# Maboroshi0327/MHAda-Style-Transfer

Hardware: AMD Instinct MI355X
Metric: stylized frames/sec (whole job) at 512x512 batch 8 fp32 [configs[1]] (higher is better)
Workload: dtype f32; 1 GPU; stylize 512x512 content+style, batch 8; resolution=512, batch_per_gpu=8, global_batch=8, compute_dtype=f32, parallelism=replicas x1

## Files before the change

### include/mhada_hip.h

```cpp
#ifndef MHADA_HIP_H
#define MHADA_HIP_H

#ifdef __cplusplus
extern "C" {
#endif

typedef void* mhada_stream_t;

enum { MHADA_OK = 0, MHADA_ERR_ARG = 1, MHADA_ERR_LAUNCH = 2 };
enum { MHADA_F32 = 0, MHADA_BF16 = 1 };
enum { MHADA_ACT_SOFTMAX = 0, MHADA_ACT_COSINE = 1 };
enum { MHADA_PAD_REFLECT = 0, MHADA_PAD_ZERO = 1 };
enum {
  MHADA_A_ROWS = 0,
  MHADA_A_PATCH8 = 1,
  MHADA_A_CONV3X3 = 2,
  MHADA_A_CONV3X3_UP2 = 3,
  MHADA_A_CONV3X3_ZERO = 4,
  MHADA_A_SPLIT3 = 5
};
enum { MHADA_BF16X3 = 2 };

int mhada_abi_version(void);
const char* mhada_last_error(void);

int mhada_set_tuning(const char* name, int value);
int mhada_get_tuning(const char* name, int* value);

int mhada_clock_probe(unsigned long long* stamps, int nblk, int iters, mhada_stream_t stream);

typedef struct mhada_gemm_args {
  int M, N, K;
  int nb1, nb2;
  int compute;
  int a_mode;
  const void* a; int a_dtype; long long lda, sa1, sa2;
  const float* a_mu; long long smu1, smu2;
  int img_c, img_h, img_w;
  const void* w; long long ldw, sw1, sw2;
  const float* bias; long long sb1, sb2;
  const void* r; int r_dtype; long long ldr, sr1, sr2;
  void* c; int c_dtype; long long ldc, sc1, sc2;
  int relu;
  int pad;
  void* c2; long long ldc2, sc21, sc22;
  void* vt; long long ldt, svt1, svt2;
  int c2_planes;
} mhada_gemm_args;

int mhada_gemm(const mhada_gemm_args* args, mhada_stream_t stream);

int mhada_layernorm(const float* x, void* y, int y_dtype, const float* gamma, const float* beta,
                    int rows, int cols, float eps, mhada_stream_t stream);

int mhada_vit_batch_attn(const void* qkv, void* out, int dtype, int L, int ntok, int heads,
                         int head_dim, mhada_stream_t stream);
int mhada_vit_batch_attn_split3(const float* qkv, void* planes, long long pstride, int L, int ntok, int heads,
                                int head_dim, mhada_stream_t stream);

int mhada_pos_embed(const float* pos, float* out, int C, int bh, int bw, int oh, int ow,
                    mhada_stream_t stream);

int mhada_instnorm_stats(const float* x, float* mu, float* rstd, double* work, int B, int N,
                         int C, int splits, float eps, mhada_stream_t stream);

int mhada_fold_block(const float* wf, const float* wg, const float* wh, const float* bg,
                     const float* bh, const float* rstd_c, const float* mu_s,
                     const float* rstd_s, void* wq, void* wkv, float* bkv, float* v_mu,
                     float kscale, int dtype, int B, int H, mhada_stream_t stream);

int mhada_transpose_v(const void* kv, void* vt, int dtype, int B, int H, int Ns, mhada_stream_t stream);

int mhada_cosine_prep(void* q, void* kv, int dtype, int B, int H, int Nc, int Ns,
                      mhada_stream_t stream);

int mhada_attn(const void* q, const void* kv, const void* vt, const float* fcs,
               const float* fcs_mu, const float* fcs_rstd, const float* v_mu, void* out,
               int dtype, int B, int H, int Nc, int Ns, int activation, mhada_stream_t stream);

int mhada_fold_block_hd(const float* wf, const float* wg, const float* wh, const float* bg,
                        const float* bh, const float* rstd_c, const float* mu_s,
                        const float* rstd_s, void* wq, void* wkv, float* bkv, float* v_mu,
                        float kscale, int dtype, int B, int H, int D, mhada_stream_t stream);

int mhada_cosine_prep_hd(void* q, void* kv, int dtype, int B, int H, int D, int Nc, int Ns,
                         mhada_stream_t stream);

int mhada_attn_hd(const void* q, const void* kv, const float* fcs, const float* fcs_mu,
                  const float* fcs_rstd, const float* v_mu, void* out, int dtype, int B, int H,
                  int D, int Nc, int Ns, int activation, mhada_stream_t stream);

int mhada_attn_wide(const void* q, const void* k, const void* v, const float* fcs, const float* fcs_mu,
                    const float* fcs_rstd, const float* v_mu, float* out, void* out16, int dtype, int B,
                    int Nc, int Ns, int D, mhada_stream_t stream);

int mhada_split3_kv(const float* kv, const float* vt, void* img, int B, int H, int Ns, mhada_stream_t stream);
int mhada_split3_rows(const float* x, void* planes, long long n, mhada_stream_t stream);
int mhada_split3_weight(const float* w, void* out, int N, int K0, int transposed, mhada_stream_t stream);

int mhada_layernorm_half2(const float* x, void* y, const float* gamma, const float* beta, int rows, int cols,
                          float eps, float scale, mhada_stream_t stream);
int mhada_half2_weight(const float* w, void* out, float* t, int N, int K0, mhada_stream_t stream);
int mhada_gemm_half2(const mhada_gemm_args* args, const float* col_scale, mhada_stream_t stream);
int mhada_gemm_half2_planes(const mhada_gemm_args* args, const float* col_scale, const float* out_scale,
                            mhada_stream_t stream);
int mhada_vit_batch_attn_half2(const float* qkv, void* planes, long long pstride, const float* out_scale, int L,
                               int ntok, int heads, int head_dim, mhada_stream_t stream);
int mhada_kv_proj_split3(const float* fs, const float* mu_s, const float* wkv, const float* bkv, void* img,
                         int B, int H, int Ns, mhada_stream_t stream);
int mhada_attn_split3(const float* q, const void* img, const float* fcs, const float* fcs_mu,
                      const float* fcs_rstd, const float* v_mu, float* out, int B, int H, int Nc, int Ns,
                      mhada_stream_t stream);
int mhada_attn_split3_planes(const float* q, const void* img, const float* fcs, const float* fcs_mu,
                             const float* fcs_rstd, const float* v_mu, void* planes, int B, int H, int Nc, int Ns,
                             mhada_stream_t stream);

int mhada_cosine_moments(const void* kv, const void* vt, int dtype, int B, int H, int Ns, float* mom,
                         float* work, int splits, mhada_stream_t stream);
int mhada_cosine_attn(const void* q, const float* mom, const float* fcs, const float* fcs_mu,
                      const float* fcs_rstd, const float* v_mu, void* out, int dtype, int B, int H,
                      int Nc, mhada_stream_t stream);

int mhada_attn_train_fwd(const float* q, const float* k, const float* v, const float* x, float* out,
                         float* mo, float* lse, int BH, int Nc, int Ns, mhada_stream_t stream);
int mhada_attn_train_fwd_vt(const float* q, const float* k, const float* v, float* vt, const float* x,
                            float* out, float* mo, float* lse, int BH, int Nc, int Ns, mhada_stream_t stream);
int mhada_attn_train_fwd_split3(const float* q, const float* k, const float* v, void* img, const float* x,
                                float* out, float* mo, float* lse, int BH, int Nc, int Ns, mhada_stream_t stream);
int mhada_transpose64(const float* src, float* dst, int BH, int N, int ldt, mhada_stream_t stream);
int mhada_gemm_n64_split3(const float* a, const void* w_planes, float* c, int nz, int M, int K, int lda,
                          long long sa, int ldw, long long sw, long long wps, int ldc, long long sc,
                          mhada_stream_t stream);
int mhada_transpose64_split3(const float* k, void* planes, int BH, int N, int ldt, mhada_stream_t stream);
int mhada_attn_train_bwd(const float* q, const float* k, const float* v, const float* lse,
                         const float* dmo, const float* dd, float* dq, float* dk, float* dv,
                         int BH, int Nc, int Ns, mhada_stream_t stream);
int mhada_attn_train_dkv(const float* q, const float* k, const float* v, const float* lse, const float* dmo,
                         const float* dd, float* dk, float* dv, float* ds, int BH, int Nc, int Ns,
                         mhada_stream_t stream);

int mhada_attn_train_fwd_hd(const float* q, const float* k, const float* v, const float* x, float* out,
                            float* mo, float* lse, int BH, int D, int Nc, int Ns, mhada_stream_t stream);
int mhada_attn_train_bwd_hd(const float* q, const float* k, const float* v, const float* lse,
                            const float* dmo, const float* dd, float* dq, float* dk, float* dv,
                            int BH, int D, int Nc, int Ns, mhada_stream_t stream);

int mhada_attn_train_dq(const float* q, const float* k, const float* v, const float* lse, const float* dmo,
                        const float* dd, float* dq, int BH, int Nc, int Ns, mhada_stream_t stream);
int mhada_attn_train_dq_hd(const float* q, const float* k, const float* v, const float* lse, const float* dmo,
                           const float* dd, float* dq, int BH, int D, int Nc, int Ns, mhada_stream_t stream);

long long mhada_attn_train_bf16_workspace(int BH, int Nc, int Ns, int backward);
int mhada_attn_train_fwd_bf16(const float* q, const float* k, const float* v, const float* x, float* out,
                              float* mo, float* lse, void* ws, long long ws_size, int BH, int Nc, int Ns,
                              mhada_stream_t stream);
int mhada_attn_train_bwd_bf16(const float* q, const float* k, const float* v, const float* lse,
                              const float* dmo, const float* mo, float* dq, float* dk, float* dv,
                              void* ws, long long ws_size, int BH, int Nc, int Ns, int phases,
                              mhada_stream_t stream);

int mhada_conv3x3_out3(const void* x, int dtype, const float* w, const float* b, float* y,
                       int B, int H, int W, int Cin, int clamp255, mhada_stream_t stream);

int mhada_upsample2x(const void* x, void* y, int dtype, int B, int H, int W, int C,
                     mhada_stream_t stream);


int mhada_warp(const float* x, const float* flow, float* y, int B, int C, int H, int W,
               int padding, mhada_stream_t stream);

int mhada_warp_bwd(const float* gy, const float* flow, float* gx, int B, int C, int H, int W,
                   int padding, mhada_stream_t stream);

int mhada_flow_warp_mask(const float* flo01, const float* flo10, float* mask, int H, int W,
                         float threshold, int padding, mhada_stream_t stream);

int mhada_warp_l1(const float* cs1, const float* cs2, const float* flow, const float* mask,
                  double* work, float* out, int B, int C, int H, int W, mhada_stream_t stream);


typedef struct mhada_gemm_tn_args {
  int M, N, K;
  const float* a; long long lda;
  const float* b; long long ldb;
  int b_mode;
  int img_c, img_h, img_w, pad;
  float* c; long long ldc;
  float* colsum;
  int nb;
  long long sza, szb;
} mhada_gemm_tn_args;
int mhada_gemm_tn_splits(int M, int N, int K);
int mhada_gemm_tn(const mhada_gemm_tn_args* args, float* work, long long work_floats, mhada_stream_t stream);

int mhada_vit_batch_attn_bwd(const float* qkv, const float* dout, float* dqkv, int L, int ntok, int heads,
                             int head_dim, mhada_stream_t stream);
int mhada_vit_batch_attn_bwd_split3(const float* qkv, const float* dout, float* dqkv, void* planes,
                                    long long pstride, int L, int ntok, int heads, int head_dim,
                                    mhada_stream_t stream);

int mhada_colsum(const float* x, float* out, long long rows, int C, float* work, long long work_floats,
                 mhada_stream_t stream);

int mhada_layernorm_fwd(const float* x, float* y, float* stats, const float* gamma, const float* beta,
                        int rows, int cols, float eps, mhada_stream_t stream);
int mhada_layernorm_fwd_split3(const float* x, float* y, void* planes, float* stats, const float* gamma,
                               const float* beta, int rows, int cols, float eps, mhada_stream_t stream);

int mhada_layernorm_bwd(const float* x, const float* dy, const float* stats, const float* gamma, float* dx,
                        float* dgamma, float* dbeta, float* work, long long work_floats, int rows, int cols,
                        mhada_stream_t stream);

int mhada_instnorm_bwd(const float* dy, const float* y, const float* rstd, float* dx, double* work,
                       int B, int N, int C, int splits, mhada_stream_t stream);

int mhada_attn_train_bwd_prep(const float* dout, const float* x, const float* mo, float* dx, float* dmo,
                              float* dd, long long rows, mhada_stream_t stream);
int mhada_attn_train_bwd_prep_hd(const float* dout, const float* x, const float* mo, float* dx, float* dmo,
                                 float* dd, long long rows, int D, mhada_stream_t stream);

int mhada_pos_embed_bwd(const float* g, float* gpos, int C, int bh, int bw, int oh, int ow,
                        mhada_stream_t stream);
long long mhada_feat_stats_work(int B, long long P, int C);
int mhada_feat_stats(const float* x, const float* t, float* mu, float* sd, float* mse, double* work,
                     long long work_doubles, int B, long long P, int C, mhada_stream_t stream);
int mhada_feat_loss_bwd(const float* x, const float* t, const float* mu, const float* alpha, const float* beta,
                        const float* kp, float ks, float* g, int B, long long P, int C, int relu, mhada_stream_t stream);
int mhada_relu_bwd(const float* dy, const float* y, float* dx, long long n, mhada_stream_t stream);
int mhada_reflect_fold(const float* dxp, float* dx, int B, int H, int W, int C, const float* relu_mask,
                       mhada_stream_t stream);
int mhada_maxpool2(const float* x, float* y, int B, int H, int W, int C, mhada_stream_t stream);
int mhada_maxpool2_bwd(const float* x, const float* dy, float* dx, int B, int H, int W, int C, int relu_mask,
                       mhada_stream_t stream);
int mhada_upsample2x_bwd(const float* dy, const float* relu_x, float* dx, int B, int H, int W, int C,
                         mhada_stream_t stream);
int mhada_vgg_input(const float* img, float* out, int B, int H, int W, int Cp, mhada_stream_t stream);
int mhada_vgg_input_bwd(const float* dout, float* dimg, int B, int H, int W, int Cp, mhada_stream_t stream);

int mhada_loss_attn(const float* q, const float* k, const float* v, const float* x, const float* x_mu,
                    const float* x_rs, float* out, int B, int Nq, int Ns, int Dqk, int Dv, int activation,
                    mhada_stream_t stream);
int mhada_rows_normalize(const float* x, const float* mu, const float* rs, float* out, int unit,
                         int B, int N, int C, mhada_stream_t stream);

int mhada_frame_ingest(const void* frames, int B, int H, int W, long long row_bytes, int bgr, float* out,
                       int Ho, int Wo, mhada_stream_t stream);

int mhada_wino_weights(const float* w, float* u, int Cout, int Cin, mhada_stream_t stream);
int mhada_conv3x3_wgrad_wino_splits(int B, int H, int W, int Cin, int Cout);
int mhada_conv3x3_wgrad_wino(const float* x, const float* g, float* dw, float* db, float* work, long long work_floats,
                             int B, int H, int W, int Cin, int Cout, long long ldg, int pad_mode,
                             mhada_stream_t stream);
int mhada_conv3x3_wino(const float* x, const float* u, const float* bias, float* y, int B, int H, int W,
                       int Cin, int Cout, long long ldc, int pad_mode, int pad, int relu,
                       const float* relu_mask, mhada_stream_t stream);
int mhada_wino_weights_split3(const float* w, void* up, int Cout, int Cin, mhada_stream_t stream);
int mhada_conv3x3_wino_split3(const float* x, const float* u, const void* up, const float* bias, float* y, int B,
                              int H, int W, int Cin, int Cout, long long ldc, int pad_mode, int pad, int relu,
                              const float* relu_mask, mhada_stream_t stream);

int mhada_vgg_stem_dgrad(const float* dy, const float* y, const float* wd, float* dimg, int B, int H, int W,
                         mhada_stream_t stream);
int mhada_out3_dgrad(const float* dy, const float* y, const float* wd, const float* relu_x, float* dx, int B, int H,
                     int W, mhada_stream_t stream);
long long mhada_out3_wgrad_work(int B, int H, int W);
int mhada_out3_wgrad(const float* x, const float* dy, const float* y, float* dw, float* db, float* work,
                     long long work_floats, int B, int H, int W, mhada_stream_t stream);

int mhada_patch_embed_dgrad(const float* dy, const float* w, float* dimg, int B, int C, int Ci, int H, int W,
                            mhada_stream_t stream);

#ifdef __cplusplus
}
#endif
#endif
```

### mhada-style-transfer_amd/csrc/attn_split3.hip

```cpp
#include "attn_common.h"

namespace mhada {

constexpr int kS3Tk = 64;

__host__ __device__ constexpr long long s3_image(int ldt) { return 576LL * ldt; }

struct Bf3 { bf16 a, b, c; };
MHADA_DEV Bf3 split3(float x) {
  const bf16 a = (bf16)x;
  const float r = x - (float)a;
  const bf16 b = (bf16)r;
  return Bf3{a, b, (bf16)(r - (float)b)};
}
template <typename V>
MHADA_DEV void split3_into(float x, V& a, V& b, V& c, int e) {
  const Bf3 s = split3(x);
  a[e] = s.a;
  b[e] = s.b;
  c[e] = s.c;
}

__global__ void __launch_bounds__(256) split3_kv_kernel(const float* __restrict__ kv, const float* __restrict__ vt,
                                                        bf16* __restrict__ img, int Ns, int ldt) {
  const int bh = blockIdx.y, n0 = blockIdx.x * 64, tid = threadIdx.x;
  bf16* kp = img + (long long)bh * s3_image(ldt);
  bf16* vp = kp + 192LL * ldt;
  const float* kvb = kv + (long long)bh * Ns * 128;
  const float* vtb = vt + (long long)bh * 128 * ldt;
  const long long kps = 64LL * ldt, vps = 128LL * ldt;
#pragma unroll
  for (int i = 0; i < 4; ++i) {
    const int idx = tid + 256 * i, key = n0 + (idx >> 4), d = (idx & 15) * 4;
    const f32x4 x = key < Ns ? *reinterpret_cast<const f32x4*>(kvb + (long long)key * 128 + d) : f32x4{0.f, 0.f, 0.f, 0.f};
    bf16x4 a, b, c;
#pragma unroll
    for (int e = 0; e < 4; ++e) split3_into(x[e], a, b, c, e);
    bf16* dst = kp + (long long)key * 64 + d;
    *reinterpret_cast<bf16x4*>(dst) = a;
    *reinterpret_cast<bf16x4*>(dst + kps) = b;
    *reinterpret_cast<bf16x4*>(dst + 2 * kps) = c;
  }
#pragma unroll
  for (int i = 0; i < 4; ++i) {
    const int idx = tid + 256 * i, row = idx >> 3, a8 = idx & 7;
    const float* src = vtb + (long long)row * ldt + n0 + 16 * (a8 >> 1) + 4 * (a8 & 1);
    const f32x4 lo = *reinterpret_cast<const f32x4*>(src), hi = *reinterpret_cast<const f32x4*>(src + 8);
    bf16x8 a, b, c;
#pragma unroll
    for (int j = 0; j < 8; ++j) split3_into(j < 4 ? lo[j] : hi[j - 4], a, b, c, j);
    bf16* dst = vp + (long long)row * ldt + n0 + 8 * a8;
    *reinterpret_cast<bf16x8*>(dst) = a;
    *reinterpret_cast<bf16x8*>(dst + vps) = b;
    *reinterpret_cast<bf16x8*>(dst + 2 * vps) = c;
  }
}

__global__ void __launch_bounds__(256) kv_proj_s3_kernel(const float* __restrict__ fs, const float* __restrict__ mu,
                                                         const float* __restrict__ wkv, const float* __restrict__ bkv,
                                                         bf16* __restrict__ img, int H, int Ns, int ldt) {
  constexpr int LX = 65, LY = 65;
  __shared__ float sm[192 * LX];
  float* sX = sm;
  float* sW = sm + 64 * LX;
  float* sY = sm;
  const int bh = blockIdx.y, b = bh / H, h = bh - b * H, n0 = blockIdx.x * 64, tid = threadIdx.x;
  const int C = 64 * H;
  const float* xb = fs + (long long)b * Ns * C + 64 * h;
  const float* mb = mu + (long long)b * C + 64 * h;
  const float* wb = wkv + (long long)bh * 128 * 64;
#pragma unroll
  for (int i = 0; i < 4; ++i) {
    const int idx = tid + 256 * i, n = idx >> 4, c = (idx & 15) * 4;
    f32x4 x = {0.f, 0.f, 0.f, 0.f};
    if (n0 + n < Ns) {
      x = *reinterpret_cast<const f32x4*>(xb + (long long)(n0 + n) * C + c);
      const f32x4 m = *reinterpret_cast<const f32x4*>(mb + c);
      x = x - m;
    }
#pragma unroll
    for (int e = 0; e < 4; ++e) sX[n * LX + c + e] = x[e];
  }
#pragma unroll
  for (int i = 0; i < 8; ++i) {
    const int idx = tid + 256 * i, o = idx >> 4, c = (idx & 15) * 4;
    const f32x4 w = *reinterpret_cast<const f32x4*>(wb + o * 64 + c);
#pragma unroll
    for (int e = 0; e < 4; ++e) sW[o * LX + c + e] = w[e];
  }
  __syncthreads();
  const int lane = tid & 63, wave = tid >> 6, r32 = lane & 31, hh = lane >> 5;
  const int nb = wave & 1, ob = wave >> 1;
  f32x16 acc[2] = {};
#pragma unroll 8
  for (int k = 0; k < 64; k += 2) {
    const float bv = sX[(32 * nb + r32) * LX + k + hh];
#pragma unroll
    for (int ni = 0; ni < 2; ++ni)
      acc[ni] = __builtin_amdgcn_mfma_f32_32x32x2f32(sW[(64 * ob + 32 * ni + r32) * LX + k + hh], bv, acc[ni], 0, 0, 0);
  }
  const float* bb = bkv + h * 128;
  __syncthreads();
#pragma unroll
  for (int ni = 0; ni < 2; ++ni)
#pragma unroll
    for (int r = 0; r < 16; ++r) {
      const int o = 64 * ob + 32 * ni + (r & 3) + 8 * (r >> 2) + 4 * hh;
      sY[o * LY + 32 * nb + r32] = acc[ni][r] + bb[o];
    }
  __syncthreads();
  bf16* kp = img + (long long)bh * s3_image(ldt);
  bf16* vp = kp + 192LL * ldt;
  const long long kps = 64LL * ldt, vps = 128LL * ldt;
#pragma unroll
  for (int i = 0; i < 2; ++i) {
    const int idx = tid + 256 * i, n = idx >> 3, o0 = (idx & 7) * 8;
    const bool valid = n0 + n < Ns;
    bf16x8 a, c1, c2;
#pragma unroll
    for (int j = 0; j < 8; ++j) split3_into(valid ? sY[(o0 + j) * LY + n] : 0.f, a, c1, c2, j);
    bf16* dst = kp + (long long)(n0 + n) * 64 + o0;
    *reinterpret_cast<bf16x8*>(dst) = a;
    *reinterpret_cast<bf16x8*>(dst + kps) = c1;
    *reinterpret_cast<bf16x8*>(dst + 2 * kps) = c2;
  }
#pragma unroll
  for (int i = 0; i < 2; ++i) {
    const int idx = tid + 256 * i, vo = idx >> 3, a8 = idx & 7;
    bf16x8 a, c1, c2, s0, s1, s2;
#pragma unroll
    for (int j = 0; j < 8; ++j) {
      const int n = 16 * (a8 >> 1) + 8 * (j >> 2) + 4 * (a8 & 1) + (j & 3);
      const float v = n0 + n < Ns ? sY[(64 + vo) * LY + n] : 0.f;
      split3_into(v, a, c1, c2, j);
      split3_into(v * v, s0, s1, s2, j);
    }
    bf16* dst = vp + (long long)vo * ldt + n0 + 8 * a8;
    *reinterpret_cast<bf16x8*>(dst) = a;
    *reinterpret_cast<bf16x8*>(dst + vps) = c1;
    *reinterpret_cast<bf16x8*>(dst + 2 * vps) = c2;
    *reinterpret_cast<bf16x8*>(dst + 64LL * ldt) = s0;
    *reinterpret_cast<bf16x8*>(dst + 64LL * ldt + vps) = s1;
    *reinterpret_cast<bf16x8*>(dst + 64LL * ldt + 2 * vps) = s2;
  }
}

MHADA_DEV f32x4 mfma6(const bf16x8& a0, const bf16x8& a1, const bf16x8& a2, const bf16x8& b0, const bf16x8& b1,
                      const bf16x8& b2, f32x4 acc) {
  acc = __builtin_amdgcn_mfma_f32_16x16x32_bf16(a2, b0, acc, 0, 0, 0);
  acc = __builtin_amdgcn_mfma_f32_16x16x32_bf16(a1, b1, acc, 0, 0, 0);
  acc = __builtin_amdgcn_mfma_f32_16x16x32_bf16(a0, b2, acc, 0, 0, 0);
  acc = __builtin_amdgcn_mfma_f32_16x16x32_bf16(a1, b0, acc, 0, 0, 0);
  acc = __builtin_amdgcn_mfma_f32_16x16x32_bf16(a0, b1, acc, 0, 0, 0);
  return __builtin_amdgcn_mfma_f32_16x16x32_bf16(a0, b0, acc, 0, 0, 0);
}

template <bool QK32>
MHADA_DEV void attn_exact_q3(const AttnP& p, const bf16* kp, const bf16* vp, const bf16x8 (&qf)[3][2][2],
                             const float (&qreg)[2][16], f32x4 (&O)[2][8], float (&lt)[2], float (&mx)[2], int g,
                             int r16) {
  const int Ns = p.Ns;
  const long long kps = 64LL * p.ldt, vps = 128LL * p.ldt;
  const f32x4 z4 = {0.f, 0.f, 0.f, 0.f};
  auto scores = [&](int k0, f32x4 (&S)[2][2]) {
#pragma unroll
    for (int t = 0; t < 2; ++t) {
      const bf16* kr = kp + (long long)(k0 + fsq_key(r16, t)) * 64 + 8 * g;
#pragma unroll
      for (int qg = 0; qg < 2; ++qg) S[qg][t] = z4;
      if constexpr (QK32) {
        const float* kf = reinterpret_cast<const float*>(kp) + (long long)(k0 + fsq_key(r16, t)) * 64 + 16 * g;
#pragma unroll
        for (int st = 0; st < 16; ++st)
#pragma unroll
          for (int qg = 0; qg < 2; ++qg) S[qg][t] = __builtin_amdgcn_mfma_f32_16x16x4f32(kf[st], qreg[qg][st], S[qg][t], 0, 0, 0);
      }
#pragma unroll
      for (int dh = 0; dh < (QK32 ? 0 : 2); ++dh) {
        const bf16x8 k0f = *reinterpret_cast<const bf16x8*>(kr + 32 * dh);
        const bf16x8 k1f = *reinterpret_cast<const bf16x8*>(kr + kps + 32 * dh);
        const bf16x8 k2f = *reinterpret_cast<const bf16x8*>(kr + 2 * kps + 32 * dh);
#pragma unroll
        for (int qg = 0; qg < 2; ++qg)
          S[qg][t] = mfma6(k0f, k1f, k2f, qf[0][qg][dh], qf[1][qg][dh], qf[2][qg][dh], S[qg][t]);
      }
#pragma unroll
      for (int j = 0; j < 4; ++j)
        if (k0 + fsq_key(4 * g + j, t) >= Ns) S[0][t][j] = S[1][t][j] = -INFINITY;
    }
  };
  float m2[2] = {-INFINITY, -INFINITY};
  for (int k0 = 0; k0 < Ns; k0 += 32) {
    f32x4 S[2][2];
    scores(k0, S);
#pragma unroll
    for (int qg = 0; qg < 2; ++qg)
#pragma unroll
      for (int t = 0; t < 2; ++t)
#pragma unroll
        for (int j = 0; j < 4; ++j) m2[qg] = fmaxf(m2[qg], S[qg][t][j]);
  }
#pragma unroll
  for (int qg = 0; qg < 2; ++qg) {
    m2[qg] = fmaxf(m2[qg], __shfl_xor(m2[qg], 16, 64));
    m2[qg] = fmaxf(m2[qg], __shfl_xor(m2[qg], 32, 64));
    lt[qg] = 0.f;
#pragma unroll
    for (int i = 0; i < 8; ++i) O[qg][i] = z4;
  }
  for (int k0 = 0; k0 < Ns; k0 += 32) {
    f32x4 S[2][2];
    scores(k0, S);
    bf16x8 pf[3][2];
#pragma unroll
    for (int qg = 0; qg < 2; ++qg)
#pragma unroll
      for (int j = 0; j < 8; ++j) {
        const float e = fast_exp2(S[qg][j >> 2][j & 3] - m2[qg]);
        lt[qg] += e;
        split3_into(e, pf[0][qg], pf[1][qg], pf[2][qg], j);
      }
#pragma unroll
    for (int dvb = 0; dvb < 8; ++dvb) {
      const bf16* vr = vp + (long long)(16 * dvb + r16) * p.ldt + k0 + 8 * g;
      const bf16x8 v0 = *reinterpret_cast<const bf16x8*>(vr);
      const bf16x8 v1 = *reinterpret_cast<const bf16x8*>(vr + vps);
      const bf16x8 v2 = *reinterpret_cast<const bf16x8*>(vr + 2 * vps);
#pragma unroll
      for (int qg = 0; qg < 2; ++qg) O[qg][dvb] += mfma6(v0, v1, v2, pf[0][qg], pf[1][qg], pf[2][qg], z4);
    }
  }
#pragma unroll
  for (int qg = 0; qg < 2; ++qg) {
    lt[qg] += __shfl_xor(lt[qg], 16, 64);
    lt[qg] += __shfl_xor(lt[qg], 32, 64);
    mx[qg] = m2[qg];
  }
}

MHADA_DEV void s3_mask(f32x4 (&S)[2][2][2], int key0, int Ns, int g) {
#pragma unroll
  for (int kg = 0; kg < 2; ++kg)
#pragma unroll
    for (int t = 0; t < 2; ++t)
#pragma unroll
      for (int j = 0; j < 4; ++j)
        if (key0 + 32 * kg + fsq_key(4 * g + j, t) >= Ns) S[0][kg][t][j] = S[1][kg][t][j] = -INFINITY;
}

__global__ void __launch_bounds__(256) train_s3_prep_kernel(const float* __restrict__ k, const float* __restrict__ v,
                                                            bf16* __restrict__ img, int Ns, int ldt) {
  __shared__ float sv[64 * 65];
  const int bh = blockIdx.y, n0 = blockIdx.x * 64, tid = threadIdx.x;
  bf16* kp = img + (long long)bh * s3_image(ldt);
  bf16* vp = kp + 192LL * ldt;
  const float* kb = k + (long long)bh * Ns * 64;
  const float* vb = v + (long long)bh * Ns * 64;
  const long long vps = 128LL * ldt;
#pragma unroll
  for (int i = 0; i < 4; ++i) {
    const int idx = tid + 256 * i, n = idx >> 4, d = (idx & 15) * 4;
    const bool ok = n0 + n < Ns;
    const f32x4 x = ok ? *reinterpret_cast<const f32x4*>(kb + (long long)(n0 + n) * 64 + d) : f32x4{0.f, 0.f, 0.f, 0.f};
    const f32x4 y = ok ? *reinterpret_cast<const f32x4*>(vb + (long long)(n0 + n) * 64 + d) : f32x4{0.f, 0.f, 0.f, 0.f};
    float* kf = reinterpret_cast<float*>(kp) + (long long)(n0 + n) * 64 + d / 4;
#pragma unroll
    for (int e = 0; e < 4; ++e) kf[16 * e] = x[e];
#pragma unroll
    for (int e = 0; e < 4; ++e) sv[n * 65 + d + e] = y[e];
  }
  __syncthreads();
#pragma unroll
  for (int i = 0; i < 2; ++i) {
    const int idx = tid + 256 * i, o = idx >> 3, a8 = idx & 7;
    bf16x8 a, c1, c2, s0, s1, s2;
#pragma unroll
    for (int j = 0; j < 8; ++j) {
      const int n = 16 * (a8 >> 1) + 8 * (j >> 2) + 4 * (a8 & 1) + (j & 3);
      const float x = sv[n * 65 + o];
      split3_into(x, a, c1, c2, j);
      split3_into(x * x, s0, s1, s2, j);
    }
    bf16* dst = vp + (long long)o * ldt + n0 + 8 * a8;
    *reinterpret_cast<bf16x8*>(dst) = a;
    *reinterpret_cast<bf16x8*>(dst + vps) = c1;
    *reinterpret_cast<bf16x8*>(dst + 2 * vps) = c2;
    *reinterpret_cast<bf16x8*>(dst + 64LL * ldt) = s0;
    *reinterpret_cast<bf16x8*>(dst + 64LL * ldt + vps) = s1;
    *reinterpret_cast<bf16x8*>(dst + 64LL * ldt + 2 * vps) = s2;
  }
}

MHADA_DEV void attn_train_epilogue_q(const AttnP& p, const f32x4 (&O)[2][8], const float (&lt)[2],
                                     const float (&m2)[2], long long bh, int q0, int g, int r16) {
#pragma unroll
  for (int qg = 0; qg < 2; ++qg) {
    const int q = q0 + 16 * qg + r16;
    if (q >= p.Nc) continue;
    const float inv = 1.0f / lt[qg];
    const long long row = bh * p.Nc + q;
    const float* xr = p.fcs + row * 64;
    float* orow = reinterpret_cast<float*>(p.out) + row * 64;
    float* mrow = p.mo + row * 128;
#pragma unroll
    for (int dvb = 0; dvb < 4; ++dvb) {
      const int dv0 = 16 * dvb + 4 * g;
      const f32x4 xx = *reinterpret_cast<const f32x4*>(xr + dv0);
      f32x4 o, mm, ee;
#pragma unroll
      for (int e = 0; e < 4; ++e) {
        const float m1 = O[qg][dvb][e] * inv;
        const float e2 = O[qg][dvb + 4][e] * inv;
        o[e] = sqrtf(fmaxf(e2 - m1 * m1, 1e-6f)) * xx[e] + m1;
        mm[e] = m1;
        ee[e] = e2;
      }
      *reinterpret_cast<f32x4*>(orow + dv0) = o;
      *reinterpret_cast<f32x4*>(mrow + dv0) = mm;
      *reinterpret_cast<f32x4*>(mrow + 64 + dv0) = ee;
    }
    if (g == 0) p.lse[row] = m2[qg] + __log2f(lt[qg]);
  }
}

template <int NW, bool TRAIN = false, bool QK32 = false, int ACC = 0, int IL = 0, bool PLANES = false>
__global__ void __launch_bounds__(64 * NW, 1) attn_s3_kernel(const AttnP p) {
  constexpr int TK = kS3Tk;
  constexpr int KPL = TK * 64, VPL = 128 * TK;
  constexpr int KREG = QK32 ? 2 * TK * 64 : 3 * KPL;
  constexpr int SLOT = KREG + 3 * VPL;
  constexpr int KPC = KREG / 512, VPC = 3 * VPL / 512;
  static_assert(KPC % NW == 0 && VPC % NW == 0, "tile config");
  constexpr int KPW = KPC / NW, VPW = VPC / NW;
  __shared__ __attribute__((aligned(16))) bf16 smem[2 * SLOT];
  int b, hh, qb;
  decode_block(p, b, hh, qb);
  const int tid = threadIdx.x, lane = tid & 63, wave = __builtin_amdgcn_readfirstlane(tid >> 6);
  const int g = lane >> 4, r16 = lane & 15;
  const int q0 = qb * (32 * NW) + wave * 32;
  const long long bh = (long long)b * p.H + hh;
  const int Ns = p.Ns, ldt = p.ldt;
  const f32x4 z4 = {0.f, 0.f, 0.f, 0.f};

  bf16x8 qf[3][2][2];
  float qreg[2][16];
#pragma unroll
  for (int qg = 0; qg < 2; ++qg) {
    const int q = q0 + 16 * qg + r16;
    if constexpr (QK32) {
      const float* qr = reinterpret_cast<const float*>(p.q) + (bh * p.Nc + (q < p.Nc ? q : 0)) * 64 + g;
#pragma unroll
      for (int st = 0; st < 16; ++st) qreg[qg][st] = q < p.Nc ? qr[4 * st] * 1.4426950408889634f : 0.f;
      continue;
    }
    const float* qp = reinterpret_cast<const float*>(p.q) + (bh * p.Nc + (q < p.Nc ? q : 0)) * 64 + 8 * g;
#pragma unroll
    for (int dh = 0; dh < 2; ++dh) {
      const f32x4 lo = *reinterpret_cast<const f32x4*>(qp + 32 * dh);
      const f32x4 hi = *reinterpret_cast<const f32x4*>(qp + 32 * dh + 4);
#pragma unroll
      for (int e = 0; e < 8; ++e) {
        const float x = q < p.Nc ? (e < 4 ? lo[e] : hi[e - 4]) * (TRAIN ? 1.4426950408889634f : 1.0f) : 0.f;
        split3_into(x, qf[0][qg][dh], qf[1][qg][dh], qf[2][qg][dh], e);
      }
    }
  }
  const bf16* kp = reinterpret_cast<const bf16*>(p.kv) + bh * s3_image(ldt);
  const bf16* vp = kp + 192LL * ldt;
  int ksrc[KPW], vsrc[VPW];
#pragma unroll
  for (int i = 0; i < KPW; ++i) {
    if constexpr (QK32) {
      const int pc = NW * i + wave, row = 4 * pc + (lane >> 4), slot = lane & 15;
      const int f = (row & 3) | (((row >> 2) & 1) << 3);
      ksrc[i] = 2 * (row * 64 + 4 * (slot ^ f));
    } else {
      const int pc = NW * i + wave, pl = pc >> 3, row = 8 * (pc & 7) + (lane >> 3), slot = lane & 7;
      ksrc[i] = pl * 64 * ldt + row * 64 + 8 * (slot ^ (row & 7));
    }
  }
#pragma unroll
  for (int i = 0; i < VPW; ++i) {
    const int pc = NW * i + wave, pl = pc >> 4, row = 8 * (pc & 15) + (lane >> 3), slot = lane & 7;
    vsrc[i] = pl * 128 * ldt + row * ldt + 8 * (slot ^ ((row >> 1) & 7));
  }
  auto stage = [&](int key0, int sl) {
    bf16* kd = smem + sl * SLOT;
    bf16* vd = kd + KREG;
    const bf16* ks = kp + (long long)key0 * (QK32 ? 128 : 64);
    const bf16* vs = vp + key0;
#pragma unroll
    for (int i = 0; i < KPW; ++i) attn_glds16(ks + ksrc[i], kd + 512 * (NW * i + wave));
#pragma unroll
    for (int i = 0; i < VPW; ++i) attn_glds16(vs + vsrc[i], vd + 512 * (NW * i + wave));
  };
  int krow[2];
#pragma unroll
  for (int t = 0; t < 2; ++t) krow[t] = fsq_key(r16, t) * 64;
  auto qk = [&](int sl, f32x4 (&S)[2][2][2], const f32x4 (&init)[2]) {
    if constexpr (QK32) {
      const float* ck = reinterpret_cast<const float*>(smem + sl * SLOT);
      const int f = (r16 & 3) | (((r16 >> 2) & 1) << 3);
#pragma unroll
      for (int kg = 0; kg < 2; ++kg)
#pragma unroll
        for (int t = 0; t < 2; ++t) {
          const float* kr = ck + (kg * 32 + fsq_key(r16, t)) * 64;
          f32x4 kf[4];
#pragma unroll
          for (int j = 0; j < 4; ++j) kf[j] = *reinterpret_cast<const f32x4*>(kr + 4 * ((4 * g + j) ^ f));
#pragma unroll
          for (int st = 0; st < 16; ++st)
#pragma unroll
            for (int qg = 0; qg < 2; ++qg)
              S[qg][kg][t] = __builtin_amdgcn_mfma_f32_16x16x4f32(kf[st >> 2][st & 3], qreg[qg][st],
                                                                  st == 0 ? init[qg] : S[qg][kg][t], 0, 0, 0);
        }
      return;
    }
    const bf16* ck = smem + sl * SLOT;
#pragma unroll
    for (int kg = 0; kg < 2; ++kg)
#pragma unroll
      for (int t = 0; t < 2; ++t) {
        const bf16* kr = ck + kg * 32 * 64 + krow[t];
#pragma unroll
        for (int dh = 0; dh < 2; ++dh) {
          const int off = 8 * ((4 * dh + g) ^ (r16 & 7));
          const bf16x8 k0f = *reinterpret_cast<const bf16x8*>(kr + off);
          const bf16x8 k1f = *reinterpret_cast<const bf16x8*>(kr + KPL + off);
          const bf16x8 k2f = *reinterpret_cast<const bf16x8*>(kr + 2 * KPL + off);
#pragma unroll
          for (int qg = 0; qg < 2; ++qg)
            S[qg][kg][t] = mfma6(k0f, k1f, k2f, qf[0][qg][dh], qf[1][qg][dh], qf[2][qg][dh],
                                 dh == 0 ? init[qg] : S[qg][kg][t]);
        }
      }
  };
  f32x4 O[2][8], L[2];
  float lsum[2] = {0.f, 0.f};
#pragma unroll
  for (int qg = 0; qg < 2; ++qg) {
    L[qg] = z4;
#pragma unroll
    for (int i = 0; i < 8; ++i) O[qg][i] = z4;
  }
  bf16x8 ones;
#pragma unroll
  for (int j = 0; j < 8; ++j) ones[j] = (bf16)1.0f;
  auto pv = [&](int sl, int kg, int dvb, const bf16x8 (&pf)[3][2]) {
    const int off = 8 * ((4 * kg + g) ^ ((r16 >> 1) & 7));
    const bf16* vr = smem + sl * SLOT + KREG + (16 * dvb + r16) * TK + off;
    const bf16x8 v0 = *reinterpret_cast<const bf16x8*>(vr);
    const bf16x8 v1 = *reinterpret_cast<const bf16x8*>(vr + VPL);
    const bf16x8 v2 = *reinterpret_cast<const bf16x8*>(vr + 2 * VPL);
#pragma unroll
    for (int qg = 0; qg < 2; ++qg) O[qg][dvb] = mfma6(v0, v1, v2, pf[0][qg], pf[1][qg], pf[2][qg], O[qg][dvb]);
  };
  auto rowsum = [&](const bf16x8 (&pf)[3][2]) {
#pragma unroll
    for (int qg = 0; qg < 2; ++qg) {
      L[qg] = __builtin_amdgcn_mfma_f32_16x16x32_bf16(ones, pf[2][qg], L[qg], 0, 0, 0);
      L[qg] = __builtin_amdgcn_mfma_f32_16x16x32_bf16(ones, pf[1][qg], L[qg], 0, 0, 0);
      L[qg] = __builtin_amdgcn_mfma_f32_16x16x32_bf16(ones, pf[0][qg], L[qg], 0, 0, 0);
    }
  };
  auto finish = [&](int sl, const f32x4 (&S)[2][2][2]) {
    const bf16* cv = smem + sl * SLOT + KREG;
    if constexpr (IL != 0 && ACC == 0) {
      bf16x8 pa[3][2], pb[3][2];
#pragma unroll
      for (int qg = 0; qg < 2; ++qg)
#pragma unroll
        for (int j = 0; j < 8; ++j) split3_into(fast_exp2(S[qg][0][j >> 2][j & 3]), pa[0][qg], pa[1][qg], pa[2][qg], j);
      rowsum(pa);
#pragma unroll
      for (int dvb = 0; dvb < 8; ++dvb) {
        pv(sl, 0, dvb, pa);
        const int qg = dvb >> 2, j = 2 * (dvb & 3);
        split3_into(fast_exp2(S[qg][1][j >> 2][j & 3]), pb[0][qg], pb[1][qg], pb[2][qg], j);
        split3_into(fast_exp2(S[qg][1][(j + 1) >> 2][(j + 1) & 3]), pb[0][qg], pb[1][qg], pb[2][qg], j + 1);
      }
      rowsum(pb);
#pragma unroll
      for (int dvb = 0; dvb < 8; ++dvb) pv(sl, 1, dvb, pb);
      return;
    }
#pragma unroll
    for (int kg = 0; kg < 2; ++kg) {
      bf16x8 pf[3][2];
#pragma unroll
      for (int qg = 0; qg < 2; ++qg)
#pragma unroll
        for (int j = 0; j < 8; ++j) split3_into(fast_exp2(S[qg][kg][j >> 2][j & 3]), pf[0][qg], pf[1][qg], pf[2][qg], j);
#pragma unroll
      for (int qg = 0; qg < 2; ++qg) {
        if constexpr (ACC == 0) {
          L[qg] = __builtin_amdgcn_mfma_f32_16x16x32_bf16(ones, pf[2][qg], L[qg], 0, 0, 0);
          L[qg] = __builtin_amdgcn_mfma_f32_16x16x32_bf16(ones, pf[1][qg], L[qg], 0, 0, 0);
          L[qg] = __builtin_amdgcn_mfma_f32_16x16x32_bf16(ones, pf[0][qg], L[qg], 0, 0, 0);
        } else {
          f32x4 t = __builtin_amdgcn_mfma_f32_16x16x32_bf16(ones, pf[2][qg], z4, 0, 0, 0);
          t = __builtin_amdgcn_mfma_f32_16x16x32_bf16(ones, pf[1][qg], t, 0, 0, 0);
          t = __builtin_amdgcn_mfma_f32_16x16x32_bf16(ones, pf[0][qg], t, 0, 0, 0);
          lsum[qg] += t[0];
        }
      }
      const int off = 8 * ((4 * kg + g) ^ ((r16 >> 1) & 7));
      f32x4 tp[2];
#pragma unroll
      for (int dvb = 0; dvb < 8; ++dvb) {
        const bf16* vr = cv + (16 * dvb + r16) * TK + off;
        const bf16x8 v0 = *reinterpret_cast<const bf16x8*>(vr);
        const bf16x8 v1 = *reinterpret_cast<const bf16x8*>(vr + VPL);
        const bf16x8 v2 = *reinterpret_cast<const bf16x8*>(vr + 2 * VPL);
        if constexpr (ACC == 0) {
#pragma unroll
          for (int qg = 0; qg < 2; ++qg) O[qg][dvb] = mfma6(v0, v1, v2, pf[0][qg], pf[1][qg], pf[2][qg], O[qg][dvb]);
        } else {
          f32x4 tn[2];
#pragma unroll
          for (int qg = 0; qg < 2; ++qg) tn[qg] = mfma6(v0, v1, v2, pf[0][qg], pf[1][qg], pf[2][qg], z4);
          if (dvb > 0) {
#pragma unroll
            for (int qg = 0; qg < 2; ++qg) O[qg][dvb - 1] += tp[qg];
          }
#pragma unroll
          for (int qg = 0; qg < 2; ++qg) tp[qg] = tn[qg];
        }
      }
      if constexpr (ACC != 0) {
#pragma unroll
        for (int qg = 0; qg < 2; ++qg) O[qg][7] += tp[qg];
      }
    }
  };

  const int NTILE = (Ns + TK - 1) / TK, NFULL = Ns / TK;
  stage(0, 0);
  asm volatile("s_waitcnt vmcnt(0)" ::: "memory");
  __syncthreads();
  f32x4 Sa[2][2][2], Cm[2];
  {
    const f32x4 zi[2] = {z4, z4};
    qk(0, Sa, zi);
    if (NFULL == 0) s3_mask(Sa, 0, Ns, g);
#pragma unroll
    for (int qg = 0; qg < 2; ++qg) {
      float m = -INFINITY;
#pragma unroll
      for (int kg = 0; kg < 2; ++kg)
#pragma unroll
        for (int t = 0; t < 2; ++t)
#pragma unroll
          for (int j = 0; j < 4; ++j) m = fmaxf(m, Sa[qg][kg][t][j]);
      m = fmaxf(m, __shfl_xor(m, 16, 64));
      m = fmaxf(m, __shfl_xor(m, 32, 64));
#pragma unroll
      for (int kg = 0; kg < 2; ++kg)
#pragma unroll
        for (int t = 0; t < 2; ++t)
#pragma unroll
          for (int j = 0; j < 4; ++j) Sa[qg][kg][t][j] -= m;
      Cm[qg] = f32x4{-m, -m, -m, -m};
    }
  }
  if (NTILE > 1) stage(TK, 1);
  finish(0, Sa);
  asm volatile("s_waitcnt vmcnt(0)" ::: "memory");
  __builtin_amdgcn_s_barrier();
  for (int t = 1; t < NFULL; ++t) {
    if (t + 1 < NTILE) stage((t + 1) * TK, (t + 1) & 1);
    qk(t & 1, Sa, Cm);
    finish(t & 1, Sa);
    asm volatile("s_waitcnt vmcnt(0)" ::: "memory");
    __builtin_amdgcn_s_barrier();
  }
  if (NFULL < NTILE && NFULL > 0) {
    qk(NFULL & 1, Sa, Cm);
    s3_mask(Sa, NFULL * TK, Ns, g);
    finish(NFULL & 1, Sa);
  }
  float lt[2], mx[2];
#pragma unroll
  for (int qg = 0; qg < 2; ++qg) {
    lt[qg] = ACC ? lsum[qg] : L[qg][0];
    mx[qg] = -Cm[qg][0];
  }
  if (__any(!(lt[0] <= kShiftSumThr) || !(lt[1] <= kShiftSumThr))) attn_exact_q3<QK32>(p, kp, vp, qf, qreg, O, lt, mx, g, r16);
  if constexpr (TRAIN) attn_train_epilogue_q(p, O, lt, mx, bh, q0, g, r16);
  else attn_epilogue_q<float, PLANES>(p, O, lt, b, hh, q0, g, r16);
}

static int s3_num_cus() {
  static int n = 0;
  if (n == 0) {
    int dev = 0;
    (void)hipGetDevice(&dev);
    if (hipDeviceGetAttribute(&n, hipDeviceAttributeMultiprocessorCount, dev) != hipSuccess || n <= 0) n = 256;
  }
  return n;
}

}

using namespace mhada;

extern "C" int mhada_split3_kv(const float* kv, const float* vt, void* img, int B, int H, int Ns, mhada_stream_t s_) {
  if (!kv || !vt || !img || B <= 0 || H <= 0 || Ns <= 0) return fail("mhada_split3_kv: bad args");
  const long long bhn = (long long)B * H;
  if (bhn > 65535) return fail("mhada_split3_kv: B * H > 65535");
  const int ldt = (Ns + 63) / 64 * 64;
  hipLaunchKernelGGL(split3_kv_kernel, dim3(ldt / 64, (unsigned)bhn), dim3(256), 0, (hipStream_t)s_, kv, vt,
                     reinterpret_cast<bf16*>(img), Ns, ldt);
  return check_launch("mhada_split3_kv");
}

extern "C" int mhada_kv_proj_split3(const float* fs, const float* mu_s, const float* wkv, const float* bkv, void* img,
                                    int B, int H, int Ns, mhada_stream_t s_) {
  if (!fs || !mu_s || !wkv || !bkv || !img || B <= 0 || H <= 0 || Ns <= 0) return fail("mhada_kv_proj_split3: bad args");
  const long long bhn = (long long)B * H;
  if (bhn > 65535) return fail("mhada_kv_proj_split3: B * H > 65535");
  const int ldt = (Ns + 63) / 64 * 64;
  hipLaunchKernelGGL(kv_proj_s3_kernel, dim3(ldt / 64, (unsigned)bhn), dim3(256), 0, (hipStream_t)s_, fs, mu_s, wkv, bkv,
                     reinterpret_cast<bf16*>(img), H, Ns, ldt);
  return check_launch("mhada_kv_proj_split3");
}

static int attn_split3_launch(const char* name, const float* q, const void* img, const float* fcs, const float* fcs_mu,
                              const float* fcs_rstd, const float* v_mu, void* out, bool planes, int B, int H, int Nc,
                              int Ns, mhada_stream_t s_) {
  if (!q || !img || !fcs || !fcs_mu || !fcs_rstd || !v_mu || !out || B <= 0 || H <= 0 || Nc <= 0 || Ns <= 0)
    return fail(std::string(name) + ": bad args");
  AttnP p = {};
  p.q = q; p.kv = img; p.vt = img; p.fcs = fcs; p.fcs_mu = fcs_mu; p.fcs_rstd = fcs_rstd; p.v_mu = v_mu;
  p.out = out; p.B = B; p.H = H; p.Nc = Nc; p.Ns = Ns;
  p.ldt = (Ns + 63) / 64 * 64;
  if (384LL * p.ldt >= (1LL << 31)) return fail(std::string(name) + ": Ns too large for 32-bit plane offsets");
  int nw = tuning().attn_waves;
  if (nw == 0) nw = (long long)B * H * ((Nc + 255) / 256) < s3_num_cus() ? 4 : 8;
  p.nqb = (Nc + 32 * nw - 1) / (32 * nw);
  const long long nblk = (long long)B * H * p.nqb;
  if (nblk > (1LL << 31) - 1) return fail(std::string(name) + ": grid too large");
  p.nblk = (int)nblk;
  const hipStream_t s = (hipStream_t)s_;
  if (planes) {
    if (nw == 8) hipLaunchKernelGGL((attn_s3_kernel<8, false, false, 0, 1, true>), dim3(p.nblk), dim3(512), 0, s, p);
    else hipLaunchKernelGGL((attn_s3_kernel<4, false, false, 0, 1, true>), dim3(p.nblk), dim3(256), 0, s, p);
  } else {
    if (nw == 8) hipLaunchKernelGGL((attn_s3_kernel<8, false, false, 0, 1>), dim3(p.nblk), dim3(512), 0, s, p);
    else hipLaunchKernelGGL((attn_s3_kernel<4, false, false, 0, 1>), dim3(p.nblk), dim3(256), 0, s, p);
  }
  return check_launch(name);
}

extern "C" int mhada_attn_split3(const float* q, const void* img, const float* fcs, const float* fcs_mu,
                                 const float* fcs_rstd, const float* v_mu, float* out, int B, int H, int Nc, int Ns,
                                 mhada_stream_t s_) {
  return attn_split3_launch("mhada_attn_split3", q, img, fcs, fcs_mu, fcs_rstd, v_mu, out, false, B, H, Nc, Ns, s_);
}

extern "C" int mhada_attn_split3_planes(const float* q, const void* img, const float* fcs, const float* fcs_mu,
                                        const float* fcs_rstd, const float* v_mu, void* planes, int B, int H, int Nc,
                                        int Ns, mhada_stream_t s_) {
  return attn_split3_launch("mhada_attn_split3_planes", q, img, fcs, fcs_mu, fcs_rstd, v_mu, planes, true, B, H, Nc, Ns,
                            s_);
}

extern "C" int mhada_attn_train_fwd_split3(const float* q, const float* k, const float* v, void* img, const float* x,
                                           float* out, float* mo, float* lse, int BH, int Nc, int Ns,
                                           mhada_stream_t s_) {
  if (!q || !k || !v || !img || !x || !out || !mo || !lse || BH <= 0 || Nc <= 0 || Ns <= 0)
    return fail("mhada_attn_train_fwd_split3: bad args");
  if (BH > 65535) return fail("mhada_attn_train_fwd_split3: BH > 65535");
  const hipStream_t s = (hipStream_t)s_;
  AttnP p = {};
  p.q = q; p.kv = img; p.vt = img; p.fcs = x; p.out = out; p.mo = mo; p.lse = lse;
  p.B = BH; p.H = 1; p.Nc = Nc; p.Ns = Ns; p.ldk = 64;
  p.ldt = (Ns + 63) / 64 * 64;
  if (384LL * p.ldt >= (1LL << 31)) return fail("mhada_attn_train_fwd_split3: Ns too large for 32-bit plane offsets");
  int nw = tuning().attn_waves;
  if (nw == 0) nw = (long long)BH * ((Nc + 255) / 256) < s3_num_cus() ? 4 : 8;
  p.nqb = (Nc + 32 * nw - 1) / (32 * nw);
  const long long nblk = (long long)BH * p.nqb;
  if (nblk > (1LL << 31) - 1) return fail("mhada_attn_train_fwd_split3: grid too large");
  p.nblk = (int)nblk;
  hipLaunchKernelGGL(train_s3_prep_kernel, dim3(p.ldt / 64, BH), dim3(256), 0, s, k, v, reinterpret_cast<bf16*>(img),
                     Ns, p.ldt);
  if (nw == 8) hipLaunchKernelGGL((attn_s3_kernel<8, true, true, 1>), dim3(p.nblk), dim3(512), 0, s, p);
  else hipLaunchKernelGGL((attn_s3_kernel<4, true, true, 1>), dim3(p.nblk), dim3(256), 0, s, p);
  return check_launch("mhada_attn_train_fwd_split3");
}
```

### mhada-style-transfer_amd/mhada_hip/_lib.py

```python
from __future__ import annotations

import ctypes
import os
import threading

LIB_PATH = os.path.join(os.path.dirname(os.path.abspath(__file__)), "libmhada_hip.so")

F32, BF16 = 0, 1
ACT_SOFTMAX, ACT_COSINE = 0, 1
A_ROWS, A_PATCH8, A_CONV3X3, A_CONV3X3_UP2, A_CONV3X3_ZERO, A_SPLIT3 = 0, 1, 2, 3, 4, 5
BF16X3 = 2
PAD_REFLECT, PAD_ZERO = 0, 1

_c_ll = ctypes.c_longlong
_vp = ctypes.c_void_p


class GemmArgs(ctypes.Structure):
    _fields_ = [
        ("M", ctypes.c_int), ("N", ctypes.c_int), ("K", ctypes.c_int),
        ("nb1", ctypes.c_int), ("nb2", ctypes.c_int),
        ("compute", ctypes.c_int), ("a_mode", ctypes.c_int),
        ("a", _vp), ("a_dtype", ctypes.c_int), ("lda", _c_ll), ("sa1", _c_ll), ("sa2", _c_ll),
        ("a_mu", _vp), ("smu1", _c_ll), ("smu2", _c_ll),
        ("img_c", ctypes.c_int), ("img_h", ctypes.c_int), ("img_w", ctypes.c_int),
        ("w", _vp), ("ldw", _c_ll), ("sw1", _c_ll), ("sw2", _c_ll),
        ("bias", _vp), ("sb1", _c_ll), ("sb2", _c_ll),
        ("r", _vp), ("r_dtype", ctypes.c_int), ("ldr", _c_ll), ("sr1", _c_ll), ("sr2", _c_ll),
        ("c", _vp), ("c_dtype", ctypes.c_int), ("ldc", _c_ll), ("sc1", _c_ll), ("sc2", _c_ll),
        ("relu", ctypes.c_int), ("pad", ctypes.c_int),
        ("c2", _vp), ("ldc2", _c_ll), ("sc21", _c_ll), ("sc22", _c_ll),
        ("vt", _vp), ("ldt", _c_ll), ("svt1", _c_ll), ("svt2", _c_ll),
        ("c2_planes", ctypes.c_int),
    ]


class GemmTnArgs(ctypes.Structure):
    _fields_ = [
        ("M", ctypes.c_int), ("N", ctypes.c_int), ("K", ctypes.c_int),
        ("a", _vp), ("lda", _c_ll), ("b", _vp), ("ldb", _c_ll), ("b_mode", ctypes.c_int),
        ("img_c", ctypes.c_int), ("img_h", ctypes.c_int), ("img_w", ctypes.c_int), ("pad", ctypes.c_int),
        ("c", _vp), ("ldc", _c_ll), ("colsum", _vp),
        ("nb", ctypes.c_int), ("sza", _c_ll), ("szb", _c_ll),
    ]


_I, _F = ctypes.c_int, ctypes.c_float
SIGNATURES = {
    "mhada_abi_version": (_I, []),
    "mhada_last_error": (ctypes.c_char_p, []),
    "mhada_set_tuning": (_I, [ctypes.c_char_p, _I]),
    "mhada_get_tuning": (_I, [ctypes.c_char_p, ctypes.POINTER(_I)]),
    "mhada_clock_probe": (_I, [_vp, _I, _I, _vp]),
    "mhada_gemm": (_I, [ctypes.POINTER(GemmArgs), _vp]),
    "mhada_layernorm": (_I, [_vp, _vp, _I, _vp, _vp, _I, _I, _F, _vp]),
    "mhada_vit_batch_attn": (_I, [_vp, _vp, _I, _I, _I, _I, _I, _vp]),
    "mhada_vit_batch_attn_split3": (_I, [_vp, _vp, _c_ll, _I, _I, _I, _I, _vp]),
    "mhada_pos_embed": (_I, [_vp, _vp, _I, _I, _I, _I, _I, _vp]),
    "mhada_instnorm_stats": (_I, [_vp, _vp, _vp, _vp, _I, _I, _I, _I, _F, _vp]),
    "mhada_fold_block": (_I, [_vp] * 12 + [_F, _I, _I, _I, _vp]),
    "mhada_transpose_v": (_I, [_vp, _vp, _I, _I, _I, _I, _vp]),
    "mhada_cosine_prep": (_I, [_vp, _vp, _I, _I, _I, _I, _I, _vp]),
    "mhada_cosine_moments": (_I, [_vp, _vp, _I, _I, _I, _I, _vp, _vp, _I, _vp]),
    "mhada_cosine_attn": (_I, [_vp, _vp, _vp, _vp, _vp, _vp, _vp, _I, _I, _I, _I, _vp]),
    "mhada_attn": (_I, [_vp] * 8 + [_I, _I, _I, _I, _I, _I, _vp]),
    "mhada_fold_block_hd": (_I, [_vp] * 12 + [_F, _I, _I, _I, _I, _vp]),
    "mhada_cosine_prep_hd": (_I, [_vp, _vp, _I, _I, _I, _I, _I, _I, _vp]),
    "mhada_attn_hd": (_I, [_vp] * 7 + [_I, _I, _I, _I, _I, _I, _I, _vp]),
    "mhada_attn_wide": (_I, [_vp] * 9 + [_I, _I, _I, _I, _I, _vp]),
    "mhada_split3_kv": (_I, [_vp, _vp, _vp, _I, _I, _I, _vp]),
    "mhada_kv_proj_split3": (_I, [_vp] * 5 + [_I, _I, _I, _vp]),
    "mhada_split3_rows": (_I, [_vp, _vp, _c_ll, _vp]),
    "mhada_split3_weight": (_I, [_vp, _vp, _I, _I, _I, _vp]),
    "mhada_layernorm_half2": (_I, [_vp, _vp, _vp, _vp, _I, _I, _F, _F, _vp]),
    "mhada_half2_weight": (_I, [_vp, _vp, _vp, _I, _I, _vp]),
    "mhada_gemm_half2": (_I, [ctypes.POINTER(GemmArgs), _vp, _vp]),
    "mhada_gemm_half2_planes": (_I, [ctypes.POINTER(GemmArgs), _vp, _vp, _vp]),
    "mhada_vit_batch_attn_half2": (_I, [_vp, _vp, _c_ll, _vp, _I, _I, _I, _I, _vp]),
    "mhada_attn_split3": (_I, [_vp] * 7 + [_I, _I, _I, _I, _vp]),
    "mhada_attn_split3_planes": (_I, [_vp] * 7 + [_I, _I, _I, _I, _vp]),
    "mhada_attn_train_fwd": (_I, [_vp] * 7 + [_I, _I, _I, _vp]),
    "mhada_attn_train_fwd_vt": (_I, [_vp] * 8 + [_I, _I, _I, _vp]),
    "mhada_attn_train_fwd_split3": (_I, [_vp] * 8 + [_I, _I, _I, _vp]),
    "mhada_transpose64": (_I, [_vp, _vp, _I, _I, _I, _vp]),
    "mhada_gemm_n64_split3": (_I, [_vp, _vp, _vp, _I, _I, _I, _I, _c_ll, _I, _c_ll, _c_ll, _I, _c_ll, _vp]),
    "mhada_transpose64_split3": (_I, [_vp, _vp, _I, _I, _I, _vp]),
    "mhada_attn_train_bwd": (_I, [_vp] * 9 + [_I, _I, _I, _vp]),
    "mhada_attn_train_dkv": (_I, [_vp] * 9 + [_I, _I, _I, _vp]),
    "mhada_attn_train_fwd_hd": (_I, [_vp] * 7 + [_I, _I, _I, _I, _vp]),
    "mhada_attn_train_bwd_hd": (_I, [_vp] * 9 + [_I, _I, _I, _I, _vp]),
    "mhada_attn_train_dq": (_I, [_vp] * 7 + [_I, _I, _I, _vp]),
    "mhada_attn_train_dq_hd": (_I, [_vp] * 7 + [_I, _I, _I, _I, _vp]),
    "mhada_patch_embed_dgrad": (_I, [_vp, _vp, _vp, _I, _I, _I, _I, _I, _vp]),
    "mhada_attn_train_bf16_workspace": (_c_ll, [_I, _I, _I, _I]),
    "mhada_attn_train_fwd_bf16": (_I, [_vp] * 8 + [_c_ll, _I, _I, _I, _vp]),
    "mhada_attn_train_bwd_bf16": (_I, [_vp] * 10 + [_c_ll, _I, _I, _I, _I, _vp]),
    "mhada_conv3x3_out3": (_I, [_vp, _I, _vp, _vp, _vp, _I, _I, _I, _I, _I, _vp]),
    "mhada_upsample2x": (_I, [_vp, _vp, _I, _I, _I, _I, _I, _vp]),
    "mhada_warp": (_I, [_vp, _vp, _vp, _I, _I, _I, _I, _I, _vp]),
    "mhada_warp_bwd": (_I, [_vp, _vp, _vp, _I, _I, _I, _I, _I, _vp]),
    "mhada_flow_warp_mask": (_I, [_vp, _vp, _vp, _I, _I, _F, _I, _vp]),
    "mhada_warp_l1": (_I, [_vp, _vp, _vp, _vp, _vp, _vp, _I, _I, _I, _I, _vp]),
    "mhada_frame_ingest": (_I, [_vp, _I, _I, _I, _c_ll, _I, _vp, _I, _I, _vp]),
    "mhada_gemm_tn_splits": (_I, [_I, _I, _I]),
    "mhada_loss_attn": (_I, [_vp] * 7 + [_I, _I, _I, _I, _I, _I, _vp]),
    "mhada_rows_normalize": (_I, [_vp] * 4 + [_I, _I, _I, _I, _vp]),
    "mhada_gemm_tn": (_I, [ctypes.POINTER(GemmTnArgs), _vp, _c_ll, _vp]),
    "mhada_colsum": (_I, [_vp, _vp, _c_ll, _I, _vp, _c_ll, _vp]),
    "mhada_layernorm_fwd": (_I, [_vp, _vp, _vp, _vp, _vp, _I, _I, _F, _vp]),
    "mhada_layernorm_fwd_split3": (_I, [_vp, _vp, _vp, _vp, _vp, _vp, _I, _I, _F, _vp]),
    "mhada_layernorm_bwd": (_I, [_vp, _vp, _vp, _vp, _vp, _vp, _vp, _vp, _c_ll, _I, _I, _vp]),
    "mhada_pos_embed_bwd": (_I, [_vp, _vp, _I, _I, _I, _I, _I, _vp]),
    "mhada_instnorm_bwd": (_I, [_vp, _vp, _vp, _vp, _vp, _I, _I, _I, _I, _vp]),
    "mhada_attn_train_bwd_prep": (_I, [_vp, _vp, _vp, _vp, _vp, _vp, _c_ll, _vp]),
    "mhada_attn_train_bwd_prep_hd": (_I, [_vp, _vp, _vp, _vp, _vp, _vp, _c_ll, _I, _vp]),
    "mhada_vit_batch_attn_bwd": (_I, [_vp, _vp, _vp, _I, _I, _I, _I, _vp]),
    "mhada_vit_batch_attn_bwd_split3": (_I, [_vp, _vp, _vp, _vp, _c_ll, _I, _I, _I, _I, _vp]),
    "mhada_relu_bwd": (_I, [_vp, _vp, _vp, _c_ll, _vp]),
    "mhada_feat_stats_work": (_c_ll, [_I, _c_ll, _I]),
    "mhada_feat_stats": (_I, [_vp, _vp, _vp, _vp, _vp, _vp, _c_ll, _I, _c_ll, _I, _vp]),
    "mhada_feat_loss_bwd": (_I, [_vp, _vp, _vp, _vp, _vp, _vp, _F, _vp, _I, _c_ll, _I, _I, _vp]),
    "mhada_reflect_fold": (_I, [_vp, _vp, _I, _I, _I, _I, _vp, _vp]),
    "mhada_maxpool2": (_I, [_vp, _vp, _I, _I, _I, _I, _vp]),
    "mhada_maxpool2_bwd": (_I, [_vp, _vp, _vp, _I, _I, _I, _I, _I, _vp]),
    "mhada_upsample2x_bwd": (_I, [_vp, _vp, _vp, _I, _I, _I, _I, _vp]),
    "mhada_vgg_input": (_I, [_vp, _vp, _I, _I, _I, _I, _vp]),
    "mhada_vgg_input_bwd": (_I, [_vp, _vp, _I, _I, _I, _I, _vp]),
    "mhada_wino_weights": (_I, [_vp, _vp, _I, _I, _vp]),
    "mhada_conv3x3_wgrad_wino_splits": (_I, [_I, _I, _I, _I, _I]),
    "mhada_conv3x3_wgrad_wino": (_I, [_vp, _vp, _vp, _vp, _vp, _c_ll, _I, _I, _I, _I, _I, _c_ll, _I, _vp]),
    "mhada_conv3x3_wino": (_I, [_vp] * 4 + [_I] * 5 + [_c_ll, _I, _I, _I, _vp, _vp]),
    "mhada_conv3x3_wino_split3": (_I, [_vp] * 5 + [_I] * 5 + [_c_ll, _I, _I, _I, _vp, _vp]),
    "mhada_wino_weights_split3": (_I, [_vp, _vp, _I, _I, _vp]),
    "mhada_vgg_stem_dgrad": (_I, [_vp] * 4 + [_I] * 3 + [_vp]),
    "mhada_out3_dgrad": (_I, [_vp] * 5 + [_I] * 3 + [_vp]),
    "mhada_out3_wgrad_work": (_c_ll, [_I, _I, _I]),
    "mhada_out3_wgrad": (_I, [_vp] * 6 + [_c_ll, _I, _I, _I, _vp]),
}

_lib = None
_lock = threading.Lock()


def load(path: str | None = None) -> ctypes.CDLL:
    global _lib
    if _lib is not None and path is None:
        return _lib
    with _lock:
        if _lib is not None and path is None:
            return _lib
        p = path or LIB_PATH
        if not os.path.exists(p):
            raise RuntimeError(
                f"MHAda HIP library not found at {p}; build it with "
                "`python -c 'import __graft_entry__ as g; g.build()'` (make -C mhada-style-transfer_amd/csrc)")
        lib = ctypes.CDLL(p)
        for name, (res, args) in SIGNATURES.items():
            fn = getattr(lib, name)
            fn.restype = res
            fn.argtypes = args
        if path is None:
            _lib = lib
        return lib


ABI_VERSION = 18


def get_tuning(name: str) -> int:
    v = ctypes.c_int()
    check(load().mhada_get_tuning(name.encode(), ctypes.byref(v)), "mhada_get_tuning")
    return v.value


def set_tuning(name: str, value: int) -> None:
    check(load().mhada_set_tuning(name.encode(), int(value)), "mhada_set_tuning")


class tuning:

    def __init__(self, **knobs: int):
        self.knobs = knobs
        self.saved = {}

    def __enter__(self):
        for k, v in self.knobs.items():
            self.saved[k] = get_tuning(k)
            set_tuning(k, v)
        return self

    def __exit__(self, *exc):
        for k, v in self.saved.items():
            set_tuning(k, v)
        return False


def check(rc: int, what: str) -> None:
    if rc != 0:
        msg = load().mhada_last_error()
        msg = msg.decode() if msg else "unknown error"
        if rc == 1:
            raise ValueError(f"{what}: {msg}")
        raise RuntimeError(f"{what}: {msg}")
```

### mhada-style-transfer_amd/mhada_hip/engine.py

```python
from __future__ import annotations

from typing import Dict, List, Optional, Sequence, Tuple

import weakref

import torch

from . import ops
from ._lib import ACT_COSINE, ACT_SOFTMAX

HEAD_DIM = 64
DECODER_LAYERS: Tuple[Tuple[str, bool], ...] = (
    ("conv1.0", False), ("conv1.1", True), ("conv1.2", False), ("conv1.3", False),
    ("conv1.4", False), ("conv2.0", True), ("conv2.1", False), ("conv3.0", True),
)
LAST_LAYER = "conv3.1"
FUSE_UPSAMPLE = {torch.float32: False, torch.bfloat16: False}


def _fuse_upsample(dt: torch.dtype, w: torch.Tensor) -> bool:
    return FUSE_UPSAMPLE[dt] or (dt == torch.bfloat16 and w.shape[0] == 64 and w.shape[1] == 9 * 64)


_event_log = None


def record_kernel_events(log) -> None:
    global _event_log
    _event_log = log


class _timed:
    def __init__(self, name):
        self.name = name

    def __enter__(self):
        if _event_log is not None:
            self.s = torch.cuda.Event(enable_timing=True)
            self.s.record()
        return self

    def __exit__(self, *exc):
        if _event_log is not None:
            e = torch.cuda.Event(enable_timing=True)
            e.record()
            _event_log.setdefault(self.name, []).append((self.s, e))
        return False


def resolve_compute_dtype(module: torch.nn.Module) -> torch.dtype:
    explicit = getattr(module, "compute_dtype", None)
    if explicit is not None:
        if explicit not in (torch.float32, torch.bfloat16):
            raise ValueError(f"compute_dtype must be torch.float32 or torch.bfloat16, got {explicit}")
        return explicit
    if torch.is_autocast_enabled("cuda"):
        if torch.get_autocast_dtype("cuda") in (torch.bfloat16, torch.float16):
            return torch.bfloat16
    return torch.float32


def _signature(module: torch.nn.Module):
    return tuple((p.data_ptr(), p._version) for p in module.parameters())


def cached_prep(module: torch.nn.Module, dtype: torch.dtype, build):
    cache: Dict = module.__dict__.setdefault("_mhada_prep", {})
    key = (dtype, _signature(module))
    hit = cache.get(dtype)
    if hit is not None and hit[0] == key:
        return hit[1]
    with torch.no_grad():
        prep = build(dtype)
    cache[dtype] = (key, prep)
    return prep


def require_device(t: torch.Tensor, what: str) -> None:
    if not t.is_cuda:
        raise RuntimeError(f"{what}: the MI355X-native network runs on ROCm device tensors only; "
                           "move the module and inputs with .to('cuda')")


def to_tokens(x: torch.Tensor) -> torch.Tensor:
    t = x.permute(0, 2, 3, 1)
    if t.dtype != torch.float32:
        t = t.float()
    return t.contiguous()


def tokens_to_nchw(t: torch.Tensor, h: int, w: int) -> torch.Tensor:
    B, _, C = t.shape
    return t.view(B, h, w, C).permute(0, 3, 1, 2)


def vit_prep(vit, dtype):
    def build(dt):
        pe = vit.patch_embedding.conv_proj
        layers = []
        for blk in vit.encoder:
            att = blk.attention
            layers.append(dict(
                ln1_g=blk.ln1.weight.float().contiguous(), ln1_b=blk.ln1.bias.float().contiguous(),
                ln2_g=blk.ln2.weight.float().contiguous(), ln2_b=blk.ln2.bias.float().contiguous(),
                w_qkv=att.in_proj_weight.to(dt).contiguous(), b_qkv=att.in_proj_bias.float().contiguous(),
                w_o=att.out_proj.weight.to(dt).contiguous(), b_o=att.out_proj.bias.float().contiguous(),
                w1=blk.mlp[0].weight.to(dt).contiguous(), b1=blk.mlp[0].bias.float().contiguous(),
                w2=blk.mlp[2].weight.to(dt).contiguous(), b2=blk.mlp[2].bias.float().contiguous(),
                heads=att.num_heads, eps=blk.ln1.eps))
        return dict(patch_w=pe.weight.reshape(pe.weight.shape[0], -1).to(dt).contiguous(),
                    patch_b=pe.bias.float().contiguous(), layers=layers, pos={})
    return cached_prep(vit, dtype, build)


_NUM_CUS: Dict = {}


def _split3_fills(M: int, N: int, dev: torch.device) -> bool:
    if not ops.F32_SPLIT:
        return False
    idx = dev.index if dev.index is not None else torch.cuda.current_device()
    if idx not in _NUM_CUS:
        _NUM_CUS[idx] = torch.cuda.get_device_properties(idx).multi_processor_count
    return 8 * ((M + 255) // 256) * ((N + 255) // 256) >= 7 * _NUM_CUS[idx]


def _w6(L: dict, key: str) -> torch.Tensor:
    k6 = key + "_split3"
    if k6 not in L:
        with torch.no_grad():
            L[k6] = ops.split3_weight(L[key])
    return L[k6]


def _h2(L: dict, ln: str, key: str) -> Optional[dict]:
    if not ops.F32_HALF2:
        return None
    k2 = key + "_half2"
    if k2 not in L:
        with torch.no_grad():
            L[k2] = ops.half2_prepare(L[ln + "_g"], L[ln + "_b"], L[key])
    return L[k2]


def _h2_chain(L: dict, key: str) -> Optional[dict]:
    if not (ops.F32_HALF2 and ops.F32_HALF2_CHAIN) or (key == "w_o" and not ops.F32_HALF2_CHAIN_OUTPROJ):
        return None
    k2 = key + "_half2"
    if k2 not in L:
        with torch.no_grad():
            if key == "w2":
                L[k2] = None if _h2(L, "ln2", "w1") is None else \
                    ops.half2_chain_prepare(L["ln2_g"], L["ln2_b"], L["w1"], L["b1"], L["w2"])
            else:
                C = L["w_o"].shape[1]
                L[k2] = ops.half2_chain_prepare(L["ln1_g"], L["ln1_b"], L["w_qkv"][2 * C:], L["b_qkv"][2 * C:],
                                                L["w_o"])
    return L[k2]


def vit_forward(vit, x: torch.Tensor) -> List[torch.Tensor]:
    require_device(x, "VisionTransformer")
    dt = resolve_compute_dtype(vit)
    prep = vit_prep(vit, dt)
    if x.dim() != 4 or x.shape[1] != 3:
        raise ValueError(f"expected an image batch (B, 3, H, W), got {tuple(x.shape)}")
    img = x.float().contiguous()
    B, _, H, W = img.shape
    p = vit.patch_size
    h, w = H // p, W // p
    N = h * w
    C = prep["patch_w"].shape[0]
    pos = None
    if vit.pos_embedding is not None:
        pos = prep["pos"].get((h, w))
        if pos is None:
            pos = ops.pos_embed(vit.pos_embedding.pos_embed.detach().float().contiguous(), h, w)
            prep["pos"][(h, w)] = pos
    tok = ops.patch_embed(img, prep["patch_w"], prep["patch_b"], pos, p)
    xs = tok.view(B * N, C)
    outs = []
    for L in prep["layers"]:
        split = dt == torch.float32 and _split3_fills(B * N, 3 * C, xs.device)
        split_mlp = dt == torch.float32 and _split3_fills(B * N, C, xs.device)
        h2q = _h2(L, "ln1", "w_qkv") if split else None
        h2m = _h2(L, "ln2", "w1") if split_mlp else None
        if h2q is not None:
            qkv = ops.linear_half2(ops.layernorm_half2(xs, L["ln1_g"], L["ln1_b"], L["eps"], h2q["s_a"]),
                                   h2q["w2"], h2q["cs"], L["b_qkv"], dt)
        elif split:
            qkv = ops.linear_split3(ops.layernorm_split3(xs, L["ln1_g"], L["ln1_b"], L["eps"]), _w6(L, "w_qkv"),
                                    L["b_qkv"], dt)
        else:
            hb = ops.layernorm(xs, L["ln1_g"], L["ln1_b"], dt, L["eps"])
            qkv = ops.linear(hb, L["w_qkv"], L["b_qkv"], dt)
        if split_mlp and ops.F32_SPLIT_OUTPROJ and C == L["heads"] * HEAD_DIM and B <= ops.VIT_ATTN_SPLIT3_MAX_L:
            h2o = _h2_chain(L, "w_o")
            if h2o is not None:
                att2 = ops.vit_batch_attn_half2(qkv.view(B, N, 3 * C), B, N, L["heads"], h2o["u"])
                xs = ops.linear_half2_planes(att2, h2o["w2"], h2o["cs"], L["b_o"], residual=xs)
            else:
                att3 = ops.vit_batch_attn_split3(qkv.view(B, N, 3 * C), B, N, L["heads"])
                xs = ops.linear_split3(att3, _w6(L, "w_o"), L["b_o"], torch.float32, residual=xs)
        else:
            att = ops.vit_batch_attn(qkv.view(B, N, 3 * C), B, N, L["heads"])
            xs = ops.linear(att.view(B * N, C), L["w_o"], L["b_o"], torch.float32, residual=xs)
        if split_mlp:
            h2c = _h2_chain(L, "w2")
            if h2m is not None:
                m1 = ops.linear_half2(ops.layernorm_half2(xs, L["ln2_g"], L["ln2_b"], L["eps"], h2m["s_a"]),
                                      h2m["w2"], h2m["cs"], L["b1"], dt, relu=True, out_planes=True,
                                      out_scale=h2c["u"] if h2c is not None else None)
            else:
                m1 = ops.linear_split3(ops.layernorm_split3(xs, L["ln2_g"], L["ln2_b"], L["eps"]), _w6(L, "w1"),
                                       L["b1"], dt, relu=True, out_planes=True)
            if h2c is not None:
                xs = ops.linear_half2_planes(m1, h2c["w2"], h2c["cs"], L["b2"], residual=xs)
            else:
                xs = ops.linear_split3(m1, _w6(L, "w2"), L["b2"], torch.float32, residual=xs)
        else:
            h2 = ops.layernorm(xs, L["ln2_g"], L["ln2_b"], dt, L["eps"])
            m1 = ops.linear(h2, L["w1"], L["b1"], dt, relu=True)
            xs = ops.linear(m1, L["w2"], L["b2"], torch.float32, residual=xs)
        outs.append(tokens_to_nchw(xs.view(B, N, C), h, w))
    return outs


def block_prep(blk, dtype):
    def build(dt):
        H = blk.num_heads
        d = blk.head_dim

        def stack(lst):
            return torch.stack([m.weight.reshape(d, d) for m in lst]).float().contiguous()

        def stackb(lst):
            return torch.stack([m.bias for m in lst]).float().contiguous()
        C = H * d
        return dict(wf=stack(blk.f_list), wg=stack(blk.g_list), wh=stack(blk.h_list),
                    bf=stackb(blk.f_list), bg=stackb(blk.g_list), bh=stackb(blk.h_list),
                    w_out=blk.out_conv.weight.reshape(C, C).to(dt).contiguous(),
                    b_out=blk.out_conv.bias.float().contiguous())
    return cached_prep(blk, dtype, build)


class _Feat:

    def __init__(self, t: torch.Tensor, h: int, w: int):
        self.t, self.h, self.w = t, h, w
        self._stats = None
        self.t16 = None

    @classmethod
    def from_nchw(cls, x: torch.Tensor):
        _, _, h, w = x.shape
        t = to_tokens(x)
        return cls(t.view(t.shape[0], h * w, t.shape[3]), h, w)

    def stats(self):
        if self._stats is None:
            self._stats = ops.instnorm_stats(self.t)
        return self._stats


def block_forward(blk, fc: _Feat, fs: Optional[_Feat], fcs: _Feat, dt: torch.dtype,
                  side: Optional[dict] = None, want_bf16: bool = False) -> _Feat:
    if blk.head_dim in ops.HD_WIDTHS:
        return _block_forward_hd(blk, fc, fs, fcs, dt, side, want_bf16)
    if blk.head_dim != HEAD_DIM:
        raise ValueError("the HIP MHAda kernels implement head_dim (qkv_dim/num_heads) in {32, 64, 128}, "
                         f"got {blk.head_dim}")
    prep = block_prep(blk, dt)
    H = blk.num_heads
    C = H * HEAD_DIM
    B, Nc, Cc = fc.t.shape
    cached = bool(side)
    mom = img = kv = vt = None
    act = ACT_COSINE if blk.activation_name == "cosine" else ACT_SOFTMAX
    split_attn = act == ACT_SOFTMAX and dt == torch.float32 and ops.F32_SPLIT_ATTN
    if cached:
        mu_s, rstd_s, mom, Ns = side["mu_s"], side["rstd_s"], side.get("mom"), side["Ns"]
        kv, vt, img = side.get("kv"), side.get("vt"), side.get("img")
        if side["B"] != B:
            raise ValueError(f"cached style batch {side['B']} != content batch {B}")
    else:
        if fs.t.shape[2] != C:
            raise ValueError(f"channel mismatch: block expects {C}")
        mu_s, rstd_s = fs.stats()
    if Cc != C or fcs.t.shape[2] != C:
        raise ValueError(f"channel mismatch: block expects {C}")
    mu_c, rstd_c = fc.stats()
    mu_o, rstd_o = fcs.stats()
    wq, wkv, bkv, v_mu = ops.fold_block(prep["wf"], prep["wg"], prep["wh"], prep["bg"], prep["bh"],
                                        rstd_c, mu_s, rstd_s, dt, ops.LOG2E if act == ACT_SOFTMAX else 1.0)
    dev = fc.t.device
    q = torch.empty(B, H, Nc, HEAD_DIM, device=dev, dtype=dt)
    ops.gemm(a=fc.t, w=wq, c=q, M=Nc, N=HEAD_DIM, K=HEAD_DIM, compute=dt, lda=C, sa=(Nc * C, HEAD_DIM),
             nb=(B, H), a_mu=mu_c, smu=(C, HEAD_DIM), ldw=HEAD_DIM, sw=(H * HEAD_DIM * HEAD_DIM, HEAD_DIM * HEAD_DIM),
             bias=prep["bf"], sb=(0, HEAD_DIM), ldc=HEAD_DIM, sc=(H * Nc * HEAD_DIM, Nc * HEAD_DIM))
    if not cached and split_attn:
        Ns = fs.t.shape[1]
        img = ops.kv_proj_split3(fs.t, mu_s, wkv, bkv)
        if side is not None:
            side.update(mu_s=mu_s, rstd_s=rstd_s, img=img, Ns=Ns, B=B)
    elif not cached:
        Ns = fs.t.shape[1]
        kv = torch.empty(B, H, Ns, 2 * HEAD_DIM, device=dev, dtype=dt)
        ldt = (Ns + 63) // 64 * 64
        vt = torch.empty(B, H, 2 * HEAD_DIM, ldt, device=dev, dtype=dt)
        ops.gemm(a=fs.t, w=wkv, c=kv, M=Ns, N=2 * HEAD_DIM, K=HEAD_DIM, compute=dt, lda=C, sa=(Ns * C, HEAD_DIM),
                 nb=(B, H), a_mu=mu_s, smu=(C, HEAD_DIM), ldw=HEAD_DIM,
                 sw=(H * 2 * HEAD_DIM * HEAD_DIM, 2 * HEAD_DIM * HEAD_DIM), bias=bkv, sb=(0, 2 * HEAD_DIM),
                 ldc=2 * HEAD_DIM, sc=(H * Ns * 2 * HEAD_DIM, Ns * 2 * HEAD_DIM),
                 vt=vt, ldt=ldt, svt=(H * 2 * HEAD_DIM * ldt, 2 * HEAD_DIM * ldt))
        if act == ACT_COSINE:
            ops.cosine_prep(None, kv)
            mom = ops.cosine_moments(kv, vt)
        if side is not None:
            side.update(mu_s=mu_s, rstd_s=rstd_s, kv=kv, vt=vt, mom=mom, Ns=Ns, B=B)
    if act == ACT_COSINE:
        ops.cosine_prep(q, None)
        with _timed("mhada_attn"):
            att = ops.cosine_attn(q, mom, fcs.t, mu_o, rstd_o, v_mu)
    elif split_attn and ops.F32_SPLIT_OUTPROJ and _split3_fills(B * Nc, C, dev):
        with _timed("mhada_attn"):
            att3 = ops.attn_split3_planes(q, img, Ns, fcs.t, mu_o, rstd_o, v_mu)
        if "w_out_split3" not in prep:
            with torch.no_grad():
                prep["w_out_split3"] = ops.split3_weight(prep["w_out"])
        out = ops.linear_split3(att3, prep["w_out_split3"], prep["b_out"], torch.float32)
        return _Feat(out.view(B, Nc, C), fc.h, fc.w)
    elif split_attn:
        with _timed("mhada_attn"):
            att = ops.attn_split3(q, img, Ns, fcs.t, mu_o, rstd_o, v_mu)
    else:
        with _timed("mhada_attn"):
            att = ops.mhada_attn(q, kv, vt, fcs.t, mu_o, rstd_o, v_mu, act)
    out = torch.empty(B * Nc, C, device=dev, dtype=torch.float32)
    t16 = torch.empty(B * Nc, C, device=dev, dtype=torch.bfloat16) if want_bf16 else None
    ops.gemm(a=att.view(B * Nc, C), w=prep["w_out"], c=out, M=B * Nc, N=C, K=C, compute=dt, lda=C, ldw=C,
             bias=prep["b_out"], ldc=C, c2=t16, ldc2=C)
    f = _Feat(out.view(B, Nc, C), fc.h, fc.w)
    f.t16 = None if t16 is None else t16.view(B, Nc, C)
    return f


def _block_forward_hd(blk, fc: _Feat, fs: Optional[_Feat], fcs: _Feat, dt: torch.dtype,
                      side: Optional[dict], want_bf16: bool) -> _Feat:
    prep = block_prep(blk, dt)
    H, D = blk.num_heads, blk.head_dim
    C = H * D
    B, Nc, Cc = fc.t.shape
    cached = bool(side)
    kv = None
    act = ACT_COSINE if blk.activation_name == "cosine" else ACT_SOFTMAX
    if cached:
        mu_s, rstd_s, kv, Ns = side["mu_s"], side["rstd_s"], side["kv"], side["Ns"]
        if side["B"] != B:
            raise ValueError(f"cached style batch {side['B']} != content batch {B}")
    else:
        if fs.t.shape[2] != C:
            raise ValueError(f"channel mismatch: block expects {C}")
        mu_s, rstd_s = fs.stats()
    if Cc != C or fcs.t.shape[2] != C:
        raise ValueError(f"channel mismatch: block expects {C}")
    mu_c, rstd_c = fc.stats()
    mu_o, rstd_o = fcs.stats()
    wq, wkv, bkv, v_mu = ops.fold_block_hd(prep["wf"], prep["wg"], prep["wh"], prep["bg"], prep["bh"],
                                           rstd_c, mu_s, rstd_s, dt, ops.LOG2E if act == ACT_SOFTMAX else 1.0)
    dev = fc.t.device
    q = torch.empty(B, H, Nc, D, device=dev, dtype=dt)
    ops.gemm(a=fc.t, w=wq, c=q, M=Nc, N=D, K=D, compute=dt, lda=C, sa=(Nc * C, D), nb=(B, H), a_mu=mu_c,
             smu=(C, D), ldw=D, sw=(H * D * D, D * D), bias=prep["bf"], sb=(0, D), ldc=D, sc=(H * Nc * D, Nc * D))
    if not cached:
        Ns = fs.t.shape[1]
        kv = torch.empty(B, H, Ns, 2 * D, device=dev, dtype=dt)
        ops.gemm(a=fs.t, w=wkv, c=kv, M=Ns, N=2 * D, K=D, compute=dt, lda=C, sa=(Ns * C, D), nb=(B, H), a_mu=mu_s,
                 smu=(C, D), ldw=D, sw=(H * 2 * D * D, 2 * D * D), bias=bkv, sb=(0, 2 * D), ldc=2 * D,
                 sc=(H * Ns * 2 * D, Ns * 2 * D))
        if act == ACT_COSINE:
            ops.cosine_prep_hd(None, kv)
        if side is not None:
            side.update(mu_s=mu_s, rstd_s=rstd_s, kv=kv, Ns=Ns, B=B)
    if act == ACT_COSINE:
        ops.cosine_prep_hd(q, None)
    with _timed("mhada_attn"):
        att = ops.attn_hd(q, kv, fcs.t, mu_o, rstd_o, v_mu, act)
    out = torch.empty(B * Nc, C, device=dev, dtype=torch.float32)
    t16 = torch.empty(B * Nc, C, device=dev, dtype=torch.bfloat16) if want_bf16 else None
    ops.gemm(a=att.view(B * Nc, C), w=prep["w_out"], c=out, M=B * Nc, N=C, K=C, compute=dt, lda=C, ldw=C,
             bias=prep["b_out"], ldc=C, c2=t16, ldc2=C)
    f = _Feat(out.view(B, Nc, C), fc.h, fc.w)
    f.t16 = None if t16 is None else t16.view(B, Nc, C)
    return f


def adaattn_prep(blk, dtype):
    def build(dt):
        def w(m):
            return m.weight.reshape(m.weight.shape[0], -1).float()
        qs = ops.LOG2E if dt == torch.bfloat16 else 1.0
        return dict(wf=(w(blk.f) * qs).to(dt).contiguous(), bf=(blk.f.bias.float() * qs).contiguous(),
                    wg=w(blk.g).to(dt).contiguous(), bg=blk.g.bias.float().contiguous(),
                    wh=w(blk.h).to(dt).contiguous(), bh=blk.h.bias.float().contiguous(),
                    wh32=w(blk.h).contiguous())
    return cached_prep(blk, dtype, build)


def adaattn_forward(blk, fc: _Feat, fs: _Feat, fcs: _Feat, dt: torch.dtype, want_bf16: bool = False) -> _Feat:
    C = ops.WIDE_WIDTH
    B, Nc, Cc = fc.t.shape
    if Cc != C or fs.t.shape[2] != C or fcs.t.shape[2] != C or blk.f.weight.shape[0] != C:
        raise ValueError(f"the HIP AdaAttN kernels implement qkv_dim {C}, got channels {Cc} / {fs.t.shape[2]} / "
                         f"{fcs.t.shape[2]} and qkv_dim {blk.f.weight.shape[0]}")
    if fs.t.shape[0] != B or fcs.t.shape[:2] != (B, Nc):
        raise ValueError(f"batch / token mismatch: fc {tuple(fc.t.shape)}, fs {tuple(fs.t.shape)}, fcs {tuple(fcs.t.shape)}")
    Ns = fs.t.shape[1]
    cosine = blk.activation_name == "cosine"
    wide = dt == torch.bfloat16 and not cosine and ops.BF16_WIDE_ATTN
    prep = adaattn_prep(blk, torch.bfloat16 if wide else torch.float32)
    pdt = torch.bfloat16 if wide else torch.float32
    mu_c, rstd_c = fc.stats()
    mu_s, rstd_s = fs.stats()
    mu_o, rstd_o = fcs.stats()
    q = ops.linear(ops.rows_normalize(fc.t, mu_c, rstd_c).view(B * Nc, C), prep["wf"], prep["bf"], pdt).view(B, Nc, C)
    k = ops.linear(ops.rows_normalize(fs.t, mu_s, rstd_s).view(B * Ns, C), prep["wg"], prep["bg"], pdt).view(B, Ns, C)
    if wide:
        v = torch.empty(B, Ns, C, device=fs.t.device, dtype=torch.bfloat16)
        ops.gemm(a=fs.t, w=prep["wh"], c=v, M=Ns, N=C, K=C, compute=torch.bfloat16, lda=C, sa=(Ns * C, 0), nb=(B, 1),
                 a_mu=mu_s, smu=(C, 0), ldw=C, ldc=C, sc=(Ns * C, 0))
        v_mu = ops.linear(mu_s, prep["wh32"], prep["bh"], torch.float32)
        with _timed("mhada_attn"):
            res = ops.attn_wide(q, k, v, fcs.t, mu_o, rstd_o, v_mu, want_bf16=want_bf16)
        out, t16 = res if want_bf16 else (res, None)
    else:
        v = ops.linear(fs.t.view(B * Ns, C), prep["wh"], prep["bh"], torch.float32).view(B, Ns, C)
        if cosine:
            q = q / q.norm(dim=-1, keepdim=True)
            k = k / k.norm(dim=-1, keepdim=True)
        with _timed("mhada_attn"):
            out = ops.loss_attn(q, k, v, fcs.t, mu_o, rstd_o, ACT_COSINE if cosine else ACT_SOFTMAX)
        t16 = None
    f = _Feat(out, fc.h, fc.w)
    f.t16 = t16
    return f


def adaformer1_forward(ada, fc: Sequence[torch.Tensor], fs: Sequence[torch.Tensor]) -> torch.Tensor:
    require_device(fc[0], "AdaAttnTransformer")
    dt = resolve_compute_dtype(ada)
    L = ada.num_layers
    fcf = [_Feat.from_nchw(t) for t in fc[:L]]
    fsf = [_Feat.from_nchw(t) for t in fs[:L]]
    fcs = fcf[0]
    for i in range(L):
        fcs = adaattn_forward(ada.adaAttNs[i], fcf[i], fsf[i], fcs, dt,
                              want_bf16=(dt == torch.bfloat16 and i == L - 1))
    B, N, C = fcs.t.shape
    x16 = None if fcs.t16 is None else fcs.t16.view(B, fcs.h, fcs.w, C)
    return decoder_forward_tokens(ada.decoder, fcs.t.view(B, fcs.h, fcs.w, C), dt, x16=x16)


def style_cache(ada, fs: Sequence[torch.Tensor], dt: torch.dtype):
    if not getattr(ada, "cache_style", True):
        return [None] * len(ada.adaAttnHead), False
    sig = tuple(_signature(b) for b in ada.adaAttnHead)
    vers = tuple(t._version for t in fs)
    mode = (dt, ops.F32_SPLIT_ATTN)
    c = ada.__dict__.get("_mhada_style")
    if (c is not None and c["mode"] == mode and c["sig"] == sig and c["vers"] == vers
            and len(c["refs"]) == len(fs) and all(r() is t for r, t in zip(c["refs"], fs))):
        return c["sides"], True
    sides = [dict() for _ in ada.adaAttnHead]
    ada.__dict__["_mhada_style"] = dict(mode=mode, sig=sig, vers=vers, refs=[weakref.ref(t) for t in fs], sides=sides)
    return sides, False


def decoder_prep(dec, dtype):
    def build(dt):
        mods = dict(dec.named_modules())
        layers = []
        for name, up in DECODER_LAYERS:
            conv = mods[name].conv.conv
            w = conv.weight.permute(0, 2, 3, 1).reshape(conv.weight.shape[0], -1).to(dt).contiguous()
            u = ops.wino_weights(w) if dt == torch.float32 and w.shape[0] % 64 == 0 and (w.shape[1] // 9) % 8 == 0 \
                else None
            layers.append((w, conv.bias.float().contiguous(), up, u))
        last = mods[LAST_LAYER].conv.conv
        return dict(layers=layers, w_last=last.weight.permute(2, 3, 1, 0).float().contiguous(),
                    b_last=last.bias.float().contiguous())
    return cached_prep(dec, dtype, build)


def decoder_forward_tokens(dec, x_nhwc: torch.Tensor, dt: torch.dtype, clamp255: bool = False,
                           x16: Optional[torch.Tensor] = None) -> torch.Tensor:
    prep = decoder_prep(dec, dt)
    x = x16 if (x16 is not None and dt == torch.bfloat16) else x_nhwc
    for w, b, up, u in prep["layers"]:
        if up and not _fuse_upsample(dt, w):
            x = ops.upsample2x(x)
            up = False
        x = ops.conv3x3(x, w, b, dt, upsample=up, relu=True, wino_u=u)
    return ops.conv3x3_out3(x, prep["w_last"], prep["b_last"], clamp255=clamp255)


def adaformer_forward(ada, fc: Sequence[torch.Tensor], fs: Sequence[torch.Tensor]):
    require_device(fc[0], "AdaAttnTransformerMultiHead")
    dt = resolve_compute_dtype(ada)
    L = ada.num_layers
    fcf = [_Feat.from_nchw(t) for t in fc[:L]]
    sides, hit = style_cache(ada, fs[:L], dt)
    fsf = [None] * L if hit else [_Feat.from_nchw(t) for t in fs[:L]]
    fcs = fcf[0]
    for i in range(L):
        fcs = block_forward(ada.adaAttnHead[2 * i], fcf[i], fsf[i], fcs, dt, sides[2 * i])
        fcs = block_forward(ada.adaAttnHead[2 * i + 1], fcs, fsf[i], fcs, dt, sides[2 * i + 1],
                            want_bf16=(dt == torch.bfloat16 and i == L - 1))
    B, N, C = fcs.t.shape
    x16 = None if fcs.t16 is None else fcs.t16.view(B, fcs.h, fcs.w, C)
    cs = decoder_forward_tokens(ada.decoder, fcs.t.view(B, fcs.h, fcs.w, C), dt, x16=x16)
    return tokens_to_nchw(fcs.t, fcs.h, fcs.w), cs
```

### mhada-style-transfer_amd/mhada_hip/ops.py

```python
from __future__ import annotations

import contextlib
import ctypes
import math
from typing import Optional

import torch

from . import _lib
from ._lib import A_CONV3X3, A_CONV3X3_UP2, A_CONV3X3_ZERO, A_PATCH8, A_ROWS, A_SPLIT3, BF16, BF16X3, F32, GemmArgs, GemmTnArgs

_DT = {torch.float32: F32, torch.bfloat16: BF16}


def dt_code(dtype: torch.dtype) -> int:
    try:
        return _DT[dtype]
    except KeyError:
        raise ValueError(f"unsupported dtype {dtype}; the HIP path computes in float32 or bfloat16")


def _ptr(t: Optional[torch.Tensor]) -> Optional[int]:
    return None if t is None else t.data_ptr()


def _need_gpu(*ts: Optional[torch.Tensor]) -> None:
    dev = None
    for t in ts:
        if t is None:
            continue
        if not t.is_cuda:
            raise RuntimeError("mhada_hip ops need ROCm device tensors (the MI355X path has no CPU fallback)")
        if dev is None:
            dev = t.device
        elif t.device != dev:
            raise RuntimeError(f"mhada_hip ops need all operands on one device, got {dev} and {t.device}")


def _call(name: str, dev_tensor: torch.Tensor, *args) -> None:
    idx = dev_tensor.device.index
    guard = contextlib.nullcontext() if idx is None or idx == torch.cuda.current_device() \
        else torch.cuda.device(idx)
    with guard:
        rc = getattr(_lib.load(), name)(*args, torch.cuda.current_stream().cuda_stream)
    _lib.check(rc, name)


def gemm(*, a: torch.Tensor, w: torch.Tensor, c: torch.Tensor, M: int, N: int, K: int,
         compute: torch.dtype, a_mode: int = A_ROWS, lda: int = 0, sa=(0, 0), nb=(1, 1),
         a_mu: Optional[torch.Tensor] = None, smu=(0, 0), img=(0, 0, 0),
         ldw: int = 0, sw=(0, 0), bias: Optional[torch.Tensor] = None, sb=(0, 0),
         r: Optional[torch.Tensor] = None, ldr: int = 0, sr=(0, 0),
         ldc: int = 0, sc=(0, 0), relu: bool = False, pad: int = 0,
         c2: Optional[torch.Tensor] = None, ldc2: int = 0, sc2=(0, 0),
         vt: Optional[torch.Tensor] = None, ldt: int = 0, svt=(0, 0), c2_planes: bool = False,
         col_scale: Optional[torch.Tensor] = None, out_scale: Optional[torch.Tensor] = None) -> torch.Tensor:
    _need_gpu(a, w, c, a_mu, bias, r, c2, vt, col_scale, out_scale)
    half2 = col_scale is not None
    if half2 and (a.dtype != torch.float16 or col_scale.dtype != torch.float32 or col_scale.numel() < N):
        raise ValueError("col_scale (fp32 [N]) goes with fp16 HALF2 operands")
    h2out = out_scale is not None
    if h2out and (not half2 or c2 is None or c2.dtype != torch.float16 or c2_planes
                  or out_scale.dtype != torch.float32 or out_scale.numel() < N):
        raise ValueError("out_scale (fp32 [N]) goes with col_scale and an fp16 c2 [2][M][ldc2]")
    if c is None and not c2_planes and not h2out:
        raise ValueError("gemm: C may be None only with c2_planes")
    if c2 is not None and ((c2.dtype != torch.bfloat16 and not h2out) or (c is not None and c.dtype != torch.float32)):
        raise ValueError("c2 is the bf16 copy of an fp32 C")
    if c2_planes and (c2 is None or c2.shape[0] != 3 or not c2.is_contiguous()):
        raise ValueError("c2_planes needs c2 = contiguous bf16 [3][M][ldc2]")
    if vt is not None and vt.dtype != c.dtype:
        raise ValueError("vt has the dtype of C")
    if w.dtype != compute:
        raise ValueError("W must already be in the compute dtype")
    for t in (a_mu, bias):
        if t is not None and t.dtype != torch.float32:
            raise ValueError("a_mu / bias must be float32")
    if r is not None and r.dtype != (c.dtype if c is not None else torch.float32):
        raise ValueError("residual dtype must equal the output dtype (fp32 for a c2_planes-only output)")
    args = GemmArgs()
    args.M, args.N, args.K = M, N, K
    args.nb1, args.nb2 = nb
    args.compute = BF16 if half2 else dt_code(compute)
    args.a_mode = a_mode
    args.a, args.a_dtype, args.lda = a.data_ptr(), BF16 if half2 else dt_code(a.dtype), lda
    args.sa1, args.sa2 = sa
    args.a_mu = _ptr(a_mu)
    args.smu1, args.smu2 = smu
    args.img_c, args.img_h, args.img_w = img
    args.w, args.ldw = w.data_ptr(), ldw
    args.sw1, args.sw2 = sw
    args.bias = _ptr(bias)
    args.sb1, args.sb2 = sb
    args.r = _ptr(r)
    args.r_dtype = dt_code(r.dtype) if r is not None else 0
    args.ldr = ldr
    args.sr1, args.sr2 = sr
    args.c, args.c_dtype, args.ldc = _ptr(c), dt_code(c.dtype) if c is not None else F32, ldc
    args.sc1, args.sc2 = sc
    args.relu = int(relu)
    args.pad = int(pad)
    args.c2, args.ldc2 = _ptr(c2), ldc2
    args.sc21, args.sc22 = sc2
    args.vt, args.ldt = _ptr(vt), ldt
    args.svt1, args.svt2 = svt
    args.c2_planes = int(c2_planes)
    if h2out:
        _call("mhada_gemm_half2_planes", a, ctypes.byref(args), col_scale.data_ptr(), out_scale.data_ptr())
    elif half2:
        _call("mhada_gemm_half2", a, ctypes.byref(args), col_scale.data_ptr())
    else:
        _call("mhada_gemm", a, ctypes.byref(args))
    return c if c is not None else c2


def linear(x: torch.Tensor, w: torch.Tensor, bias: Optional[torch.Tensor], out_dtype: torch.dtype,
           residual: Optional[torch.Tensor] = None, relu: bool = False,
           relu_mask: Optional[torch.Tensor] = None) -> torch.Tensor:
    M, K = x.shape
    N = w.shape[0]
    c = torch.empty(M, N, device=x.device, dtype=out_dtype)
    if relu_mask is not None:
        if residual is not None or relu or out_dtype != torch.float32 or relu_mask.dtype != torch.float32 \
                or relu_mask.shape != (M, N) or not relu_mask.is_contiguous():
            raise ValueError("linear: relu_mask needs fp32 output, a contiguous fp32 [M][N] mask, no residual / relu")
        return gemm(a=x, w=w, c=c, M=M, N=N, K=K, compute=w.dtype, lda=x.stride(0), ldw=w.stride(0),
                    bias=bias, r=relu_mask, ldr=N, ldc=N, relu=2)
    return gemm(a=x, w=w, c=c, M=M, N=N, K=K, compute=w.dtype, lda=x.stride(0), ldw=w.stride(0),
                bias=bias, r=residual, ldr=N if residual is not None else 0, ldc=N, relu=relu)


def patch_embed(img: torch.Tensor, w: torch.Tensor, bias: torch.Tensor, pos: Optional[torch.Tensor],
                patch: int = 8) -> torch.Tensor:
    if patch != 8:
        raise ValueError("the HIP patch embedding implements patch_size=8 (the reference default)")
    B, Ci, H, W = img.shape
    h, wd = H // 8, W // 8
    N, C = h * wd, w.shape[0]
    out = torch.empty(B, N, C, device=img.device, dtype=torch.float32)
    return gemm(a=img, w=w, c=out, M=N, N=C, K=Ci * 64, compute=w.dtype, a_mode=A_PATCH8,
                sa=(Ci * H * W, 0), nb=(B, 1), img=(Ci, H, W), ldw=w.stride(0), bias=bias,
                r=pos, ldr=C, sr=(0, 0), ldc=C, sc=(N * C, 0))


def patch_embed_dgrad(dy: torch.Tensor, w: torch.Tensor, H: int, W: int,
                      out: Optional[torch.Tensor] = None) -> torch.Tensor:
    _need_gpu(dy, w, out)
    for t, what in ((dy, "dy"), (w, "w"), (out, "out")):
        if t is not None and (t.dtype != torch.float32 or not t.is_contiguous()):
            raise ValueError(f"patch_embed_dgrad: {what} must be contiguous float32")
    if dy.dim() != 3 or w.dim() not in (2, 4) or w.shape[0] != dy.shape[2] or (w.dim() == 4 and w.shape[2:] != (8, 8)) \
            or (w.dim() == 2 and w.shape[1] % 64):
        raise ValueError(f"patch_embed_dgrad: dy [B][N][C] and w (C, Ci, 8, 8) or [C][64 Ci], got "
                         f"{tuple(dy.shape)} and {tuple(w.shape)}")
    B, N, C = dy.shape
    Ci = w.shape[1] if w.dim() == 4 else w.shape[1] // 64
    if H < 8 or W < 8 or N != (H // 8) * (W // 8):
        raise ValueError(f"patch_embed_dgrad: {N} token rows do not match a {H} x {W} image")
    if out is None:
        out =(torch.zeros if H % 8 else torch.empty)(B, Ci, H, W, device=dy.device, dtype=torch.float32)
    elif out.shape != (B, Ci, H, W):
        raise ValueError(f"patch_embed_dgrad: out must be {(B, Ci, H, W)}, got {tuple(out.shape)}")
    _call("mhada_patch_embed_dgrad", dy, dy.data_ptr(), w.data_ptr(), out.data_ptr(), B, C, Ci, H, W)
    return out


WINO = True


def wino_eligible(x: torch.Tensor, w: torch.Tensor, upsample: bool) -> bool:
    return (WINO and w.dtype == torch.float32 and x.dtype == torch.float32 and not upsample
            and x.shape[-1] % 8 == 0 and w.shape[0] % 64 == 0 and x.shape[1] >= 2 and x.shape[2] >= 2
            and x.numel() < 2 ** 31 and x.numel() // x.shape[-1] * w.shape[0] < 2 ** 31)


WINO_WGRAD = True


def wgrad_wino_eligible(x: torch.Tensor, g: torch.Tensor, cout: int) -> bool:
    if not (WINO_WGRAD and x.is_cuda and x.dtype == torch.float32 and g.dtype == torch.float32):
        return False
    B, H, W, ci = x.shape
    return (ci % 64 == 0 and cout % 64 == 0 and H % 2 == 0 and W % 16 == 0 and g.shape[:3] == x.shape[:3]
            and g.shape[3] >= cout and g.shape[3] % 4 == 0 and x.is_contiguous() and g.is_contiguous()
            and B * H * W * max(ci, g.shape[3]) < 2 ** 31)


def conv3x3_wgrad_wino(x: torch.Tensor, g: torch.Tensor, cout: int, pad_mode: str = "reflect",
                       bias: bool = True):
    _need_gpu(x, g)
    B, H, W, ci = x.shape
    lib = _lib.load()
    S = lib.mhada_conv3x3_wgrad_wino_splits(B, H, W, ci, cout)
    if S <= 0:
        raise ValueError("conv3x3_wgrad_wino: ineligible shape")
    work = torch.empty(S * (16 * cout * ci + (cout if bias else 0)), device=x.device, dtype=torch.float32)
    dw = torch.empty(cout, 9 * ci, device=x.device, dtype=torch.float32)
    db = torch.empty(cout, device=x.device, dtype=torch.float32) if bias else None
    _call("mhada_conv3x3_wgrad_wino", x, x.data_ptr(), g.data_ptr(), dw.data_ptr(),
          db.data_ptr() if bias else None, work.data_ptr(), work.numel(), B, H, W, ci, cout, g.shape[3],
          _lib.PAD_REFLECT if pad_mode == "reflect" else _lib.PAD_ZERO)
    return dw, db


def wino_weights_split3(w: torch.Tensor) -> torch.Tensor:
    _need_gpu(w)
    Co, K = w.shape
    Ci = K // 9
    if w.dtype != torch.float32 or K != 9 * Ci or Ci % 16 or not w.is_contiguous():
        raise ValueError("wino_weights_split3 needs a contiguous fp32 [Cout][9*Cin] weight, Cin % 16 == 0")
    up = torch.empty(Ci // 16, 16, 3, Co, 16, device=w.device, dtype=torch.bfloat16)
    _call("mhada_wino_weights_split3", w, w.data_ptr(), up.data_ptr(), Co, Ci)
    return up


def wino_weights(w: torch.Tensor) -> torch.Tensor:
    _need_gpu(w)
    Co, K = w.shape
    Ci = K // 9
    if w.dtype != torch.float32 or K != 9 * Ci or not w.is_contiguous():
        raise ValueError("wino_weights needs a contiguous fp32 [Cout][9*Cin] weight")
    u = torch.empty(Ci // 8, 16, Co, 8, device=w.device, dtype=torch.float32)
    _call("mhada_wino_weights", w, w.data_ptr(), u.data_ptr(), Co, Ci)
    if Ci % 16 == 0:
        u.split3 = wino_weights_split3(w)
    return u


def conv3x3_wino(x: torch.Tensor, u: torch.Tensor, bias: Optional[torch.Tensor], relu: bool = True,
                 pad_mode: str = "reflect", pad: int = 1, out: Optional[torch.Tensor] = None,
                 relu_mask: Optional[torch.Tensor] = None) -> torch.Tensor:
    _need_gpu(x, u, bias, out, relu_mask)
    B, H, W, Ci = x.shape
    Co = u.shape[2]
    if x.dtype != torch.float32 or not x.is_contiguous() or u.shape[0] * 8 != Ci:
        raise ValueError("conv3x3_wino: contiguous fp32 NHWC input matching the filters")
    if pad_mode == "reflect":
        mode, Ho, Wo, pad = _lib.PAD_REFLECT, H, W, 1
    elif pad_mode == "zero":
        mode, Ho, Wo = _lib.PAD_ZERO, H + 2 * (pad - 1), W + 2 * (pad - 1)
    else:
        raise ValueError(f"pad_mode {pad_mode!r}")
    y = torch.empty(B, Ho, Wo, Co, device=x.device, dtype=torch.float32) if out is None else out
    if y.shape[:3] != (B, Ho, Wo) or y.dtype != torch.float32 or y.shape[-1] < Co or not y.is_contiguous():
        raise ValueError("conv3x3_wino: bad output buffer")
    if relu_mask is not None and (relu_mask.shape != y.shape or relu_mask.dtype != torch.float32
                                  or not relu_mask.is_contiguous()):
        raise ValueError("conv3x3_wino: relu_mask must be a contiguous fp32 tensor shaped like the output")
    up = getattr(u, "split3", None)
    if up is not None:
        _call("mhada_conv3x3_wino_split3", x, x.data_ptr(), u.data_ptr(), up.data_ptr(), _ptr(bias), y.data_ptr(),
              B, H, W, Ci, Co, y.shape[-1], mode, pad, int(relu), _ptr(relu_mask))
    else:
        _call("mhada_conv3x3_wino", x, x.data_ptr(), u.data_ptr(), _ptr(bias), y.data_ptr(), B, H, W, Ci, Co,
              y.shape[-1], mode, pad, int(relu), _ptr(relu_mask))
    return y


def conv3x3(x: torch.Tensor, w: torch.Tensor, bias: Optional[torch.Tensor], out_dtype: torch.dtype,
            upsample: bool, relu: bool = True, pad_mode: str = "reflect", pad: int = 1,
            out: Optional[torch.Tensor] = None, wino_u: Optional[torch.Tensor] = None,
            relu_mask: Optional[torch.Tensor] = None) -> torch.Tensor:
    B, H, W, Ci = x.shape
    Co = w.shape[0]
    if out_dtype == torch.float32 and wino_eligible(x, w, upsample) and x.is_contiguous():
        u = wino_u if wino_u is not None else wino_weights(w)
        return conv3x3_wino(x, u, bias, relu, pad_mode, pad, out, relu_mask)
    if relu_mask is not None:
        return relu_bwd(conv3x3(x, w, bias, out_dtype, upsample, relu, pad_mode, pad, out), relu_mask)
    if pad_mode == "zero":
        if upsample:
            raise ValueError("zero-padded conv3x3 has no fused upsample")
        Ho, Wo = H + 2 * (pad - 1), W + 2 * (pad - 1)
        mode = A_CONV3X3_ZERO
    elif pad_mode == "reflect":
        Ho, Wo = (2 * H, 2 * W) if upsample else (H, W)
        mode = A_CONV3X3_UP2 if upsample else A_CONV3X3
        pad = 0
    else:
        raise ValueError(f"pad_mode {pad_mode!r}")
    y = torch.empty(B, Ho, Wo, Co, device=x.device, dtype=out_dtype) if out is None else out
    return gemm(a=x, w=w, c=y, M=B * Ho * Wo, N=Co, K=9 * Ci, compute=w.dtype, a_mode=mode, img=(Ci, H, W),
                ldw=w.stride(0), bias=bias, ldc=y.shape[-1], relu=relu, pad=pad)


def upsample2x(x: torch.Tensor) -> torch.Tensor:
    _need_gpu(x)
    B, H, W, C = x.shape
    y = torch.empty(B, 2 * H, 2 * W, C, device=x.device, dtype=x.dtype)
    _call("mhada_upsample2x", x, x.data_ptr(), y.data_ptr(), dt_code(x.dtype), B, H, W, C)
    return y


def conv3x3_out3(x: torch.Tensor, w: torch.Tensor, bias: torch.Tensor, clamp255: bool = False) -> torch.Tensor:
    B, H, W, Ci = x.shape
    _need_gpu(x, w, bias)
    y = torch.empty(B, 3, H, W, device=x.device, dtype=torch.float32)
    _call("mhada_conv3x3_out3", x, x.data_ptr(), dt_code(x.dtype), w.data_ptr(), bias.data_ptr(),
                                        y.data_ptr(), B, H, W, Ci, int(clamp255))
    return y


def layernorm(x: torch.Tensor, g: torch.Tensor, b: torch.Tensor, out_dtype: torch.dtype, eps: float) -> torch.Tensor:
    _need_gpu(x, g, b)
    rows, cols = x.shape
    y = torch.empty(rows, cols, device=x.device, dtype=out_dtype)
    _call("mhada_layernorm", x, x.data_ptr(), y.data_ptr(), dt_code(out_dtype), g.data_ptr(), b.data_ptr(),
                                     rows, cols, eps)
    return y


F32_SPLIT = True


F32_SPLIT_OUTPROJ = True


def layernorm_split3(x: torch.Tensor, g: torch.Tensor, b: torch.Tensor, eps: float) -> torch.Tensor:
    _need_gpu(x, g, b)
    rows, cols = x.shape
    y = torch.empty(3, rows, cols, device=x.device, dtype=torch.bfloat16)
    _call("mhada_layernorm", x, x.data_ptr(), y.data_ptr(), BF16X3, g.data_ptr(), b.data_ptr(), rows, cols, eps)
    return y


def split3_weight(w: torch.Tensor) -> torch.Tensor:
    w = w.float()
    N, K0 = w.shape
    if K0 % 64:
        raise ValueError("split3_weight: K0 must be a multiple of 64")
    q0 = w.bfloat16()
    r = w - q0.float()
    q1 = r.bfloat16()
    q2 = (r - q1.float()).bfloat16()
    terms = torch.stack([t.view(N, K0 // 64, 64) for t in (q1, q0, q2, q0, q1, q0)], dim=2)
    return terms.reshape(N, 6 * K0).contiguous()


def split3_weight_dev(w: torch.Tensor, transposed: bool = False) -> torch.Tensor:
    _need_gpu(w)
    if w.dtype != torch.float32 or not w.is_contiguous() or w.dim() != 2:
        raise ValueError("split3_weight_dev needs a contiguous float32 matrix")
    N, K0 = (w.shape[1], w.shape[0]) if transposed else w.shape
    if K0 % 64:
        raise ValueError("split3_weight_dev: K0 must be a multiple of 64")
    out = torch.empty(N, 6 * K0, device=w.device, dtype=torch.bfloat16)
    _call("mhada_split3_weight", w, w.data_ptr(), out.data_ptr(), N, K0, int(transposed))
    return out


def split3_rows(x: torch.Tensor) -> torch.Tensor:
    _need_gpu(x)
    if x.dtype != torch.float32 or not x.is_contiguous() or x.dim() != 2:
        raise ValueError("split3_rows needs a contiguous float32 [M][K0] matrix")
    y = torch.empty(3, *x.shape, device=x.device, dtype=torch.bfloat16)
    _call("mhada_split3_rows", x, x.data_ptr(), y.data_ptr(), x.numel())
    return y


def linear_split3(planes: torch.Tensor, w6: torch.Tensor, bias: Optional[torch.Tensor], out_dtype: torch.dtype,
                  residual: Optional[torch.Tensor] = None, relu: bool = False,
                  out_planes: bool = False, relu_mask: Optional[torch.Tensor] = None, both: bool = False):
    if planes.dim() != 3 or planes.shape[0] != 3 or planes.dtype != torch.bfloat16 or not planes.is_contiguous():
        raise ValueError("linear_split3: planes must be contiguous bf16 [3][M][K0]")
    _, M, K0 = planes.shape
    N = w6.shape[0]
    if w6.dtype != torch.bfloat16 or w6.shape[1] != 6 * K0:
        raise ValueError("linear_split3: w6 must be split3_weight(w), bf16 [N][6*K0]")
    if out_planes:
        if out_dtype != torch.float32:
            raise ValueError("linear_split3: out_planes splits an fp32 result")
        c2 = torch.empty(3, M, N, device=planes.device, dtype=torch.bfloat16)
        return gemm(a=planes, w=w6, c=None, M=M, N=N, K=6 * K0, compute=torch.bfloat16, a_mode=A_SPLIT3, lda=K0,
                    ldw=6 * K0, bias=bias, r=residual, ldr=N if residual is not None else 0, ldc=N, relu=relu,
                    c2=c2, ldc2=N, c2_planes=True)
    c = torch.empty(M, N, device=planes.device, dtype=out_dtype)
    c2 = None
    if both:
        if out_dtype != torch.float32:
            raise ValueError("linear_split3: both splits an fp32 result")
        c2 = torch.empty(3, M, N, device=planes.device, dtype=torch.bfloat16)
    if relu_mask is not None:
        if residual is not None or relu or out_dtype != torch.float32 or relu_mask.dtype != torch.float32 \
                or relu_mask.shape != (M, N) or not relu_mask.is_contiguous():
            raise ValueError("linear_split3: relu_mask needs fp32 output, a contiguous fp32 [M][N] mask, no residual / relu")
        gemm(a=planes, w=w6, c=c, M=M, N=N, K=6 * K0, compute=torch.bfloat16, a_mode=A_SPLIT3, lda=K0,
             ldw=6 * K0, bias=bias, r=relu_mask, ldr=N, ldc=N, relu=2, c2=c2, ldc2=N if both else 0, c2_planes=both)
    else:
        gemm(a=planes, w=w6, c=c, M=M, N=N, K=6 * K0, compute=torch.bfloat16, a_mode=A_SPLIT3, lda=K0,
             ldw=6 * K0, bias=bias, r=residual, ldr=N if residual is not None else 0, ldc=N, relu=relu,
             c2=c2, ldc2=N if both else 0, c2_planes=both)
    return (c, c2) if both else c


F32_HALF2 = True

_H2_MIN = 2.0 ** -14
_H2_SCALE_WINDOW = (2.0 ** -40, 2.0 ** 40)


def _half2_planes(v: torch.Tensor):
    hi = v.half()
    hi = torch.where(hi.abs() < _H2_MIN, torch.zeros_like(hi), hi)
    lo = (v - hi.float()).half()
    lo = torch.where(lo.abs() < _H2_MIN, torch.zeros_like(lo), lo)
    return hi, lo


def half2_a_scale(gamma: torch.Tensor, beta: torch.Tensor) -> Optional[float]:
    Y = math.sqrt(gamma.numel()) * float(gamma.detach().abs().max()) + float(beta.detach().abs().max())
    if not math.isfinite(Y) or Y <= 0.0:
        return None
    q = 32768.0 / Y
    if not math.isfinite(q) or q <= 0.0:
        return None
    s_a = 2.0 ** (math.frexp(q)[1] - 1)
    return s_a if _H2_SCALE_WINDOW[0] <= s_a <= _H2_SCALE_WINDOW[1] else None


def half2_weight(w: torch.Tensor):
    w = w.float()
    N, K0 = w.shape
    if K0 % 64:
        raise ValueError("half2_weight: K0 must be a multiple of 64")
    m = w.abs().amax(dim=1)
    ok = torch.isfinite(m) & (m > 0)
    e = torch.frexp(torch.where(ok, m, torch.ones_like(m)))[1]
    t = ((127 + torch.clamp(15 - e, max=127)).to(torch.int32) << 23).view(torch.float32)
    t = torch.where(ok, t, torch.ones_like(m))
    hi, lo = _half2_planes(w * t[:, None])
    w2 = torch.stack([p.view(N, K0 // 64, 64) for p in (hi, lo)], dim=2)
    return w2.reshape(N, 2 * K0).contiguous(), t


def half2_weight_dev(w: torch.Tensor):
    _need_gpu(w)
    if w.dtype != torch.float32 or not w.is_contiguous() or w.dim() != 2 or w.shape[1] % 64:
        raise ValueError("half2_weight_dev needs a contiguous float32 [N][K0] matrix, K0 % 64 == 0")
    N, K0 = w.shape
    w2 = torch.empty(N, 2 * K0, device=w.device, dtype=torch.float16)
    t = torch.empty(N, device=w.device, dtype=torch.float32)
    _call("mhada_half2_weight", w, w.data_ptr(), w2.data_ptr(), t.data_ptr(), N, K0)
    return w2, t


def half2_prepare(gamma: torch.Tensor, beta: torch.Tensor, w: torch.Tensor) -> Optional[dict]:
    s_a = half2_a_scale(gamma, beta)
    if s_a is None or w.shape[1] % 64 or not bool(torch.isfinite(w).all()):
        return None
    w2, t = half2_weight_dev(w.float().contiguous()) if w.is_cuda else half2_weight(w)
    lo, hi = _H2_SCALE_WINDOW
    if float(t.min()) < lo or float(t.max()) > hi:
        return None
    return dict(s_a=s_a, w2=w2, cs=(1.0 / (s_a * t.double())).float().contiguous())


def layernorm_half2(x: torch.Tensor, g: torch.Tensor, b: torch.Tensor, eps: float, s_a: float) -> torch.Tensor:
    _need_gpu(x, g, b)
    rows, cols = x.shape
    y = torch.empty(2, rows, cols, device=x.device, dtype=torch.float16)
    _call("mhada_layernorm_half2", x, x.data_ptr(), y.data_ptr(), g.data_ptr(), b.data_ptr(), rows, cols, eps, s_a)
    return y


def linear_half2(planes: torch.Tensor, w2: torch.Tensor, cs: torch.Tensor, bias: Optional[torch.Tensor],
                 out_dtype: torch.dtype, residual: Optional[torch.Tensor] = None, relu: bool = False,
                 out_planes: bool = False, out_scale: Optional[torch.Tensor] = None):
    if planes.dim() != 3 or planes.shape[0] != 2 or planes.dtype != torch.float16 or not planes.is_contiguous():
        raise ValueError("linear_half2: planes must be contiguous fp16 [2][M][K0]")
    _, M, K0 = planes.shape
    N = w2.shape[0]
    if w2.dtype != torch.float16 or w2.shape[1] != 2 * K0 or not w2.is_contiguous():
        raise ValueError("linear_half2: w2 must be half2_weight(w), fp16 [N][2*K0]")
    kw = dict(a=planes, w=w2, M=M, N=N, K=K0, compute=torch.float16, lda=K0, ldw=2 * K0, bias=bias, r=residual,
              ldr=N if residual is not None else 0, ldc=N, relu=relu, col_scale=cs)
    if out_planes:
        if out_dtype != torch.float32:
            raise ValueError("linear_half2: out_planes splits an fp32 result")
        if out_scale is not None:
            c2 = torch.empty(2, M, N, device=planes.device, dtype=torch.float16)
            return gemm(c=None, c2=c2, ldc2=N, out_scale=out_scale, **kw)
        c2 = torch.empty(3, M, N, device=planes.device, dtype=torch.bfloat16)
        return gemm(c=None, c2=c2, ldc2=N, c2_planes=True, **kw)
    if out_scale is not None:
        raise ValueError("linear_half2: out_scale goes with out_planes")
    return gemm(c=torch.empty(M, N, device=planes.device, dtype=out_dtype), **kw)


F32_HALF2_CHAIN = True
F32_HALF2_CHAIN_OUTPROJ = False


def half2_chain_bound(gamma: torch.Tensor, beta: torch.Tensor, w: torch.Tensor, b: Optional[torch.Tensor]):
    g, be, W = gamma.detach().double(), beta.detach().double(), w.detach().double()
    off = W @ be
    if b is not None:
        off = off + b.detach().double()
    return math.sqrt(g.numel()) * (W * g[None, :]).norm(dim=1) + off.abs()


def half2_out_scale(Z: torch.Tensor) -> Optional[torch.Tensor]:
    Z = Z.detach().double()
    if not bool((torch.isfinite(Z) & (Z > 0)).all()):
        return None
    q = 32768.0 / Z
    if not bool((torch.isfinite(q) & (q > 0)).all()):
        return None
    e = torch.frexp(q)[1] - 1
    if int(e.min()) < -40 or int(e.max()) > 40:
        return None
    return ((127 + e).to(torch.int32) << 23).view(torch.float32)


def half2_chain_prepare(gamma: torch.Tensor, beta: torch.Tensor, w_p: torch.Tensor, b_p: Optional[torch.Tensor],
                        w_c: torch.Tensor) -> Optional[dict]:
    ts = [t for t in (gamma, beta, w_p, b_p, w_c) if t is not None]
    if w_c.shape[1] % 64 or w_c.shape[1] != w_p.shape[0] or not all(bool(torch.isfinite(t).all()) for t in ts):
        return None
    u = half2_out_scale(half2_chain_bound(gamma, beta, w_p, b_p))
    if u is None:
        return None
    lo, hi = _H2_SCALE_WINDOW
    wu = (w_c.detach().float() / u.to(w_c.device)[None, :]).contiguous()
    m = wu.abs().amax(dim=1)
    if not bool(torch.isfinite(m).all()) or float(m.min()) < lo or float(m.max()) > hi:
        return None
    w2, t = half2_weight_dev(wu) if wu.is_cuda else half2_weight(wu)
    if float(t.min()) < lo or float(t.max()) > hi:
        return None
    return dict(u=u.to(w_c.device).contiguous(), w2=w2, cs=(1.0 / t.double()).float().contiguous())


def linear_half2_planes(planes: torch.Tensor, w2: torch.Tensor, cs: torch.Tensor, bias: Optional[torch.Tensor],
                        residual: Optional[torch.Tensor] = None) -> torch.Tensor:
    if planes.dim() != 3 or planes.shape[0] != 2 or planes.dtype != torch.float16 or not planes.is_contiguous():
        raise ValueError("linear_half2_planes: planes must be contiguous fp16 [2][M][K0]")
    _, M, K0 = planes.shape
    N = w2.shape[0]
    if w2.dtype != torch.float16 or w2.shape[1] != 2 * K0 or not w2.is_contiguous():
        raise ValueError("linear_half2_planes: w2 must be half2_weight(w / u), fp16 [N][2*K0]")
    return gemm(a=planes, w=w2, c=torch.empty(M, N, device=planes.device, dtype=torch.float32), M=M, N=N, K=K0,
                compute=torch.float16, lda=K0, ldw=2 * K0, bias=bias, r=residual,
                ldr=N if residual is not None else 0, ldc=N, col_scale=cs)


def vit_batch_attn(qkv: torch.Tensor, L: int, ntok: int, heads: int, groups: int = 1) -> torch.Tensor:
    _need_gpu(qkv)
    C = qkv.shape[-1] // 3
    if L % groups:
        raise ValueError("vit_batch_attn: L must be a multiple of groups")
    out = torch.empty(L, ntok, C, device=qkv.device, dtype=qkv.dtype)
    Lg, es = L // groups, qkv.element_size()
    for g in range(groups):
        _call("mhada_vit_batch_attn", qkv, qkv.data_ptr() + g * Lg * ntok * 3 * C * es,
              out.data_ptr() + g * Lg * ntok * C * es, dt_code(qkv.dtype), Lg, ntok, heads, C // heads)
    return out


VIT_ATTN_SPLIT3_MAX_L = 8


def vit_batch_attn_split3(qkv: torch.Tensor, L: int, ntok: int, heads: int) -> torch.Tensor:
    _need_gpu(qkv)
    if qkv.dtype != torch.float32 or not qkv.is_contiguous():
        raise ValueError("vit_batch_attn_split3 needs contiguous float32 qkv")
    C = qkv.shape[-1] // 3
    planes = torch.empty(3, L * ntok, C, device=qkv.device, dtype=torch.bfloat16)
    _call("mhada_vit_batch_attn_split3", qkv, qkv.data_ptr(), planes.data_ptr(), L * ntok * C, L, ntok, heads,
          C // heads)
    return planes


def vit_batch_attn_half2(qkv: torch.Tensor, L: int, ntok: int, heads: int, out_scale: torch.Tensor) -> torch.Tensor:
    _need_gpu(qkv, out_scale)
    C = qkv.shape[-1] // 3
    if qkv.dtype != torch.float32 or not qkv.is_contiguous():
        raise ValueError("vit_batch_attn_half2 needs contiguous float32 qkv")
    if out_scale.dtype != torch.float32 or out_scale.numel() != C or not out_scale.is_contiguous():
        raise ValueError("vit_batch_attn_half2: out_scale must be contiguous float32 [C]")
    planes = torch.empty(2, L * ntok, C, device=qkv.device, dtype=torch.float16)
    _call("mhada_vit_batch_attn_half2", qkv, qkv.data_ptr(), planes.data_ptr(), L * ntok * C, out_scale.data_ptr(),
          L, ntok, heads, C // heads)
    return planes


def pos_embed(pos: torch.Tensor, oh: int, ow: int) -> torch.Tensor:
    _need_gpu(pos)
    _, C, bh, bw = pos.shape
    out = torch.empty(oh * ow, C, device=pos.device, dtype=torch.float32)
    _call("mhada_pos_embed", pos, pos.data_ptr(), out.data_ptr(), C, bh, bw, oh, ow)
    return out


def pos_embed_bwd(g: torch.Tensor, bh: int, bw: int) -> torch.Tensor:
    _need_gpu(g)
    oh, ow, C = g.shape
    if g.dtype != torch.float32 or not g.is_contiguous():
        raise ValueError("pos_embed_bwd needs a contiguous float32 [oh][ow][C] gradient")
    out = torch.empty(1, C, bh, bw, device=g.device, dtype=torch.float32)
    _call("mhada_pos_embed_bwd", g, g.data_ptr(), out.data_ptr(), C, bh, bw, oh, ow)
    return out


def instnorm_bwd(dy: torch.Tensor, y: torch.Tensor, rs: torch.Tensor) -> torch.Tensor:
    _need_gpu(dy, y, rs)
    for t in (dy, y, rs):
        if t.dtype != torch.float32 or not t.is_contiguous():
            raise ValueError("instnorm_bwd needs contiguous float32 operands")
    B, N, C = y.shape
    if dy.shape != y.shape or rs.shape != (B, C):
        raise ValueError("instnorm_bwd: shape mismatch")
    splits = max(1, min(N // 32, 2048 // max(1, B * ((C + 63) // 64))))
    work = torch.empty(splits * B * C * 2 + B * C, device=y.device, dtype=torch.float64)
    dx = torch.empty_like(y)
    _call("mhada_instnorm_bwd", y, dy.data_ptr(), y.data_ptr(), rs.data_ptr(), dx.data_ptr(), work.data_ptr(), B, N, C,
          splits)
    return dx


def attn_train_bwd_prep(dout: torch.Tensor, x: torch.Tensor, mo: torch.Tensor):
    _rows64(dout, x, mo)
    BH, Nc, _ = x.shape
    if dout.shape != x.shape or mo.shape != (BH, Nc, 128):
        raise ValueError("attn_train_bwd_prep: bad shapes")
    dx = torch.empty_like(x)
    dmo = torch.empty_like(mo)
    dd = torch.empty(BH, Nc, device=x.device, dtype=torch.float32)
    _call("mhada_attn_train_bwd_prep", x, dout.data_ptr(), x.data_ptr(), mo.data_ptr(), dx.data_ptr(), dmo.data_ptr(),
          dd.data_ptr(), BH * Nc)
    return dx, dmo, dd


def attn_train_bwd_prep_hd(dout: torch.Tensor, x: torch.Tensor, mo: torch.Tensor):
    _rows64(dout, x, mo)
    D = _train_hd_width("attn_train_bwd_prep_hd", x)
    BH, Nc, _ = x.shape
    if dout.shape != x.shape or mo.shape != (BH, Nc, 2 * D):
        raise ValueError("attn_train_bwd_prep_hd: bad shapes")
    dx = torch.empty_like(x)
    dmo = torch.empty_like(mo)
    dd = torch.empty(BH, Nc, device=x.device, dtype=torch.float32)
    _call("mhada_attn_train_bwd_prep_hd", x, dout.data_ptr(), x.data_ptr(), mo.data_ptr(), dx.data_ptr(),
          dmo.data_ptr(), dd.data_ptr(), BH * Nc, D)
    return dx, dmo, dd


def layernorm_fwd(x: torch.Tensor, gamma: torch.Tensor, beta: torch.Tensor, eps: float, planes: bool = False):
    _need_gpu(x, gamma, beta)
    for t in (x, gamma, beta):
        if t.dtype != torch.float32 or not t.is_contiguous():
            raise ValueError("layernorm_fwd needs contiguous float32 operands")
    M, C = x.shape
    y = torch.empty_like(x)
    st = torch.empty(M, 2, device=x.device, dtype=torch.float32)
    if planes:
        pl = torch.empty(3, M, C, device=x.device, dtype=torch.bfloat16)
        _call("mhada_layernorm_fwd_split3", x, x.data_ptr(), y.data_ptr(), pl.data_ptr(), st.data_ptr(),
              gamma.data_ptr(), beta.data_ptr(), M, C, float(eps))
        return y, st, pl
    _call("mhada_layernorm_fwd", x, x.data_ptr(), y.data_ptr(), st.data_ptr(), gamma.data_ptr(), beta.data_ptr(),
          M, C, float(eps))
    return y, st


def layernorm_bwd(x: torch.Tensor, dy: torch.Tensor, st: torch.Tensor, gamma: torch.Tensor):
    _need_gpu(x, dy, st, gamma)
    for t in (x, dy, st, gamma):
        if t.dtype != torch.float32 or not t.is_contiguous():
            raise ValueError("layernorm_bwd needs contiguous float32 operands")
    M, C = x.shape
    dx = torch.empty_like(x)
    dg = torch.empty(C, device=x.device, dtype=torch.float32)
    db = torch.empty(C, device=x.device, dtype=torch.float32)
    nw = ((M + 127) // 128 * 2 + 2) * C
    work = torch.empty(nw, device=x.device, dtype=torch.float32)
    _call("mhada_layernorm_bwd", x, x.data_ptr(), dy.data_ptr(), st.data_ptr(), gamma.data_ptr(), dx.data_ptr(),
          dg.data_ptr(), db.data_ptr(), work.data_ptr(), nw, M, C)
    return dx, dg, db


def instnorm_stats(x: torch.Tensor, eps: float = 1e-5):
    _need_gpu(x)
    if x.dtype != torch.float32 or not x.is_contiguous() or x.dim() != 3:
        raise ValueError(f"instnorm_stats needs contiguous float32 token rows [B][N][C], got {x.dtype} "
                         f"{tuple(x.shape)}")
    B, N, C = x.shape
    splits = max(1, min(N // 32, 2048 // max(1, B * ((C + 63) // 64))))
    mu = torch.empty(B, C, device=x.device, dtype=torch.float32)
    rstd = torch.empty(B, C, device=x.device, dtype=torch.float32)
    work = torch.empty(splits, B, C, 2, device=x.device, dtype=torch.float64)
    _call("mhada_instnorm_stats", x, x.data_ptr(), mu.data_ptr(), rstd.data_ptr(), work.data_ptr(), B, N, C,
                                          splits, eps)
    return mu, rstd


LOG2E = 1.4426950408889634


def fold_block(wf, wg, wh, bg, bh, rstd_c, mu_s, rstd_s, dtype: torch.dtype, kscale: float = LOG2E):
    B, C = rstd_c.shape
    H = wf.shape[0]
    dev = wf.device
    wq = torch.empty(B, H, 64, 64, device=dev, dtype=dtype)
    wkv = torch.empty(B, H, 128, 64, device=dev, dtype=dtype)
    bkv = torch.empty(H, 128, device=dev, dtype=torch.float32)
    v_mu = torch.empty(B, C, device=dev, dtype=torch.float32)
    _need_gpu(wf, wg, wh, bg, bh, rstd_c, mu_s, rstd_s)
    _call("mhada_fold_block", wf, wf.data_ptr(), wg.data_ptr(), wh.data_ptr(), bg.data_ptr(), bh.data_ptr(),
          rstd_c.data_ptr(), mu_s.data_ptr(), rstd_s.data_ptr(), wq.data_ptr(), wkv.data_ptr(), bkv.data_ptr(),
          v_mu.data_ptr(), kscale, dt_code(dtype), B, H)
    return wq, wkv, bkv, v_mu


def transpose_v(kv: torch.Tensor) -> torch.Tensor:
    _need_gpu(kv)
    B, H, Ns, _ = kv.shape
    ldt = (Ns + 63) // 64 * 64
    vt = torch.empty(B, H, 128, ldt, device=kv.device, dtype=kv.dtype)
    _call("mhada_transpose_v", kv, kv.data_ptr(), vt.data_ptr(), dt_code(kv.dtype), B, H, Ns)
    return vt


def cosine_prep(q: Optional[torch.Tensor], kv: Optional[torch.Tensor]) -> None:
    _need_gpu(q, kv)
    ref = q if q is not None else kv
    B, H = ref.shape[0], ref.shape[1]
    Nc = q.shape[2] if q is not None else 0
    Ns = kv.shape[2] if kv is not None else 0
    _call("mhada_cosine_prep", ref, _ptr(q), _ptr(kv), dt_code(ref.dtype), B, H, Nc, Ns)


def cosine_moments(kv: torch.Tensor, vt: torch.Tensor) -> torch.Tensor:
    _need_gpu(kv, vt)
    B, H, Ns, _ = kv.shape
    if vt.shape != (B, H, 128, (Ns + 63) // 64 * 64) or vt.dtype != kv.dtype:
        raise ValueError(f"cosine_moments: vt {tuple(vt.shape)} does not match kv {tuple(kv.shape)}")
    splits = max(1, min((Ns + 63) // 64, -(-512 // (B * H))))
    mom = torch.empty(B, H, 65, 132, device=kv.device, dtype=torch.float32)
    work = torch.empty(splits, B * H * 65 * 132, device=kv.device, dtype=torch.float32) if splits > 1 else None
    _call("mhada_cosine_moments", kv, kv.data_ptr(), vt.data_ptr(), dt_code(kv.dtype), B, H, Ns, mom.data_ptr(),
          _ptr(work), splits)
    return mom


def cosine_attn(q, mom, fcs, fcs_mu, fcs_rstd, v_mu) -> torch.Tensor:
    _need_gpu(q, mom, fcs, fcs_mu, fcs_rstd, v_mu)
    B, H, Nc, _ = q.shape
    if mom.shape != (B, H, 65, 132) or mom.dtype != torch.float32:
        raise ValueError(f"cosine_attn: mom {tuple(mom.shape)} does not match q {tuple(q.shape)}")
    out = torch.empty(B, Nc, H * 64, device=q.device, dtype=q.dtype)
    _call("mhada_cosine_attn", q, q.data_ptr(), mom.data_ptr(), fcs.data_ptr(), fcs_mu.data_ptr(),
          fcs_rstd.data_ptr(), v_mu.data_ptr(), out.data_ptr(), dt_code(q.dtype), B, H, Nc)
    return out


def mhada_attn(q, kv, vt, fcs, fcs_mu, fcs_rstd, v_mu, activation: int) -> torch.Tensor:
    _need_gpu(q, kv, vt, fcs, fcs_mu, fcs_rstd, v_mu)
    B, H, Nc, _ = q.shape
    Ns = kv.shape[2]
    out = torch.empty(B, Nc, H * 64, device=q.device, dtype=q.dtype)
    _call("mhada_attn", q, q.data_ptr(), kv.data_ptr(), _ptr(vt), fcs.data_ptr(), fcs_mu.data_ptr(),
                                fcs_rstd.data_ptr(), v_mu.data_ptr(), out.data_ptr(), dt_code(q.dtype), B, H, Nc,
                                Ns, activation)
    return out


HD_WIDTHS = (32, 128)


def _hd_width(what: str, D: int) -> None:
    if D not in HD_WIDTHS:
        raise ValueError(f"{what}: head width must be 32 or 128 (64 has its own entry point), got {D}")


def fold_block_hd(wf, wg, wh, bg, bh, rstd_c, mu_s, rstd_s, dtype: torch.dtype, kscale: float = LOG2E):
    _need_gpu(wf, wg, wh, bg, bh, rstd_c, mu_s, rstd_s)
    B, C = rstd_c.shape
    H, D = wf.shape[0], wf.shape[1]
    _hd_width("fold_block_hd", D)
    for t, shape in ((wf, (H, D, D)), (wg, (H, D, D)), (wh, (H, D, D)), (bg, (H, D)), (bh, (H, D)),
                     (rstd_c, (B, H * D)), (mu_s, (B, H * D)), (rstd_s, (B, H * D))):
        if tuple(t.shape) != shape or t.dtype != torch.float32 or not t.is_contiguous():
            raise ValueError(f"fold_block_hd: needs contiguous fp32 {shape}, got {tuple(t.shape)} {t.dtype}")
    dt_code(dtype)
    dev = wf.device
    wq = torch.empty(B, H, D, D, device=dev, dtype=dtype)
    wkv = torch.empty(B, H, 2 * D, D, device=dev, dtype=dtype)
    bkv = torch.empty(H, 2 * D, device=dev, dtype=torch.float32)
    v_mu = torch.empty(B, C, device=dev, dtype=torch.float32)
    _call("mhada_fold_block_hd", wf, wf.data_ptr(), wg.data_ptr(), wh.data_ptr(), bg.data_ptr(), bh.data_ptr(),
          rstd_c.data_ptr(), mu_s.data_ptr(), rstd_s.data_ptr(), wq.data_ptr(), wkv.data_ptr(), bkv.data_ptr(),
          v_mu.data_ptr(), kscale, dt_code(dtype), B, H, D)
    return wq, wkv, bkv, v_mu


def cosine_prep_hd(q: Optional[torch.Tensor], kv: Optional[torch.Tensor]) -> None:
    _need_gpu(q, kv)
    if q is None and kv is None:
        raise ValueError("cosine_prep_hd: needs q or kv")
    ref = q if q is not None else kv
    D = q.shape[-1] if q is not None else kv.shape[-1] // 2
    _hd_width("cosine_prep_hd", D)
    for t, w in ((q, D), (kv, 2 * D)):
        if t is not None and (t.dim() != 4 or t.shape[-1] != w or t.dtype != ref.dtype or not t.is_contiguous()
                              or t.shape[:2] != ref.shape[:2]):
            raise ValueError(f"cosine_prep_hd: needs contiguous q [B][H][Nc][{D}] / kv [B][H][Ns][{2 * D}] of one "
                             f"dtype, got {tuple(t.shape)} {t.dtype}")
    B, H = ref.shape[0], ref.shape[1]
    Nc = q.shape[2] if q is not None else 0
    Ns = kv.shape[2] if kv is not None else 0
    if Nc == 0 and Ns == 0:
        return
    _call("mhada_cosine_prep_hd", ref, _ptr(q) if Nc else None, _ptr(kv) if Ns else None, dt_code(ref.dtype), B, H,
          D, Nc, Ns)


def attn_hd(q, kv, fcs, fcs_mu, fcs_rstd, v_mu, activation: int) -> torch.Tensor:
    _need_gpu(q, kv, fcs, fcs_mu, fcs_rstd, v_mu)
    if q.dim() != 4 or kv.dim() != 4:
        raise ValueError(f"attn_hd: needs q [B][H][Nc][D] and kv [B][H][Ns][2D], got {tuple(q.shape)} / {tuple(kv.shape)}")
    B, H, Nc, D = q.shape
    Ns = kv.shape[2]
    _hd_width("attn_hd", D)
    C = H * D
    if kv.shape != (B, H, Ns, 2 * D) or kv.dtype != q.dtype or not q.is_contiguous() or not kv.is_contiguous():
        raise ValueError(f"attn_hd: needs contiguous q [B][H][Nc][{D}] and kv [B][H][Ns][{2 * D}] of one dtype, got "
                         f"{tuple(q.shape)} {q.dtype} / {tuple(kv.shape)} {kv.dtype}")
    if Nc <= 0 or Ns <= 0:
        raise ValueError(f"attn_hd: needs Nc > 0 and Ns > 0, got {Nc} / {Ns}")
    for t, shape in ((fcs, (B, Nc, C)), (fcs_mu, (B, C)), (fcs_rstd, (B, C)), (v_mu, (B, C))):
        if tuple(t.shape) != shape or t.dtype != torch.float32 or not t.is_contiguous():
            raise ValueError(f"attn_hd: needs contiguous fp32 {shape}, got {tuple(t.shape)} {t.dtype}")
    out = torch.empty(B, Nc, C, device=q.device, dtype=q.dtype)
    _call("mhada_attn_hd", q, q.data_ptr(), kv.data_ptr(), fcs.data_ptr(), fcs_mu.data_ptr(), fcs_rstd.data_ptr(),
          v_mu.data_ptr(), out.data_ptr(), dt_code(q.dtype), B, H, D, Nc, Ns, activation)
    return out


WIDE_WIDTH = 512
BF16_WIDE_ATTN = True


def attn_wide(q, k, v, fcs, fcs_mu, fcs_rstd, v_mu, want_bf16: bool = False):
    _need_gpu(q, k, v, fcs, fcs_mu, fcs_rstd, v_mu)
    if q.dim() != 3 or k.dim() != 3 or v.dim() != 3:
        raise ValueError(f"attn_wide: needs q [B][Nc][{WIDE_WIDTH}], k and v [B][Ns][{WIDE_WIDTH}], got "
                         f"{tuple(q.shape)} / {tuple(k.shape)} / {tuple(v.shape)}")
    B, Nc, D = q.shape
    Ns = k.shape[1]
    if D != WIDE_WIDTH:
        raise ValueError(f"attn_wide: head width must be {WIDE_WIDTH}, got {D}")
    if k.shape != (B, Ns, D) or v.shape != (B, Ns, D):
        raise ValueError(f"attn_wide: needs k and v [B][Ns][{D}] matching q, got {tuple(q.shape)} / {tuple(k.shape)} / "
                         f"{tuple(v.shape)}")
    for t in (q, k, v):
        if t.dtype != torch.bfloat16 or not t.is_contiguous():
            raise ValueError(f"attn_wide: q, k, v must be contiguous bfloat16, got {t.dtype}")
    if Nc <= 0 or Ns <= 0:
        raise ValueError(f"attn_wide: needs Nc > 0 and Ns > 0, got {Nc} / {Ns}")
    for t, shape in ((fcs, (B, Nc, D)), (fcs_mu, (B, D)), (fcs_rstd, (B, D)), (v_mu, (B, D))):
        if tuple(t.shape) != shape or t.dtype != torch.float32 or not t.is_contiguous():
            raise ValueError(f"attn_wide: needs contiguous fp32 {shape}, got {tuple(t.shape)} {t.dtype}")
    out = torch.empty(B, Nc, D, device=q.device, dtype=torch.float32)
    out16 = torch.empty(B, Nc, D, device=q.device, dtype=torch.bfloat16) if want_bf16 else None
    _call("mhada_attn_wide", q, q.data_ptr(), k.data_ptr(), v.data_ptr(), fcs.data_ptr(), fcs_mu.data_ptr(),
          fcs_rstd.data_ptr(), v_mu.data_ptr(), out.data_ptr(), _ptr(out16), BF16, B, Nc, Ns, D)
    return (out, out16) if want_bf16 else out


F32_SPLIT_ATTN = True


def split3_kv(kv: torch.Tensor, vt: torch.Tensor) -> torch.Tensor:
    _need_gpu(kv, vt)
    B, H, Ns, _ = kv.shape
    ldt = (Ns + 63) // 64 * 64
    if kv.dtype != torch.float32 or vt.dtype != torch.float32 or vt.shape != (B, H, 128, ldt) \
            or kv.shape[3] != 128 or not kv.is_contiguous() or not vt.is_contiguous():
        raise ValueError(f"split3_kv: needs contiguous fp32 kv [B][H][Ns][128] and vt [B][H][128][{ldt}], "
                         f"got {tuple(kv.shape)} / {tuple(vt.shape)}")
    img = torch.empty(B, H, 576 * ldt, device=kv.device, dtype=torch.bfloat16)
    _call("mhada_split3_kv", kv, kv.data_ptr(), vt.data_ptr(), img.data_ptr(), B, H, Ns)
    return img


def kv_proj_split3(fs: torch.Tensor, mu_s: torch.Tensor, wkv: torch.Tensor, bkv: torch.Tensor) -> torch.Tensor:
    _need_gpu(fs, mu_s, wkv, bkv)
    B, Ns, C = fs.shape
    H = C // 64
    for t in (fs, mu_s, wkv, bkv):
        if t.dtype != torch.float32 or not t.is_contiguous():
            raise ValueError("kv_proj_split3 needs contiguous float32 operands")
    if C % 64 or mu_s.shape != (B, C) or wkv.shape != (B, H, 128, 64) or bkv.shape != (H, 128):
        raise ValueError(f"kv_proj_split3: bad shapes fs {tuple(fs.shape)} mu {tuple(mu_s.shape)} "
                         f"wkv {tuple(wkv.shape)} bkv {tuple(bkv.shape)}")
    ldt = (Ns + 63) // 64 * 64
    img = torch.empty(B, H, 576 * ldt, device=fs.device, dtype=torch.bfloat16)
    _call("mhada_kv_proj_split3", fs, fs.data_ptr(), mu_s.data_ptr(), wkv.data_ptr(), bkv.data_ptr(), img.data_ptr(),
          B, H, Ns)
    return img


def attn_split3(q, img, Ns: int, fcs, fcs_mu, fcs_rstd, v_mu) -> torch.Tensor:
    _need_gpu(q, img, fcs, fcs_mu, fcs_rstd, v_mu)
    B, H, Nc, _ = q.shape
    ldt = (Ns + 63) // 64 * 64
    if q.dtype != torch.float32 or not q.is_contiguous() or img.dtype != torch.bfloat16 \
            or img.shape != (B, H, 576 * ldt):
        raise ValueError(f"attn_split3: q must be contiguous fp32 and img bf16 [B][H][576*{ldt}], got "
                         f"{q.dtype} / {tuple(img.shape)}")
    out = torch.empty(B, Nc, H * 64, device=q.device, dtype=torch.float32)
    _call("mhada_attn_split3", q, q.data_ptr(), img.data_ptr(), fcs.data_ptr(), fcs_mu.data_ptr(),
          fcs_rstd.data_ptr(), v_mu.data_ptr(), out.data_ptr(), B, H, Nc, Ns)
    return out


def attn_split3_planes(q, img, Ns: int, fcs, fcs_mu, fcs_rstd, v_mu) -> torch.Tensor:
    _need_gpu(q, img, fcs, fcs_mu, fcs_rstd, v_mu)
    B, H, Nc, _ = q.shape
    ldt = (Ns + 63) // 64 * 64
    if q.dtype != torch.float32 or not q.is_contiguous() or img.dtype != torch.bfloat16 \
            or img.shape != (B, H, 576 * ldt):
        raise ValueError(f"attn_split3_planes: q must be contiguous fp32 and img bf16 [B][H][576*{ldt}], got "
                         f"{q.dtype} / {tuple(img.shape)}")
    planes = torch.empty(3, B * Nc, H * 64, device=q.device, dtype=torch.bfloat16)
    _call("mhada_attn_split3_planes", q, q.data_ptr(), img.data_ptr(), fcs.data_ptr(), fcs_mu.data_ptr(),
          fcs_rstd.data_ptr(), v_mu.data_ptr(), planes.data_ptr(), B, H, Nc, Ns)
    return planes


def _rows64(*ts: torch.Tensor) -> None:
    _need_gpu(*ts)
    for t in ts:
        if t.dtype != torch.float32 or not t.is_contiguous():
            raise ValueError("training attention operands must be contiguous float32")


def attn_train_fwd(q: torch.Tensor, k: torch.Tensor, v: torch.Tensor, x: torch.Tensor):
    _rows64(q, k, v, x)
    BH, Nc, d = q.shape
    Ns = k.shape[1]
    if d != 64 or k.shape != (BH, Ns, 64) or v.shape != k.shape or x.shape != q.shape:
        raise ValueError(f"attn_train_fwd: bad shapes q{tuple(q.shape)} k{tuple(k.shape)} v{tuple(v.shape)} "
                         f"x{tuple(x.shape)}")
    out = torch.empty_like(q)
    mo = torch.empty(BH, Nc, 128, device=q.device, dtype=torch.float32)
    lse = torch.empty(BH, Nc, device=q.device, dtype=torch.float32)
    if TRAIN_FWD_S3:
        img = torch.empty(BH, 576 * ((Ns + 63) // 64 * 64), device=q.device, dtype=torch.bfloat16)
        _call("mhada_attn_train_fwd_split3", q, q.data_ptr(), k.data_ptr(), v.data_ptr(), img.data_ptr(), x.data_ptr(),
              out.data_ptr(), mo.data_ptr(), lse.data_ptr(), BH, Nc, Ns)
    elif TRAIN_FWD_VT:
        vt = torch.empty(BH, 128, (Ns + 63) // 64 * 64, device=q.device, dtype=torch.float32)
        _call("mhada_attn_train_fwd_vt", q, q.data_ptr(), k.data_ptr(), v.data_ptr(), vt.data_ptr(), x.data_ptr(),
              out.data_ptr(), mo.data_ptr(), lse.data_ptr(), BH, Nc, Ns)
    else:
        _call("mhada_attn_train_fwd", q, q.data_ptr(), k.data_ptr(), v.data_ptr(), x.data_ptr(), out.data_ptr(),
              mo.data_ptr(), lse.data_ptr(), BH, Nc, Ns)
    return out, mo, lse


TRAIN_FWD_S3 = True
TRAIN_FWD_VT = True


DS_SPILL_BYTES = 16 << 30
DS_SPILL_MAX_ROWS = 0x7fff0000 // 4
BWD_PATH_COUNTS = {"spill": 0, "recompute": 0}


def ds_spill_eligible(BH: int, Nc: int, Ns: int) -> bool:
    return Ns % 4 == 0 and 4 * BH * Nc * Ns <= DS_SPILL_BYTES and (Nc + 32) * Ns <= DS_SPILL_MAX_ROWS


def transpose64(x: torch.Tensor) -> torch.Tensor:
    _need_gpu(x)
    if x.dtype != torch.float32 or x.dim() != 3 or x.shape[-1] != 64:
        raise ValueError("transpose64: fp32 [BH][N][64]")
    x = x.contiguous()
    BH, N, _ = x.shape
    ldt = (N + 63) // 64 * 64
    out = torch.empty(BH, 64, ldt, device=x.device, dtype=torch.float32)
    _call("mhada_transpose64", x, x.data_ptr(), out.data_ptr(), BH, N, ldt)
    return out


def attn_train_bwd(q, k, v, lse, dmo, dd, spill: Optional[bool] = None):
    _rows64(q, k, v, lse, dmo, dd)
    BH, Nc, _ = q.shape
    Ns = k.shape[1]
    if lse.shape != (BH, Nc) or dmo.shape != (BH, Nc, 128) or dd.shape != (BH, Nc) or k.shape != (BH, Ns, 64) \
            or v.shape != k.shape:
        raise ValueError("attn_train_bwd: bad shapes")
    auto = spill is None
    if auto:
        spill = ds_spill_eligible(BH, Nc, Ns)
    ds = None
    if spill:
        try:
            ds = torch.empty(BH, Nc, Ns, device=q.device, dtype=torch.float32)
        except torch.cuda.OutOfMemoryError:
            if not auto:
                raise
            spill = False
    BWD_PATH_COUNTS["spill" if spill else "recompute"] += 1
    dq = torch.empty_like(q)
    dk = torch.empty_like(k)
    dv = torch.empty_like(v)
    if not spill:
        _call("mhada_attn_train_bwd", q, q.data_ptr(), k.data_ptr(), v.data_ptr(), lse.data_ptr(), dmo.data_ptr(),
              dd.data_ptr(), dq.data_ptr(), dk.data_ptr(), dv.data_ptr(), BH, Nc, Ns)
        return dq, dk, dv
    if Ns % 4:
        raise ValueError("attn_train_bwd: the dS spill needs Ns % 4 == 0")
    _call("mhada_attn_train_dkv", q, q.data_ptr(), k.data_ptr(), v.data_ptr(), lse.data_ptr(), dmo.data_ptr(),
          dd.data_ptr(), dk.data_ptr(), dv.data_ptr(), ds.data_ptr(), BH, Nc, Ns)
    if TRAIN_DQ_S3 and Ns % 32 == 0:
        ldt = (Ns + 63) // 64 * 64
        gemm_n64_split3(ds, transpose64_split3(k), dq, BH, Nc, Ns, ldt)
    else:
        kt = transpose64(k)
        ldt = kt.shape[-1]
        gemm(a=ds, w=kt, c=dq, M=Nc, N=64, K=Ns, compute=torch.float32, lda=Ns, sa=(Nc * Ns, 0), nb=(BH, 1),
             ldw=ldt, sw=(64 * ldt, 0), ldc=64, sc=(Nc * 64, 0))
    return dq, dk, dv


DQ_ONLY_COUNTS = {"dq_only": 0}


def attn_train_dq(q, k, v, lse, dmo, dd):
    _rows64(q, k, v, lse, dmo, dd)
    BH, Nc, _ = q.shape
    Ns = k.shape[1]
    if lse.shape != (BH, Nc) or dmo.shape != (BH, Nc, 128) or dd.shape != (BH, Nc) or k.shape != (BH, Ns, 64) \
            or v.shape != k.shape:
        raise ValueError("attn_train_dq: bad shapes")
    DQ_ONLY_COUNTS["dq_only"] += 1
    dq = torch.empty_like(q)
    _call("mhada_attn_train_dq", q, q.data_ptr(), k.data_ptr(), v.data_ptr(), lse.data_ptr(), dmo.data_ptr(),
          dd.data_ptr(), dq.data_ptr(), BH, Nc, Ns)
    return dq


def _train_hd_width(what: str, t: torch.Tensor) -> int:
    D = t.shape[-1] if t.dim() == 3 else -1
    if D not in (32, 128):
        raise ValueError(f"{what}: rows of 32 or 128 floats (64: the op without _hd), got {tuple(t.shape)}")
    return D


def attn_train_fwd_hd(q: torch.Tensor, k: torch.Tensor, v: torch.Tensor, x: torch.Tensor):
    _rows64(q, k, v, x)
    D = _train_hd_width("attn_train_fwd_hd", q)
    BH, Nc, _ = q.shape
    Ns = k.shape[1] if k.dim() == 3 else -1
    if k.shape != (BH, Ns, D) or v.shape != k.shape or x.shape != q.shape or Ns <= 0:
        raise ValueError(f"attn_train_fwd_hd: bad shapes q{tuple(q.shape)} k{tuple(k.shape)} v{tuple(v.shape)} "
                         f"x{tuple(x.shape)}")
    out = torch.empty_like(q)
    mo = torch.empty(BH, Nc, 2 * D, device=q.device, dtype=torch.float32)
    lse = torch.empty(BH, Nc, device=q.device, dtype=torch.float32)
    _call("mhada_attn_train_fwd_hd", q, q.data_ptr(), k.data_ptr(), v.data_ptr(), x.data_ptr(), out.data_ptr(),
          mo.data_ptr(), lse.data_ptr(), BH, D, Nc, Ns)
    return out, mo, lse


def attn_train_bwd_hd(q, k, v, lse, dmo, dd):
    _rows64(q, k, v, lse, dmo, dd)
    D = _train_hd_width("attn_train_bwd_hd", q)
    BH, Nc, _ = q.shape
    Ns = k.shape[1] if k.dim() == 3 else -1
    if lse.shape != (BH, Nc) or dmo.shape != (BH, Nc, 2 * D) or dd.shape != (BH, Nc) or k.shape != (BH, Ns, D) \
            or v.shape != k.shape or Ns <= 0:
        raise ValueError("attn_train_bwd_hd: bad shapes")
    dq = torch.empty_like(q)
    dk = torch.empty_like(k)
    dv = torch.empty_like(v)
    _call("mhada_attn_train_bwd_hd", q, q.data_ptr(), k.data_ptr(), v.data_ptr(), lse.data_ptr(), dmo.data_ptr(),
          dd.data_ptr(), dq.data_ptr(), dk.data_ptr(), dv.data_ptr(), BH, D, Nc, Ns)
    return dq, dk, dv


def attn_train_dq_hd(q, k, v, lse, dmo, dd):
    _rows64(q, k, v, lse, dmo, dd)
    D = _train_hd_width("attn_train_dq_hd", q)
    BH, Nc, _ = q.shape
    Ns = k.shape[1] if k.dim() == 3 else -1
    if lse.shape != (BH, Nc) or dmo.shape != (BH, Nc, 2 * D) or dd.shape != (BH, Nc) or k.shape != (BH, Ns, D) \
            or v.shape != k.shape or Ns <= 0:
        raise ValueError("attn_train_dq_hd: bad shapes")
    DQ_ONLY_COUNTS["dq_only"] += 1
    dq = torch.empty_like(q)
    _call("mhada_attn_train_dq_hd", q, q.data_ptr(), k.data_ptr(), v.data_ptr(), lse.data_ptr(), dmo.data_ptr(),
          dd.data_ptr(), dq.data_ptr(), BH, D, Nc, Ns)
    return dq


BF16_TRAIN_COUNTS = {"fwd": 0, "bwd": 0}


def _bf16_workspace(q: torch.Tensor, BH: int, Nc: int, Ns: int, backward: bool) -> torch.Tensor:
    n = _lib.load().mhada_attn_train_bf16_workspace(BH, Nc, Ns, int(backward))
    if n < 0:
        raise ValueError("attn_train_bf16: bad sizes")
    return torch.empty(max(n, 16), device=q.device, dtype=torch.uint8)


def attn_train_fwd_bf16(q: torch.Tensor, k: torch.Tensor, v: torch.Tensor, x: torch.Tensor):
    _rows64(q, k, v, x)
    BH, Nc, d = q.shape if q.dim() == 3 else (0, 0, 0)
    Ns = k.shape[1] if k.dim() == 3 else -1
    if d != 64 or k.shape != (BH, Ns, 64) or v.shape != k.shape or x.shape != q.shape or Ns <= 0:
        raise ValueError(f"attn_train_fwd_bf16: bad shapes q{tuple(q.shape)} k{tuple(k.shape)} v{tuple(v.shape)} "
                         f"x{tuple(x.shape)}")
    out = torch.empty_like(q)
    mo = torch.empty(BH, Nc, 128, device=q.device, dtype=torch.float32)
    lse = torch.empty(BH, Nc, device=q.device, dtype=torch.float32)
    ws = _bf16_workspace(q, BH, Nc, Ns, False)
    BF16_TRAIN_COUNTS["fwd"] += 1
    _call("mhada_attn_train_fwd_bf16", q, q.data_ptr(), k.data_ptr(), v.data_ptr(), x.data_ptr(), out.data_ptr(),
          mo.data_ptr(), lse.data_ptr(), ws.data_ptr(), ws.numel(), BH, Nc, Ns)
    return out, mo, lse


def attn_train_bwd_bf16_prepass(q, k, v, dmo, mo) -> torch.Tensor:
    _rows64(q, k, v, dmo, mo)
    BH, Nc, d = q.shape if q.dim() == 3 else (0, 0, 0)
    Ns = k.shape[1] if k.dim() == 3 else -1
    if d != 64 or dmo.shape != (BH, Nc, 128) or mo.shape != dmo.shape or k.shape != (BH, Ns, 64) \
            or v.shape != k.shape or Ns <= 0:
        raise ValueError("attn_train_bwd_bf16: bad shapes")
    ws = _bf16_workspace(q, BH, Nc, Ns, True)
    _call("mhada_attn_train_bwd_bf16", q, q.data_ptr(), k.data_ptr(), v.data_ptr(), None, dmo.data_ptr(),
          mo.data_ptr(), None, None, None, ws.data_ptr(), ws.numel(), BH, Nc, Ns, 1)
    return ws


def attn_train_bwd_bf16_run(q, k, v, lse, ws: torch.Tensor):
    _rows64(q, k, v, lse)
    _need_gpu(ws)
    BH, Nc, d = q.shape if q.dim() == 3 else (0, 0, 0)
    Ns = k.shape[1] if k.dim() == 3 else -1
    if d != 64 or lse.shape != (BH, Nc) or k.shape != (BH, Ns, 64) or v.shape != k.shape or Ns <= 0 \
            or ws.dtype != torch.uint8:
        raise ValueError("attn_train_bwd_bf16: bad shapes")
    dq = torch.empty_like(q)
    dk = torch.empty_like(k)
    dv = torch.empty_like(v)
    BF16_TRAIN_COUNTS["bwd"] += 1
    _call("mhada_attn_train_bwd_bf16", q, q.data_ptr(), k.data_ptr(), v.data_ptr(), lse.data_ptr(), None, None,
          dq.data_ptr(), dk.data_ptr(), dv.data_ptr(), ws.data_ptr(), ws.numel(), BH, Nc, Ns, 2)
    return dq, dk, dv


def attn_train_bwd_bf16(q, k, v, lse, dmo, mo):
    _rows64(lse)
    return attn_train_bwd_bf16_run(q, k, v, lse, attn_train_bwd_bf16_prepass(q, k, v, dmo, mo))


TRAIN_DQ_S3 = True


def transpose64_split3(k: torch.Tensor) -> torch.Tensor:
    _need_gpu(k)
    if k.dtype != torch.float32 or k.dim() != 3 or k.shape[-1] != 64:
        raise ValueError("transpose64_split3: fp32 [BH][N][64]")
    k = k.contiguous()
    BH, N, _ = k.shape
    ldt = (N + 63) // 64 * 64
    out = torch.empty(3, BH * 64, ldt, device=k.device, dtype=torch.bfloat16)
    _call("mhada_transpose64_split3", k, k.data_ptr(), out.data_ptr(), BH, N, ldt)
    return out


def gemm_n64_split3(ds: torch.Tensor, kt_planes: torch.Tensor, dq: torch.Tensor, BH: int, Nc: int, Ns: int,
                    ldt: int):
    if ds.dtype != torch.float32 or not ds.is_contiguous() or ds.shape != (BH, Nc, Ns):
        raise ValueError("gemm_n64_split3: ds must be contiguous float32 [BH][Nc][Ns]")
    if kt_planes.dtype != torch.bfloat16 or kt_planes.shape != (3, BH * 64, ldt) or not kt_planes.is_contiguous():
        raise ValueError("gemm_n64_split3: kt_planes must be contiguous bf16 [3][BH*64][ldt]")
    if dq.dtype != torch.float32 or not dq.is_contiguous() or dq.shape != (BH, Nc, 64):
        raise ValueError("gemm_n64_split3: dq must be contiguous float32 [BH][Nc][64]")
    _call("mhada_gemm_n64_split3", ds, ds.data_ptr(), kt_planes.data_ptr(), dq.data_ptr(), BH, Nc, Ns, Ns, Nc * Ns,
          ldt, 64 * ldt, BH * 64 * ldt, 64, Nc * 64)


_PADDING = {"zeros": 0, "border": 1}


def _padding_code(padding_mode: str) -> int:
    try:
        return _PADDING[padding_mode]
    except KeyError:
        raise ValueError(f"padding_mode {padding_mode!r}: the HIP warp implements 'zeros' and 'border'")


def _f32c(t: torch.Tensor, what: str) -> torch.Tensor:
    if t.dtype != torch.float32:
        raise ValueError(f"{what} must be float32")
    return t.contiguous()


def warp(x: torch.Tensor, flow: torch.Tensor, padding_mode: str = "zeros") -> torch.Tensor:
    _need_gpu(x, flow)
    x, flow = _f32c(x, "x"), _f32c(flow, "flow")
    B, C, H, W = x.shape
    if tuple(flow.shape) != (B, 2, H, W):
        raise ValueError(f"flow must be [B,2,H,W] = {[B, 2, H, W]}, got {list(flow.shape)}")
    y = torch.empty_like(x)
    _call("mhada_warp", x, x.data_ptr(), flow.data_ptr(), y.data_ptr(), B, C, H, W,
                                _padding_code(padding_mode))
    return y


def warp_bwd(gy: torch.Tensor, flow: torch.Tensor, padding_mode: str = "zeros") -> torch.Tensor:
    _need_gpu(gy, flow)
    gy, flow = _f32c(gy, "gy"), _f32c(flow, "flow")
    B, C, H, W = gy.shape
    if tuple(flow.shape) != (B, 2, H, W):
        raise ValueError(f"flow must be [B,2,H,W] = {[B, 2, H, W]}, got {list(flow.shape)}")
    gx = torch.zeros_like(gy)
    _call("mhada_warp_bwd", gy, gy.data_ptr(), flow.data_ptr(), gx.data_ptr(), B, C, H, W, _padding_code(padding_mode))
    return gx


def flow_warp_mask(flo01: torch.Tensor, flo10: torch.Tensor, padding_mode: str = "zeros",
                   threshold: float = 2) -> torch.Tensor:
    _need_gpu(flo01, flo10)
    flo01, flo10 = _f32c(flo01, "flo01"), _f32c(flo10, "flo10")
    if flo01.dim() != 3 or flo01.shape[0] != 2 or flo01.shape != flo10.shape:
        raise ValueError("flows must both be [2,H,W]")
    H, W = flo01.shape[1:]
    mask = torch.empty(H, W, device=flo01.device, dtype=torch.float32)
    _call("mhada_flow_warp_mask", flo01, flo01.data_ptr(), flo10.data_ptr(), mask.data_ptr(), H, W,
                                          float(threshold), _padding_code(padding_mode))
    return mask


def warp_l1(cs1: torch.Tensor, cs2: torch.Tensor, flow: torch.Tensor, mask: torch.Tensor) -> torch.Tensor:
    _need_gpu(cs1, cs2, flow, mask)
    cs1, cs2, flow, mask = (_f32c(t, n) for t, n in ((cs1, "cs1"), (cs2, "cs2"), (flow, "flow"), (mask, "mask")))
    B, C, H, W = cs1.shape
    if cs2.shape != cs1.shape or tuple(flow.shape) != (B, 2, H, W) or tuple(mask.shape) != (B, H, W):
        raise ValueError("warp_l1: cs1/cs2 [B,C,H,W], flow [B,2,H,W], mask [B,H,W]")
    work = torch.empty(B * ((H * W + 255) // 256), device=cs1.device, dtype=torch.float64)
    out = torch.empty(B, device=cs1.device, dtype=torch.float32)
    _call("mhada_warp_l1", cs1, cs1.data_ptr(), cs2.data_ptr(), flow.data_ptr(), mask.data_ptr(),
                                   work.data_ptr(), out.data_ptr(), B, C, H, W)
    return out


def frame_ingest(frames: torch.Tensor, out_hw=None, bgr: bool = True) -> torch.Tensor:
    _need_gpu(frames)
    if frames.dtype != torch.uint8:
        raise ValueError("frames must be uint8 (H, W, 3) images")
    if frames.dim() == 3:
        frames = frames.unsqueeze(0)
    if frames.dim() != 4 or frames.shape[3] != 3 or frames.stride(3) != 1 or frames.stride(2) != 3:
        raise ValueError(f"frames must be [B][H][W][3] with packed pixels, got {tuple(frames.shape)}")
    B, H, W, _ = frames.shape
    if B > 1 and frames.stride(0) != H * frames.stride(1):
        frames = frames.contiguous()
    Ho, Wo = (H, W) if out_hw is None else out_hw
    out = torch.empty(B, 3, Ho, Wo, device=frames.device, dtype=torch.float32)
    _call("mhada_frame_ingest", frames, frames.data_ptr(), B, H, W, frames.stride(1), int(bgr), out.data_ptr(), Ho, Wo)
    return out


def gemm_tn(a: torch.Tensor, b: torch.Tensor, M: int, N: int, K: int, lda: int, ldb: int = 0,
            b_mode: int = A_ROWS, img=(0, 0, 0), pad: int = 0, colsum: bool = False, nb: int = 1,
            sza: int = 0, szb: int = 0):
    _need_gpu(a, b)
    if a.dtype != torch.float32 or b.dtype != torch.float32:
        raise ValueError("gemm_tn is fp32")
    lib = _lib.load()
    splits = lib.mhada_gemm_tn_splits(M, N, K)
    work = torch.empty(max(1, splits) * (M * N + (M if colsum else 0)) if nb == 1 else
                       max(1, splits // nb) * nb * (M * N + (M if colsum else 0)), device=a.device, dtype=torch.float32)
    c = torch.empty(*((nb,) if nb > 1 else ()), M, N, device=a.device, dtype=torch.float32)
    cs = torch.empty(*((nb,) if nb > 1 else ()), M, device=a.device, dtype=torch.float32) if colsum else None
    args = GemmTnArgs()
    args.M, args.N, args.K = M, N, K
    args.a, args.lda, args.b, args.ldb, args.b_mode = a.data_ptr(), lda, b.data_ptr(), ldb, b_mode
    args.img_c, args.img_h, args.img_w = img
    args.pad = pad
    args.c, args.ldc = c.data_ptr(), N
    args.colsum = cs.data_ptr() if colsum else None
    args.nb, args.sza, args.szb = nb, sza, szb
    _call("mhada_gemm_tn", a, ctypes.byref(args), work.data_ptr(), work.numel())
    return (c, cs) if colsum else c


def colsum(x: torch.Tensor) -> torch.Tensor:
    _need_gpu(x)
    C = x.shape[-1]
    rows = x.numel() // C
    out = torch.empty(C, device=x.device, dtype=torch.float32)
    work = torch.empty(min(128, max(1, rows // 64)) * C, device=x.device, dtype=torch.float32)
    _call("mhada_colsum", x, x.data_ptr(), out.data_ptr(), rows, C, work.data_ptr(), work.numel())
    return out


def relu_bwd(dy: torch.Tensor, y: torch.Tensor) -> torch.Tensor:
    _need_gpu(dy, y)
    dx = torch.empty_like(y)
    _call("mhada_relu_bwd", y, dy.data_ptr(), y.data_ptr(), dx.data_ptr(), y.numel())
    return dx


def feat_stats(x: torch.Tensor, t: Optional[torch.Tensor] = None, stats: bool = True):
    _need_gpu(x, t)
    B, H, W, C = x.shape
    for u in (x, t):
        if u is not None and (u.dtype != torch.float32 or not u.is_contiguous()):
            raise ValueError("feat_stats: contiguous fp32 NHWC operands")
    if t is not None and t.shape != x.shape:
        raise ValueError("feat_stats: target shape")
    if not stats and t is None:
        raise ValueError("feat_stats: nothing to compute")
    P = H * W
    nwork = int(_lib.load().mhada_feat_stats_work(B, P, C))
    work = torch.empty(max(1, nwork), device=x.device, dtype=torch.float64)
    mu = torch.empty(B, C, device=x.device, dtype=torch.float32) if stats else None
    sd = torch.empty(B, C, device=x.device, dtype=torch.float32) if stats else None
    mse = torch.empty((), device=x.device, dtype=torch.float32) if t is not None else None
    ptr = lambda u: None if u is None else u.data_ptr()
    _call("mhada_feat_stats", x, x.data_ptr(), ptr(t), ptr(mu), ptr(sd), ptr(mse), work.data_ptr(), nwork, B, P, C)
    return mu, sd, mse


def feat_loss_bwd(x: torch.Tensor, mu: Optional[torch.Tensor], alpha: Optional[torch.Tensor],
                  beta: Optional[torch.Tensor], t: Optional[torch.Tensor], ks: float,
                  kp: Optional[torch.Tensor] = None, relu: bool = False) -> torch.Tensor:
    _need_gpu(x)
    B, H, W, C = x.shape
    for u in (x, t, mu, alpha, beta, kp):
        if u is not None and (u.dtype != torch.float32 or not u.is_contiguous()):
            raise ValueError("feat_loss_bwd: contiguous fp32 operands")
    if kp is not None and kp.numel() != 1:
        raise ValueError("feat_loss_bwd: kp is one element")
    if t is not None and t.shape != x.shape:
        raise ValueError("feat_loss_bwd: target shape")
    if alpha is not None and not (alpha.shape == beta.shape == mu.shape == (B, C)):
        raise ValueError("feat_loss_bwd: statistics [B][C]")
    g = torch.empty_like(x)
    ptr = lambda u: None if u is None else u.data_ptr()
    _call("mhada_feat_loss_bwd", x, x.data_ptr(), ptr(t), ptr(mu), ptr(alpha), ptr(beta), ptr(kp), float(ks),
          g.data_ptr(), B, H * W, C, int(relu))
    return g


def reflect_fold(dxp: torch.Tensor, relu_mask: Optional[torch.Tensor] = None) -> torch.Tensor:
    _need_gpu(dxp, relu_mask)
    B, Hp, Wp, C = dxp.shape
    dx = torch.empty(B, Hp - 2, Wp - 2, C, device=dxp.device, dtype=torch.float32)
    if relu_mask is not None and (relu_mask.shape != dx.shape or relu_mask.dtype != torch.float32
                                  or not relu_mask.is_contiguous()):
        raise ValueError("reflect_fold: relu_mask must be a contiguous fp32 tensor shaped like the result")
    _call("mhada_reflect_fold", dxp, dxp.data_ptr(), dx.data_ptr(), B, Hp - 2, Wp - 2, C, _ptr(relu_mask))
    return dx


def maxpool2(x: torch.Tensor) -> torch.Tensor:
    _need_gpu(x)
    B, H, W, C = x.shape
    y = torch.empty(B, H // 2, W // 2, C, device=x.device, dtype=torch.float32)
    _call("mhada_maxpool2", x, x.data_ptr(), y.data_ptr(), B, H, W, C)
    return y


def maxpool2_bwd(x: torch.Tensor, dy: torch.Tensor, relu_mask: bool = False) -> torch.Tensor:
    _need_gpu(x, dy)
    B, H, W, C = x.shape
    dx = torch.empty_like(x)
    _call("mhada_maxpool2_bwd", x, x.data_ptr(), dy.data_ptr(), dx.data_ptr(), B, H, W, C, int(relu_mask))
    return dx


def upsample2x_bwd(dy: torch.Tensor, relu_x: Optional[torch.Tensor] = None) -> torch.Tensor:
    _need_gpu(dy, relu_x)
    B, Ho, Wo, C = dy.shape
    dx = torch.empty(B, Ho // 2, Wo // 2, C, device=dy.device, dtype=torch.float32)
    if relu_x is not None and (relu_x.shape != dx.shape or relu_x.dtype != torch.float32 or not relu_x.is_contiguous()):
        raise ValueError("upsample2x_bwd: relu_x must be the contiguous fp32 upsample input")
    _call("mhada_upsample2x_bwd", dy, dy.data_ptr(), _ptr(relu_x), dx.data_ptr(), B, Ho // 2, Wo // 2, C)
    return dx


def vgg_input(img: torch.Tensor, cp: int = 32) -> torch.Tensor:
    _need_gpu(img)
    B, _, H, W = img.shape
    out = torch.empty(B, H, W, cp, device=img.device, dtype=torch.float32)
    _call("mhada_vgg_input", img, img.data_ptr(), out.data_ptr(), B, H, W, cp)
    return out


def vgg_input_bwd(dout: torch.Tensor) -> torch.Tensor:
    _need_gpu(dout)
    B, H, W, cp = dout.shape
    dimg = torch.empty(B, 3, H, W, device=dout.device, dtype=torch.float32)
    _call("mhada_vgg_input_bwd", dout, dout.data_ptr(), dimg.data_ptr(), B, H, W, cp)
    return dimg


def _f32_contig(*ts: torch.Tensor, what: str) -> None:
    for t in ts:
        if t.dtype != torch.float32 or not t.is_contiguous():
            raise ValueError(f"{what}: contiguous fp32 tensors expected")


def vgg_stem_dgrad(dy: torch.Tensor, y: torch.Tensor, wd: torch.Tensor) -> torch.Tensor:
    _need_gpu(dy, y, wd)
    _f32_contig(dy, y, wd, what="vgg_stem_dgrad")
    B, H, W, C = y.shape
    if C != 64 or dy.shape != y.shape or wd.shape != (9, 64, 3):
        raise ValueError("vgg_stem_dgrad: dy, y [B][H][W][64], wd [9][64][3]")
    dimg = torch.empty(B, 3, H, W, device=y.device, dtype=torch.float32)
    _call("mhada_vgg_stem_dgrad", y, dy.data_ptr(), y.data_ptr(), wd.data_ptr(), dimg.data_ptr(), B, H, W)
    return dimg


def out3_dgrad(dy: torch.Tensor, y: torch.Tensor, wd: torch.Tensor, relu_x: Optional[torch.Tensor] = None) -> torch.Tensor:
    _need_gpu(dy, y, wd, relu_x)
    _f32_contig(dy, y, wd, *(() if relu_x is None else (relu_x,)), what="out3_dgrad")
    B, C, H, W = y.shape
    if C != 3 or dy.shape != y.shape or wd.shape != (9, 3, 64):
        raise ValueError("out3_dgrad: dy, y [B][3][H][W], wd [9][3][64]")
    dx = torch.empty(B, H, W, 64, device=y.device, dtype=torch.float32)
    if relu_x is not None and relu_x.shape != dx.shape:
        raise ValueError("out3_dgrad: relu_x must be the [B][H][W][64] layer input")
    _call("mhada_out3_dgrad", y, dy.data_ptr(), y.data_ptr(), wd.data_ptr(), _ptr(relu_x), dx.data_ptr(), B, H, W)
    return dx


def out3_wgrad(x: torch.Tensor, dy: torch.Tensor, y: torch.Tensor, bias: bool = True):
    _need_gpu(x, dy, y)
    _f32_contig(x, dy, y, what="out3_wgrad")
    B, H, W, C = x.shape
    if C != 64 or y.shape != (B, 3, H, W) or dy.shape != y.shape:
        raise ValueError("out3_wgrad: x [B][H][W][64], dy, y [B][3][H][W]")
    lib = _lib.load()
    n = lib.mhada_out3_wgrad_work(B, H, W)
    if n <= 0:
        raise ValueError("out3_wgrad: bad shape")
    work = torch.empty(n, device=x.device, dtype=torch.float32)
    dw = torch.empty(3, 64, 3, 3, device=x.device, dtype=torch.float32)
    db = torch.empty(3, device=x.device, dtype=torch.float32) if bias else None
    _call("mhada_out3_wgrad", x, x.data_ptr(), dy.data_ptr(), y.data_ptr(), dw.data_ptr(), _ptr(db),
          work.data_ptr(), n, B, H, W)
    return dw, db


def rows_normalize(x: torch.Tensor, mu: torch.Tensor, rs: torch.Tensor, unit: bool = False) -> torch.Tensor:
    _need_gpu(x, mu, rs)
    for t in (x, mu, rs):
        if t.dtype != torch.float32 or not t.is_contiguous():
            raise ValueError("rows_normalize needs contiguous float32 rows and statistics")
    B, N, C = x.shape
    if mu.shape != (B, C) or rs.shape != (B, C):
        raise ValueError(f"rows_normalize: statistics {tuple(mu.shape)} do not match rows {tuple(x.shape)}")
    out = torch.empty_like(x)
    _call("mhada_rows_normalize", x, x.data_ptr(), mu.data_ptr(), rs.data_ptr(), out.data_ptr(), int(unit), B, N, C)
    return out


def loss_attn(qn: torch.Tensor, kn: torch.Tensor, v: torch.Tensor, x: torch.Tensor, x_mu: torch.Tensor,
              x_rs: torch.Tensor, activation: int) -> torch.Tensor:
    _need_gpu(qn, kn, v, x, x_mu, x_rs)
    for t in (qn, kn, v, x):
        if t.dtype != torch.float32 or not t.is_contiguous():
            raise ValueError("loss_attn operands must be contiguous float32 token rows")
    B, Nq, Dqk = qn.shape
    Ns, Dv = v.shape[1], v.shape[2]
    if kn.shape != (B, Ns, Dqk) or x.shape != (B, Nq, Dv):
        raise ValueError(f"loss_attn: bad shapes q{tuple(qn.shape)} k{tuple(kn.shape)} v{tuple(v.shape)} "
                         f"x{tuple(x.shape)}")
    out = torch.empty(B, Nq, Dv, device=qn.device, dtype=torch.float32)
    _call("mhada_loss_attn", qn, qn.data_ptr(), kn.data_ptr(), v.data_ptr(), x.data_ptr(), x_mu.data_ptr(),
          x_rs.data_ptr(), out.data_ptr(), B, Nq, Ns, Dqk, Dv, activation)
    return out


def vit_batch_attn_bwd(qkv: torch.Tensor, dout: torch.Tensor, L: int, ntok: int, heads: int,
                       groups: int = 1, planes: bool = False):
    _need_gpu(qkv, dout)
    C = qkv.shape[-1] // 3
    if L % groups:
        raise ValueError("vit_batch_attn_bwd: L must be a multiple of groups")
    dqkv = torch.empty_like(qkv)
    pl = torch.empty(3, L * ntok, 3 * C, device=qkv.device, dtype=torch.bfloat16) if planes else None
    Lg = L // groups
    for g in range(groups):
        o3, o1 = g * Lg * ntok * 3 * C * 4, g * Lg * ntok * C * 4
        if planes:
            _call("mhada_vit_batch_attn_bwd_split3", qkv, qkv.data_ptr() + o3, dout.data_ptr() + o1,
                  dqkv.data_ptr() + o3, pl.data_ptr() + o3 // 2, L * ntok * 3 * C, Lg, ntok, heads, C // heads)
        else:
            _call("mhada_vit_batch_attn_bwd", qkv, qkv.data_ptr() + o3, dout.data_ptr() + o1, dqkv.data_ptr() + o3,
                  Lg, ntok, heads, C // heads)
    return (dqkv, pl) if planes else dqkv
```

Before: 371.1 frames/s.

## Compute attention QK^T with scaled two-plane fp16 split instead of bf16x3

Adds a half2 form of the fp32-emulating attention in which Q and K are scaled by power-of-two exponents (per query row and per 64-key tile) and split into hi/lo fp16 planes. QK^T then takes three f16 MFMAs instead of six bf16 ones, and the K part of the image shrinks from three planes to two. Per-tile exponents are stored in the image tail, and the running-max offset is folded into the accumulator init, with range checks falling back to adding it after the MFMAs. The aim is to cut MFMA work and K traffic in the attention score loop. In exchange it adds exponent reductions, ldexp rescaling and a different accuracy profile, and it is enabled by default.

Result: no change. 374.6 frames/s (median of 6 runs) (+0.9%).

```diff
diff --git a/include/mhada_hip.h b/include/mhada_hip.h
--- a/include/mhada_hip.h
+++ b/include/mhada_hip.h
@@ -114,6 +114,15 @@
 int mhada_attn_split3_planes(const float* q, const void* img, const float* fcs, const float* fcs_mu,
                              const float* fcs_rstd, const float* v_mu, void* planes, int B, int H, int Nc, int Ns,
                              mhada_stream_t stream);
+int mhada_split3_kv_half2(const float* kv, const float* vt, void* img, int B, int H, int Ns, mhada_stream_t stream);
+int mhada_kv_proj_half2(const float* fs, const float* mu_s, const float* wkv, const float* bkv, void* img,
+                        int B, int H, int Ns, mhada_stream_t stream);
+int mhada_attn_half2(const float* q, const void* img, const float* fcs, const float* fcs_mu,
+                     const float* fcs_rstd, const float* v_mu, float* out, int B, int H, int Nc, int Ns,
+                     mhada_stream_t stream);
+int mhada_attn_half2_planes(const float* q, const void* img, const float* fcs, const float* fcs_mu,
+                            const float* fcs_rstd, const float* v_mu, void* planes, int B, int H, int Nc, int Ns,
+                            mhada_stream_t stream);
 
 int mhada_cosine_moments(const void* kv, const void* vt, int dtype, int B, int H, int Ns, float* mom,
                          float* work, int splits, mhada_stream_t stream);
diff --git a/mhada-style-transfer_amd/csrc/attn_split3.hip b/mhada-style-transfer_amd/csrc/attn_split3.hip
--- a/mhada-style-transfer_amd/csrc/attn_split3.hip
+++ b/mhada-style-transfer_amd/csrc/attn_split3.hip
@@ -21,16 +21,70 @@
   c[e] = s.c;
 }
 
+typedef _Float16 f16x8 __attribute__((ext_vector_type(8)));
+typedef _Float16 f16x4 __attribute__((ext_vector_type(4)));
+
+__host__ __device__ constexpr long long h2_image(int ldt) { return 512LL * ldt + ldt / 8; }
+
+MHADA_DEV int h2_exp(unsigned mbits) {
+  const int e = (int)(mbits >> 23);
+  return (e == 0 || e == 255) ? 0 : 141 - e;
+}
+MHADA_DEV unsigned abs_bits(float x) { return __float_as_uint(x) & 0x7fffffffu; }
+MHADA_DEV unsigned wave_max_u(unsigned v) {
+#pragma unroll
+  for (int o = 32; o > 0; o >>= 1) {
+    const unsigned w = (unsigned)__shfl_xor((int)v, o, 64);
+    v = v > w ? v : w;
+  }
+  return v;
+}
+template <typename V>
+MHADA_DEV void split2_into(float x, int ex, V& hi, V& lo, int e) {
+  const float s = ldexpf(x, ex);
+  const _Float16 h = half2_plane(s);
+  hi[e] = h;
+  lo[e] = half2_plane(s - (float)h);
+}
+
+template <bool H2>
 __global__ void __launch_bounds__(256) split3_kv_kernel(const float* __restrict__ kv, const float* __restrict__ vt,
                                                         bf16* __restrict__ img, int Ns, int ldt) {
   const int bh = blockIdx.y, n0 = blockIdx.x * 64, tid = threadIdx.x;
-  bf16* kp = img + (long long)bh * s3_image(ldt);
-  bf16* vp = kp + 192LL * ldt;
+  bf16* kp = img + (long long)bh * (H2 ? h2_image(ldt) : s3_image(ldt));
+  bf16* vp = kp + (H2 ? 128LL : 192LL) * ldt;
   const float* kvb = kv + (long long)bh * Ns * 128;
   const float* vtb = vt + (long long)bh * 128 * ldt;
   const long long kps = 64LL * ldt, vps = 128LL * ldt;
-#pragma unroll
-  for (int i = 0; i < 4; ++i) {
+  if constexpr (H2) {
+    __shared__ unsigned red[4];
+    f32x4 x[4];
+    unsigned mb = 0;
+#pragma unroll
+    for (int i = 0; i < 4; ++i) {
+      const int idx = tid + 256 * i, key = n0 + (idx >> 4), d = (idx & 15) * 4;
+      x[i] = key < Ns ? *reinterpret_cast<const f32x4*>(kvb + (long long)key * 128 + d) : f32x4{0.f, 0.f, 0.f, 0.f};
+#pragma unroll
+      for (int e = 0; e < 4; ++e) mb = max(mb, abs_bits(x[i][e]));
+    }
+    mb = wave_max_u(mb);
+    if ((tid & 63) == 0) red[tid >> 6] = mb;
+    __syncthreads();
+    const int ex = h2_exp(max(max(red[0], red[1]), max(red[2], red[3])));
+    if (tid == 0) reinterpret_cast<int*>(kp + 512LL * ldt)[4 * blockIdx.x] = ex;
+#pragma unroll
+    for (int i = 0; i < 4; ++i) {
+      const int idx = tid + 256 * i, key = n0 + (idx >> 4), d = (idx & 15) * 4;
+      f16x4 hi, lo;
+#pragma unroll
+      for (int e = 0; e < 4; ++e) split2_into(x[i][e], ex, hi, lo, e);
+      _Float16* dst = reinterpret_cast<_Float16*>(kp) + (long long)key * 64 + d;
+      *reinterpret_cast<f16x4*>(dst) = hi;
+      *reinterpret_cast<f16x4*>(dst + kps) = lo;
+    }
+  }
+#pragma unroll
+  for (int i = 0; i < (H2 ? 0 : 4); ++i) {
     const int idx = tid + 256 * i, key = n0 + (idx >> 4), d = (idx & 15) * 4;
     const f32x4 x = key < Ns ? *reinterpret_cast<const f32x4*>(kvb + (long long)key * 128 + d) : f32x4{0.f, 0.f, 0.f, 0.f};
     bf16x4 a, b, c;
@@ -56,6 +110,7 @@
   }
 }
 
+template <bool H2>
 __global__ void __launch_bounds__(256) kv_proj_s3_kernel(const float* __restrict__ fs, const float* __restrict__ mu,
                                                          const float* __restrict__ wkv, const float* __restrict__ bkv,
                                                          bf16* __restrict__ img, int H, int Ns, int ldt) {
@@ -109,11 +164,41 @@
       sY[o * LY + 32 * nb + r32] = acc[ni][r] + bb[o];
     }
   __syncthreads();
-  bf16* kp = img + (long long)bh * s3_image(ldt);
-  bf16* vp = kp + 192LL * ldt;
+  bf16* kp = img + (long long)bh * (H2 ? h2_image(ldt) : s3_image(ldt));
+  bf16* vp = kp + (H2 ? 128LL : 192LL) * ldt;
   const long long kps = 64LL * ldt, vps = 128LL * ldt;
-#pragma unroll
-  for (int i = 0; i < 2; ++i) {
+  if constexpr (H2) {
+    unsigned* red = reinterpret_cast<unsigned*>(sm + 128 * LY);
+    float y[2][8];
+    unsigned mb = 0;
+#pragma unroll
+    for (int i = 0; i < 2; ++i) {
+      const int idx = tid + 256 * i, n = idx >> 3, o0 = (idx & 7) * 8;
+      const bool valid = n0 + n < Ns;
+#pragma unroll
+      for (int j = 0; j < 8; ++j) {
+        y[i][j] = valid ? sY[(o0 + j) * LY + n] : 0.f;
+        mb = max(mb, abs_bits(y[i][j]));
+      }
+    }
+    mb = wave_max_u(mb);
+    if (lane == 0) red[wave] = mb;
+    __syncthreads();
+    const int ex = h2_exp(max(max(red[0], red[1]), max(red[2], red[3])));
+    if (tid == 0) reinterpret_cast<int*>(kp + 512LL * ldt)[4 * blockIdx.x] = ex;
+#pragma unroll
+    for (int i = 0; i < 2; ++i) {
+      const int idx = tid + 256 * i, n = idx >> 3, o0 = (idx & 7) * 8;
+      f16x8 hi, lo;
+#pragma unroll
+      for (int j = 0; j < 8; ++j) split2_into(y[i][j], ex, hi, lo, j);
+      _Float16* dst = reinterpret_cast<_Float16*>(kp) + (long long)(n0 + n) * 64 + o0;
+      *reinterpret_cast<f16x8*>(dst) = hi;
+      *reinterpret_cast<f16x8*>(dst + kps) = lo;
+    }
+  }
+#pragma unroll
+  for (int i = 0; i < (H2 ? 0 : 2); ++i) {
     const int idx = tid + 256 * i, n = idx >> 3, o0 = (idx & 7) * 8;
     const bool valid = n0 + n < Ns;
     bf16x8 a, c1, c2;
@@ -155,10 +240,16 @@
   return __builtin_amdgcn_mfma_f32_16x16x32_bf16(a0, b0, acc, 0, 0, 0);
 }
 
-template <bool QK32>
+MHADA_DEV f32x4 mfma3h(const f16x8& ah, const f16x8& al, const f16x8& bh, const f16x8& bl, f32x4 acc) {
+  acc = __builtin_amdgcn_mfma_f32_16x16x32_f16(al, bh, acc, 0, 0, 0);
+  acc = __builtin_amdgcn_mfma_f32_16x16x32_f16(ah, bh, acc, 0, 0, 0);
+  return __builtin_amdgcn_mfma_f32_16x16x32_f16(ah, bl, acc, 0, 0, 0);
+}
+
+template <bool QK32, bool QH2 = false>
 MHADA_DEV void attn_exact_q3(const AttnP& p, const bf16* kp, const bf16* vp, const bf16x8 (&qf)[3][2][2],
                              const float (&qreg)[2][16], f32x4 (&O)[2][8], float (&lt)[2], float (&mx)[2], int g,
-                             int r16) {
+                             int r16, const f16x8 (&qh)[2][2][2], const int (&aq)[2], const int* etab) {
   const int Ns = p.Ns;
   const long long kps = 64LL * p.ldt, vps = 128LL * p.ldt;
   const f32x4 z4 = {0.f, 0.f, 0.f, 0.f};
@@ -175,8 +266,23 @@
 #pragma unroll
           for (int qg = 0; qg < 2; ++qg) S[qg][t] = __builtin_amdgcn_mfma_f32_16x16x4f32(kf[st], qreg[qg][st], S[qg][t], 0, 0, 0);
       }
-#pragma unroll
-      for (int dh = 0; dh < (QK32 ? 0 : 2); ++dh) {
+      if constexpr (QH2) {
+        const _Float16* kh = reinterpret_cast<const _Float16*>(kr);
+#pragma unroll
+        for (int dh = 0; dh < 2; ++dh) {
+          const f16x8 khi = *reinterpret_cast<const f16x8*>(kh + 32 * dh);
+          const f16x8 klo = *reinterpret_cast<const f16x8*>(kh + kps + 32 * dh);
+#pragma unroll
+          for (int qg = 0; qg < 2; ++qg) S[qg][t] = mfma3h(khi, klo, qh[0][qg][dh], qh[1][qg][dh], S[qg][t]);
+        }
+        const int et = etab[4 * (k0 >> 6)];
+#pragma unroll
+        for (int qg = 0; qg < 2; ++qg)
+#pragma unroll
+          for (int j = 0; j < 4; ++j) S[qg][t][j] = ldexpf(S[qg][t][j], -(aq[qg] + et));
+      }
+#pragma unroll
+      for (int dh = 0; dh < (QK32 || QH2 ? 0 : 2); ++dh) {
         const bf16x8 k0f = *reinterpret_cast<const bf16x8*>(kr + 32 * dh);
         const bf16x8 k1f = *reinterpret_cast<const bf16x8*>(kr + kps + 32 * dh);
         const bf16x8 k2f = *reinterpret_cast<const bf16x8*>(kr + 2 * kps + 32 * dh);
@@ -323,11 +429,12 @@
   }
 }
 
-template <int NW, bool TRAIN = false, bool QK32 = false, int ACC = 0, int IL = 0, bool PLANES = false>
+template <int NW, bool TRAIN = false, bool QK32 = false, int ACC = 0, int IL = 0, bool PLANES = false, bool QH2 = false>
 __global__ void __launch_bounds__(64 * NW, 1) attn_s3_kernel(const AttnP p) {
+  static_assert(!QH2 || (!TRAIN && !QK32 && ACC == 0), "HALF2 Q K^T: the inference form only");
   constexpr int TK = kS3Tk;
   constexpr int KPL = TK * 64, VPL = 128 * TK;
-  constexpr int KREG = QK32 ? 2 * TK * 64 : 3 * KPL;
+  constexpr int KREG = QK32 || QH2 ? 2 * TK * 64 : 3 * KPL;
   constexpr int SLOT = KREG + 3 * VPL;
   constexpr int KPC = KREG / 512, VPC = 3 * VPL / 512;
   static_assert(KPC % NW == 0 && VPC % NW == 0, "tile config");
@@ -344,9 +451,34 @@
 
   bf16x8 qf[3][2][2];
   float qreg[2][16];
+  f16x8 qh[2][2][2];
+  int aq[2] = {0, 0};
 #pragma unroll
   for (int qg = 0; qg < 2; ++qg) {
     const int q = q0 + 16 * qg + r16;
+    if constexpr (QH2) {
+      const float* qp = reinterpret_cast<const float*>(p.q) + (bh * p.Nc + (q < p.Nc ? q : 0)) * 64 + 8 * g;
+      float x[2][8];
+      unsigned mb = 0;
+#pragma unroll
+      for (int dh = 0; dh < 2; ++dh) {
+        const f32x4 lo = *reinterpret_cast<const f32x4*>(qp + 32 * dh);
+        const f32x4 hi = *reinterpret_cast<const f32x4*>(qp + 32 * dh + 4);
+#pragma unroll
+        for (int e = 0; e < 8; ++e) {
+          x[dh][e] = q < p.Nc ? (e < 4 ? lo[e] : hi[e - 4]) : 0.f;
+          mb = max(mb, abs_bits(x[dh][e]));
+        }
+      }
+      mb = max(mb, (unsigned)__shfl_xor((int)mb, 16, 64));
+      mb = max(mb, (unsigned)__shfl_xor((int)mb, 32, 64));
+      aq[qg] = h2_exp(mb);
+#pragma unroll
+      for (int dh = 0; dh < 2; ++dh)
+#pragma unroll
+        for (int e = 0; e < 8; ++e) split2_into(x[dh][e], aq[qg], qh[0][qg][dh], qh[1][qg][dh], e);
+      continue;
+    }
     if constexpr (QK32) {
       const float* qr = reinterpret_cast<const float*>(p.q) + (bh * p.Nc + (q < p.Nc ? q : 0)) * 64 + g;
 #pragma unroll
@@ -365,8 +497,9 @@
       }
     }
   }
-  const bf16* kp = reinterpret_cast<const bf16*>(p.kv) + bh * s3_image(ldt);
-  const bf16* vp = kp + 192LL * ldt;
+  const bf16* kp = reinterpret_cast<const bf16*>(p.kv) + bh * (QH2 ? h2_image(ldt) : s3_image(ldt));
+  const bf16* vp = kp + (QH2 ? 128LL : 192LL) * ldt;
+  const int* etab = reinterpret_cast<const int*>(kp + 512LL * ldt);
   int ksrc[KPW], vsrc[VPW];
 #pragma unroll
   for (int i = 0; i < KPW; ++i) {
@@ -419,6 +552,25 @@
       return;
     }
     const bf16* ck = smem + sl * SLOT;
+    if constexpr (QH2) {
+      const _Float16* ch = reinterpret_cast<const _Float16*>(ck);
+#pragma unroll
+      for (int kg = 0; kg < 2; ++kg)
+#pragma unroll
+        for (int t = 0; t < 2; ++t) {
+          const _Float16* kr = ch + kg * 32 * 64 + krow[t];
+#pragma unroll
+          for (int dh = 0; dh < 2; ++dh) {
+            const int off = 8 * ((4 * dh + g) ^ (r16 & 7));
+            const f16x8 khi = *reinterpret_cast<const f16x8*>(kr + off);
+            const f16x8 klo = *reinterpret_cast<const f16x8*>(kr + KPL + off);
+#pragma unroll
+            for (int qg = 0; qg < 2; ++qg)
+              S[qg][kg][t] = mfma3h(khi, klo, qh[0][qg][dh], qh[1][qg][dh], dh == 0 ? init[qg] : S[qg][kg][t]);
+          }
+        }
+      return;
+    }
 #pragma unroll
     for (int kg = 0; kg < 2; ++kg)
 #pragma unroll
@@ -541,9 +693,46 @@
   asm volatile("s_waitcnt vmcnt(0)" ::: "memory");
   __syncthreads();
   f32x4 Sa[2][2][2], Cm[2];
+  int qlo[2] = {0, 0}, qhi[2] = {0, 0}, wlo = 0, whi = 0;
+  auto qk_h2 = [&](int tile, f32x4 (&S)[2][2][2], bool first) {
+    const int et = etab[4 * tile];
+    const bool fast = first || (et >= wlo && et <= whi);
+    f32x4 init[2];
+    float post[2];
+    int n[2];
+#pragma unroll
+    for (int qg = 0; qg < 2; ++qg) {
+      n[qg] = aq[qg] + et;
+      const bool ok = fast || (et >= qlo[qg] && et <= qhi[qg]);
+      const float c = first || !ok ? 0.f : ldexpf(Cm[qg][0], n[qg]);
+      init[qg] = f32x4{c, c, c, c};
+      post[qg] = first || ok ? 0.f : Cm[qg][0];
+    }
+    qk(tile & 1, S, init);
+    if (fast) {
+#pragma unroll
+      for (int qg = 0; qg < 2; ++qg)
+#pragma unroll
+        for (int kg = 0; kg < 2; ++kg)
+#pragma unroll
+          for (int t = 0; t < 2; ++t)
+#pragma unroll
+            for (int j = 0; j < 4; ++j) S[qg][kg][t][j] = ldexpf(S[qg][kg][t][j], -n[qg]);
+    } else {
+#pragma unroll
+      for (int qg = 0; qg < 2; ++qg)
+#pragma unroll
+        for (int kg = 0; kg < 2; ++kg)
+#pragma unroll
+          for (int t = 0; t < 2; ++t)
+#pragma unroll
+            for (int j = 0; j < 4; ++j) S[qg][kg][t][j] = ldexpf(S[qg][kg][t][j], -n[qg]) + post[qg];
+    }
+  };
   {
     const f32x4 zi[2] = {z4, z4};
-    qk(0, Sa, zi);
+    if constexpr (QH2) qk_h2(0, Sa, true);
+    else qk(0, Sa, zi);
     if (NFULL == 0) s3_mask(Sa, 0, Ns, g);
 #pragma unroll
     for (int qg = 0; qg < 2; ++qg) {
@@ -563,6 +752,22 @@
 #pragma unroll
           for (int j = 0; j < 4; ++j) Sa[qg][kg][t][j] -= m;
       Cm[qg] = f32x4{-m, -m, -m, -m};
+      if constexpr (QH2) {
+        const int em = (int)(abs_bits(m) >> 23);
+        const bool any = m == 0.f || em == 255;
+        qlo[qg] = any ? -(1 << 20) : em == 0 ? 1 : 1 - em - aq[qg];
+        qhi[qg] = any ? (1 << 20) : em == 0 ? 0 : 250 - em - aq[qg];
+      }
+    }
+    if constexpr (QH2) {
+      int lo = max(qlo[0], qlo[1]), hi = min(qhi[0], qhi[1]);
+#pragma unroll
+      for (int o = 32; o > 0; o >>= 1) {
+        lo = max(lo, __shfl_xor(lo, o, 64));
+        hi = min(hi, __shfl_xor(hi, o, 64));
+      }
+      wlo = __builtin_amdgcn_readfirstlane(lo);
+      whi = __builtin_amdgcn_readfirstlane(hi);
     }
   }
   if (NTILE > 1) stage(TK, 1);
@@ -571,13 +776,15 @@
   __builtin_amdgcn_s_barrier();
   for (int t = 1; t < NFULL; ++t) {
     if (t + 1 < NTILE) stage((t + 1) * TK, (t + 1) & 1);
-    qk(t & 1, Sa, Cm);
+    if constexpr (QH2) qk_h2(t, Sa, false);
+    else qk(t & 1, Sa, Cm);
     finish(t & 1, Sa);
     asm volatile("s_waitcnt vmcnt(0)" ::: "memory");
     __builtin_amdgcn_s_barrier();
   }
   if (NFULL < NTILE && NFULL > 0) {
-    qk(NFULL & 1, Sa, Cm);
+    if constexpr (QH2) qk_h2(NFULL, Sa, false);
+    else qk(NFULL & 1, Sa, Cm);
     s3_mask(Sa, NFULL * TK, Ns, g);
     finish(NFULL & 1, Sa);
   }
@@ -587,7 +794,7 @@
     lt[qg] = ACC ? lsum[qg] : L[qg][0];
     mx[qg] = -Cm[qg][0];
   }
-  if (__any(!(lt[0] <= kShiftSumThr) || !(lt[1] <= kShiftSumThr))) attn_exact_q3<QK32>(p, kp, vp, qf, qreg, O, lt, mx, g, r16);
+  if (__any(!(lt[0] <= kShiftSumThr) || !(lt[1] <= kShiftSumThr))) attn_exact_q3<QK32, QH2>(p, kp, vp, qf, qreg, O, lt, mx, g, r16, qh, aq, etab);
   if constexpr (TRAIN) attn_train_epilogue_q(p, O, lt, mx, bh, q0, g, r16);
   else attn_epilogue_q<float, PLANES>(p, O, lt, b, hh, q0, g, r16);
 }
@@ -611,9 +818,20 @@
   const long long bhn = (long long)B * H;
   if (bhn > 65535) return fail("mhada_split3_kv: B * H > 65535");
   const int ldt = (Ns + 63) / 64 * 64;
-  hipLaunchKernelGGL(split3_kv_kernel, dim3(ldt / 64, (unsigned)bhn), dim3(256), 0, (hipStream_t)s_, kv, vt,
+  hipLaunchKernelGGL(split3_kv_kernel<false>, dim3(ldt / 64, (unsigned)bhn), dim3(256), 0, (hipStream_t)s_, kv, vt,
                      reinterpret_cast<bf16*>(img), Ns, ldt);
   return check_launch("mhada_split3_kv");
+}
+
+extern "C" int mhada_split3_kv_half2(const float* kv, const float* vt, void* img, int B, int H, int Ns,
+                                     mhada_stream_t s_) {
+  if (!kv || !vt || !img || B <= 0 || H <= 0 || Ns <= 0) return fail("mhada_split3_kv_half2: bad args");
+  const long long bhn = (long long)B * H;
+  if (bhn > 65535) return fail("mhada_split3_kv_half2: B * H > 65535");
+  const int ldt = (Ns + 63) / 64 * 64;
+  hipLaunchKernelGGL(split3_kv_kernel<true>, dim3(ldt / 64, (unsigned)bhn), dim3(256), 0, (hipStream_t)s_, kv, vt,
+                     reinterpret_cast<bf16*>(img), Ns, ldt);
+  return check_launch("mhada_split3_kv_half2");
 }
 
 extern "C" int mhada_kv_proj_split3(const float* fs, const float* mu_s, const float* wkv, const float* bkv, void* img,
@@ -622,14 +840,25 @@
   const long long bhn = (long long)B * H;
   if (bhn > 65535) return fail("mhada_kv_proj_split3: B * H > 65535");
   const int ldt = (Ns + 63) / 64 * 64;
-  hipLaunchKernelGGL(kv_proj_s3_kernel, dim3(ldt / 64, (unsigned)bhn), dim3(256), 0, (hipStream_t)s_, fs, mu_s, wkv, bkv,
-                     reinterpret_cast<bf16*>(img), H, Ns, ldt);
+  hipLaunchKernelGGL(kv_proj_s3_kernel<false>, dim3(ldt / 64, (unsigned)bhn), dim3(256), 0, (hipStream_t)s_, fs, mu_s, wkv,
+                     bkv, reinterpret_cast<bf16*>(img), H, Ns, ldt);
   return check_launch("mhada_kv_proj_split3");
+}
+
+extern "C" int mhada_kv_proj_half2(const float* fs, const float* mu_s, const float* wkv, const float* bkv, void* img,
+                                   int B, int H, int Ns, mhada_stream_t s_) {
+  if (!fs || !mu_s || !wkv || !bkv || !img || B <= 0 || H <= 0 || Ns <= 0) return fail("mhada_kv_proj_half2: bad args");
+  const long long bhn = (long long)B * H;
+  if (bhn > 65535) return fail("mhada_kv_proj_half2: B * H > 65535");
+  const int ldt = (Ns + 63) / 64 * 64;
+  hipLaunchKernelGGL(kv_proj_s3_kernel<true>, dim3(ldt / 64, (unsigned)bhn), dim3(256), 0, (hipStream_t)s_, fs, mu_s, wkv,
+                     bkv, reinterpret_cast<bf16*>(img), H, Ns, ldt);
+  return check_launch("mhada_kv_proj_half2");
 }
 
 static int attn_split3_launch(const char* name, const float* q, const void* img, const float* fcs, const float* fcs_mu,
                               const float* fcs_rstd, const float* v_mu, void* out, bool planes, int B, int H, int Nc,
-                              int Ns, mhada_stream_t s_) {
+                              int Ns, mhada_stream_t s_, bool qh2 = false) {
   if (!q || !img || !fcs || !fcs_mu || !fcs_rstd || !v_mu || !out || B <= 0 || H <= 0 || Nc <= 0 || Ns <= 0)
     return fail(std::string(name) + ": bad args");
   AttnP p = {};
@@ -644,6 +873,16 @@
   if (nblk > (1LL << 31) - 1) return fail(std::string(name) + ": grid too large");
   p.nblk = (int)nblk;
   const hipStream_t s = (hipStream_t)s_;
+  if (qh2) {
+    if (planes) {
+      if (nw == 8) hipLaunchKernelGGL((attn_s3_kernel<8, false, false, 0, 1, true, true>), dim3(p.nblk), dim3(512), 0, s, p);
+      else hipLaunchKernelGGL((attn_s3_kernel<4, false, false, 0, 1, true, true>), dim3(p.nblk), dim3(256), 0, s, p);
+    } else {
+      if (nw == 8) hipLaunchKernelGGL((attn_s3_kernel<8, false, false, 0, 1, false, true>), dim3(p.nblk), dim3(512), 0, s, p);
+      else hipLaunchKernelGGL((attn_s3_kernel<4, false, false, 0, 1, false, true>), dim3(p.nblk), dim3(256), 0, s, p);
+    }
+    return check_launch(name);
+  }
   if (planes) {
     if (nw == 8) hipLaunchKernelGGL((attn_s3_kernel<8, false, false, 0, 1, true>), dim3(p.nblk), dim3(512), 0, s, p);
     else hipLaunchKernelGGL((attn_s3_kernel<4, false, false, 0, 1, true>), dim3(p.nblk), dim3(256), 0, s, p);
@@ -665,6 +904,19 @@
                                         int Ns, mhada_stream_t s_) {
   return attn_split3_launch("mhada_attn_split3_planes", q, img, fcs, fcs_mu, fcs_rstd, v_mu, planes, true, B, H, Nc, Ns,
                             s_);
+}
+
+extern "C" int mhada_attn_half2(const float* q, const void* img, const float* fcs, const float* fcs_mu,
+                                const float* fcs_rstd, const float* v_mu, float* out, int B, int H, int Nc, int Ns,
+                                mhada_stream_t s_) {
+  return attn_split3_launch("mhada_attn_half2", q, img, fcs, fcs_mu, fcs_rstd, v_mu, out, false, B, H, Nc, Ns, s_, true);
+}
+
+extern "C" int mhada_attn_half2_planes(const float* q, const void* img, const float* fcs, const float* fcs_mu,
+                                       const float* fcs_rstd, const float* v_mu, void* planes, int B, int H, int Nc,
+                                       int Ns, mhada_stream_t s_) {
+  return attn_split3_launch("mhada_attn_half2_planes", q, img, fcs, fcs_mu, fcs_rstd, v_mu, planes, true, B, H, Nc, Ns,
+                            s_, true);
 }
 
 extern "C" int mhada_attn_train_fwd_split3(const float* q, const float* k, const float* v, void* img, const float* x,
diff --git a/mhada-style-transfer_amd/mhada_hip/_lib.py b/mhada-style-transfer_amd/mhada_hip/_lib.py
--- a/mhada-style-transfer_amd/mhada_hip/_lib.py
+++ b/mhada-style-transfer_amd/mhada_hip/_lib.py
@@ -79,6 +79,10 @@
     "mhada_vit_batch_attn_half2": (_I, [_vp, _vp, _c_ll, _vp, _I, _I, _I, _I, _vp]),
     "mhada_attn_split3": (_I, [_vp] * 7 + [_I, _I, _I, _I, _vp]),
     "mhada_attn_split3_planes": (_I, [_vp] * 7 + [_I, _I, _I, _I, _vp]),
+    "mhada_split3_kv_half2": (_I, [_vp, _vp, _vp, _I, _I, _I, _vp]),
+    "mhada_kv_proj_half2": (_I, [_vp] * 5 + [_I, _I, _I, _vp]),
+    "mhada_attn_half2": (_I, [_vp] * 7 + [_I, _I, _I, _I, _vp]),
+    "mhada_attn_half2_planes": (_I, [_vp] * 7 + [_I, _I, _I, _I, _vp]),
     "mhada_attn_train_fwd": (_I, [_vp] * 7 + [_I, _I, _I, _vp]),
     "mhada_attn_train_fwd_vt": (_I, [_vp] * 8 + [_I, _I, _I, _vp]),
     "mhada_attn_train_fwd_split3": (_I, [_vp] * 8 + [_I, _I, _I, _vp]),
diff --git a/mhada-style-transfer_amd/mhada_hip/engine.py b/mhada-style-transfer_amd/mhada_hip/engine.py
--- a/mhada-style-transfer_amd/mhada_hip/engine.py
+++ b/mhada-style-transfer_amd/mhada_hip/engine.py
@@ -278,11 +278,14 @@
     mom = img = kv = vt = None
     act = ACT_COSINE if blk.activation_name == "cosine" else ACT_SOFTMAX
     split_attn = act == ACT_SOFTMAX and dt == torch.float32 and ops.F32_SPLIT_ATTN
+    qk_half2 = bool(split_attn and ops.F32_ATTN_QK_HALF2)
     if cached:
         mu_s, rstd_s, mom, Ns = side["mu_s"], side["rstd_s"], side.get("mom"), side["Ns"]
         kv, vt, img = side.get("kv"), side.get("vt"), side.get("img")
         if side["B"] != B:
             raise ValueError(f"cached style batch {side['B']} != content batch {B}")
+        if img is not None and side.get("img_half2", False) != qk_half2:
+            raise ValueError("the cached style image was written for the other attention form")
     else:
         if fs.t.shape[2] != C:
             raise ValueError(f"channel mismatch: block expects {C}")
@@ -300,9 +303,9 @@
              bias=prep["bf"], sb=(0, HEAD_DIM), ldc=HEAD_DIM, sc=(H * Nc * HEAD_DIM, Nc * HEAD_DIM))
     if not cached and split_attn:
         Ns = fs.t.shape[1]
-        img = ops.kv_proj_split3(fs.t, mu_s, wkv, bkv)
+        img = ops.kv_proj_split3(fs.t, mu_s, wkv, bkv, half2=qk_half2)
         if side is not None:
-            side.update(mu_s=mu_s, rstd_s=rstd_s, img=img, Ns=Ns, B=B)
+            side.update(mu_s=mu_s, rstd_s=rstd_s, img=img, img_half2=qk_half2, Ns=Ns, B=B)
     elif not cached:
         Ns = fs.t.shape[1]
         kv = torch.empty(B, H, Ns, 2 * HEAD_DIM, device=dev, dtype=dt)
@@ -324,7 +327,7 @@
             att = ops.cosine_attn(q, mom, fcs.t, mu_o, rstd_o, v_mu)
     elif split_attn and ops.F32_SPLIT_OUTPROJ and _split3_fills(B * Nc, C, dev):
         with _timed("mhada_attn"):
-            att3 = ops.attn_split3_planes(q, img, Ns, fcs.t, mu_o, rstd_o, v_mu)
+            att3 = ops.attn_split3_planes(q, img, Ns, fcs.t, mu_o, rstd_o, v_mu, half2=qk_half2)
         if "w_out_split3" not in prep:
             with torch.no_grad():
                 prep["w_out_split3"] = ops.split3_weight(prep["w_out"])
@@ -332,7 +335,7 @@
         return _Feat(out.view(B, Nc, C), fc.h, fc.w)
     elif split_attn:
         with _timed("mhada_attn"):
-            att = ops.attn_split3(q, img, Ns, fcs.t, mu_o, rstd_o, v_mu)
+            att = ops.attn_split3(q, img, Ns, fcs.t, mu_o, rstd_o, v_mu, half2=qk_half2)
     else:
         with _timed("mhada_attn"):
             att = ops.mhada_attn(q, kv, vt, fcs.t, mu_o, rstd_o, v_mu, act)
@@ -466,7 +469,7 @@
         return [None] * len(ada.adaAttnHead), False
     sig = tuple(_signature(b) for b in ada.adaAttnHead)
     vers = tuple(t._version for t in fs)
-    mode = (dt, ops.F32_SPLIT_ATTN)
+    mode = (dt, ops.F32_SPLIT_ATTN, ops.F32_ATTN_QK_HALF2)
     c = ada.__dict__.get("_mhada_style")
     if (c is not None and c["mode"] == mode and c["sig"] == sig and c["vers"] == vers
             and len(c["refs"]) == len(fs) and all(r() is t for r, t in zip(c["refs"], fs))):
diff --git a/mhada-style-transfer_amd/mhada_hip/ops.py b/mhada-style-transfer_amd/mhada_hip/ops.py
--- a/mhada-style-transfer_amd/mhada_hip/ops.py
+++ b/mhada-style-transfer_amd/mhada_hip/ops.py
@@ -870,8 +870,19 @@
 
 F32_SPLIT_ATTN = True
 
-
-def split3_kv(kv: torch.Tensor, vt: torch.Tensor) -> torch.Tensor:
+F32_ATTN_QK_HALF2 = True
+
+
+def half2_image_len(Ns: int) -> int:
+    ldt = (Ns + 63) // 64 * 64
+    return 512 * ldt + ldt // 8
+
+
+def _attn_image_len(Ns: int, half2: bool) -> int:
+    return half2_image_len(Ns) if half2 else 576 * ((Ns + 63) // 64 * 64)
+
+
+def split3_kv(kv: torch.Tensor, vt: torch.Tensor, half2: bool = False) -> torch.Tensor:
     _need_gpu(kv, vt)
     B, H, Ns, _ = kv.shape
     ldt = (Ns + 63) // 64 * 64
@@ -879,12 +890,26 @@
             or kv.shape[3] != 128 or not kv.is_contiguous() or not vt.is_contiguous():
         raise ValueError(f"split3_kv: needs contiguous fp32 kv [B][H][Ns][128] and vt [B][H][128][{ldt}], "
                          f"got {tuple(kv.shape)} / {tuple(vt.shape)}")
-    img = torch.empty(B, H, 576 * ldt, device=kv.device, dtype=torch.bfloat16)
-    _call("mhada_split3_kv", kv, kv.data_ptr(), vt.data_ptr(), img.data_ptr(), B, H, Ns)
+    img = torch.empty(B, H, _attn_image_len(Ns, half2), device=kv.device, dtype=torch.bfloat16)
+    _call("mhada_split3_kv_half2" if half2 else "mhada_split3_kv", kv, kv.data_ptr(), vt.data_ptr(), img.data_ptr(),
+          B, H, Ns)
     return img
 
 
-def kv_proj_split3(fs: torch.Tensor, mu_s: torch.Tensor, wkv: torch.Tensor, bkv: torch.Tensor) -> torch.Tensor:
+def kv_proj_half2(fs: torch.Tensor, mu_s: torch.Tensor, wkv: torch.Tensor, bkv: torch.Tensor) -> torch.Tensor:
+    return kv_proj_split3(fs, mu_s, wkv, bkv, half2=True)
+
+
+def attn_half2(q, img, Ns: int, fcs, fcs_mu, fcs_rstd, v_mu) -> torch.Tensor:
+    return attn_split3(q, img, Ns, fcs, fcs_mu, fcs_rstd, v_mu, half2=True)
+
+
+def attn_half2_planes(q, img, Ns: int, fcs, fcs_mu, fcs_rstd, v_mu) -> torch.Tensor:
+    return attn_split3_planes(q, img, Ns, fcs, fcs_mu, fcs_rstd, v_mu, half2=True)
+
+
+def kv_proj_split3(fs: torch.Tensor, mu_s: torch.Tensor, wkv: torch.Tensor, bkv: torch.Tensor,
+                   half2: bool = False) -> torch.Tensor:
     _need_gpu(fs, mu_s, wkv, bkv)
     B, Ns, C = fs.shape
     H = C // 64
@@ -894,37 +919,36 @@
     if C % 64 or mu_s.shape != (B, C) or wkv.shape != (B, H, 128, 64) or bkv.shape != (H, 128):
         raise ValueError(f"kv_proj_split3: bad shapes fs {tuple(fs.shape)} mu {tuple(mu_s.shape)} "
                          f"wkv {tuple(wkv.shape)} bkv {tuple(bkv.shape)}")
-    ldt = (Ns + 63) // 64 * 64
-    img = torch.empty(B, H, 576 * ldt, device=fs.device, dtype=torch.bfloat16)
-    _call("mhada_kv_proj_split3", fs, fs.data_ptr(), mu_s.data_ptr(), wkv.data_ptr(), bkv.data_ptr(), img.data_ptr(),
-          B, H, Ns)
+    img = torch.empty(B, H, _attn_image_len(Ns, half2), device=fs.device, dtype=torch.bfloat16)
+    _call("mhada_kv_proj_half2" if half2 else "mhada_kv_proj_split3", fs, fs.data_ptr(), mu_s.data_ptr(),
+          wkv.data_ptr(), bkv.data_ptr(), img.data_ptr(), B, H, Ns)
     return img
 
 
-def attn_split3(q, img, Ns: int, fcs, fcs_mu, fcs_rstd, v_mu) -> torch.Tensor:
+def attn_split3(q, img, Ns: int, fcs, fcs_mu, fcs_rstd, v_mu, half2: bool = False) -> torch.Tensor:
     _need_gpu(q, img, fcs, fcs_mu, fcs_rstd, v_mu)
     B, H, Nc, _ = q.shape
-    ldt = (Ns + 63) // 64 * 64
+    n = _attn_image_len(Ns, half2)
     if q.dtype != torch.float32 or not q.is_contiguous() or img.dtype != torch.bfloat16 \
-            or img.shape != (B, H, 576 * ldt):
-        raise ValueError(f"attn_split3: q must be contiguous fp32 and img bf16 [B][H][576*{ldt}], got "
+            or img.shape != (B, H, n) or not img.is_contiguous():
+        raise ValueError(f"attn_split3: q must be contiguous fp32 and img bf16 [B][H][{n}], got "
                          f"{q.dtype} / {tuple(img.shape)}")
     out = torch.empty(B, Nc, H * 64, device=q.device, dtype=torch.float32)
-    _call("mhada_attn_split3", q, q.data_ptr(), img.data_ptr(), fcs.data_ptr(), fcs_mu.data_ptr(),
+    _call("mhada_attn_half2" if half2 else "mhada_attn_split3", q, q.data_ptr(), img.data_ptr(), fcs.data_ptr(), fcs_mu.data_ptr(),
           fcs_rstd.data_ptr(), v_mu.data_ptr(), out.data_ptr(), B, H, Nc, Ns)
     return out
 
 
-def attn_split3_planes(q, img, Ns: int, fcs, fcs_mu, fcs_rstd, v_mu) -> torch.Tensor:
+def attn_split3_planes(q, img, Ns: int, fcs, fcs_mu, fcs_rstd, v_mu, half2: bool = False) -> torch.Tensor:
     _need_gpu(q, img, fcs, fcs_mu, fcs_rstd, v_mu)
     B, H, Nc, _ = q.shape
-    ldt = (Ns + 63) // 64 * 64
+    n = _attn_image_len(Ns, half2)
     if q.dtype != torch.float32 or not q.is_contiguous() or img.dtype != torch.bfloat16 \
-            or img.shape != (B, H, 576 * ldt):
-        raise ValueError(f"attn_split3_planes: q must be contiguous fp32 and img bf16 [B][H][576*{ldt}], got "
+            or img.shape != (B, H, n) or not img.is_contiguous():
+        raise ValueError(f"attn_split3_planes: q must be contiguous fp32 and img bf16 [B][H][{n}], got "
                          f"{q.dtype} / {tuple(img.shape)}")
     planes = torch.empty(3, B * Nc, H * 64, device=q.device, dtype=torch.bfloat16)
-    _call("mhada_attn_split3_planes", q, q.data_ptr(), img.data_ptr(), fcs.data_ptr(), fcs_mu.data_ptr(),
+    _call("mhada_attn_half2_planes" if half2 else "mhada_attn_split3_planes", q, q.data_ptr(), img.data_ptr(), fcs.data_ptr(), fcs_mu.data_ptr(),
           fcs_rstd.data_ptr(), v_mu.data_ptr(), planes.data_ptr(), B, H, Nc, Ns)
     return planes
 
```
